# PlatformLab/RAMCloud

Hardware: AMD Instinct MI355X
Metric: device-resident CRC32C GB/s over 8MiB-segment batch; % of HBM roofline (higher is better)
Workload: dtype u8; 1 GPU; 1024 x 8 MiB device-resident segments (BASELINE config 2); segments_per_gpu=1024, segment_bytes=8388608, batch_bytes_per_gpu=8589934592, parallelism=single, exchange=none

## Files before the change

### ramcloud_amd/csrc/dev_checks.inc

```

namespace {

__device__ __forceinline__ uint32_t crc_bytes_g(const uint32_t* t1, uint32_t c, const gu8* p,
                                                uint32_t n)
{
    for (uint32_t k = 0; k < n; k++)
        c = t1[(c ^ p[k]) & 0xFF] ^ (c >> 8);
    return c;
}

__device__ __forceinline__ uint32_t le32_g(const gu8* p)
{
    return uint32_t(p[0]) | (uint32_t(p[1]) << 8) | (uint32_t(p[2]) << 16) | (uint32_t(p[3]) << 24);
}


__device__ __forceinline__ void obj_compare_one(const BatchDesc& d, ramcrc_seg_status* status,
                                                uint64_t i);

__global__ __launch_bounds__(256) void k_obj_compare(BatchDesc d, ramcrc_seg_status* status,
                                                     const uint32_t* nother)
{
    if (nother && *nother == 0)
        return;
    const uint64_t n = entry_count<kRecords>(d);
    for (uint64_t i = uint64_t(blockIdx.x) * blockDim.x + threadIdx.x; i < n;
         i += uint64_t(gridDim.x) * blockDim.x)
        obj_compare_one(d, status, i);
}

__device__ __forceinline__ void obj_compare_one(const BatchDesc& d, ramcrc_seg_status* status,
                                                uint64_t i)
{
    const u32x4 r = d.rec[i];
    const uint32_t type = r.w & 0x3f;
    const uint32_t hdr = replay_header_bytes(type);
    if (hdr == 0)
        return;
    const bool readable = r.z >= hdr && !(r.w & kRecOverlong);
    if (d.vstat && type == RAMCRC_LOG_ENTRY_TYPE_OBJ && readable && !is_large(uint64_t(r.z) - 4))
        return;
    const uint64_t payload = reinterpret_cast<uint64_t>(d.base) + uint64_t(r.x) * d.seg_bytes +
                             r.y + 1 + ((r.w >> 6) & 3) + 1;
    const gu8* p = reinterpret_cast<const gu8*>(payload);
    const uint32_t seg_flags = d.seg_status[r.x].x;
    uint32_t stored = 0, computed = 0;
    if (type == RAMCRC_LOG_ENTRY_TYPE_OBJ && readable) {
        stored = le32_g(p);
        computed = d.out[i];
    }
    if (!(seg_flags & RAMCRC_SEG_OK))
        return;
    bool ok = false;
    if (readable) {
        if (type == RAMCRC_LOG_ENTRY_TYPE_OBJ) {
            ok = computed == stored;
        } else {
            uint32_t at = hdr - 4, from = hdr, tail = 0;
            bool fits = true;
            switch (type) {
            case RAMCRC_LOG_ENTRY_TYPE_OBJTOMB: tail = r.z - hdr; break;
            case RAMCRC_LOG_ENTRY_TYPE_PREP:
                at = kPrepHeaderBytes - 4;
                from = kPrepHeaderBytes + 4;
                tail = r.z - from;
                break;
            case RAMCRC_LOG_ENTRY_TYPE_TXDECISION:
                tail = min(24u * le32_g(p + 36), r.z - hdr);
                break;
            case RAMCRC_LOG_ENTRY_TYPE_TXPLIST:
                tail = 24u * le32_g(p + 16);
                fits = tail <= r.z - hdr;
                break;
            default: break;
            }
            if (fits) {
                const uint32_t* t1 = &g_tab.pos[1 + kTinyRow0][0];
                const uint32_t c = ~crc_bytes_g(t1, crc_bytes_g(t1, 0xFFFFFFFFu, p, at), p + from, tail);
                d.out[i] = c;
                ok = c == le32_g(p + at);
            }
        }
    }
    if (!ok)
        atomicAdd(&status[r.x].bad_objects, 1u);
}

__global__ __launch_bounds__(256) void k_left(BatchDesc d, ramcrc_seg_status* status, const uint32_t* sum,
                                              const uint32_t* left, const unsigned long long* nleft,
                                              uint64_t left_cap, uint64_t nseg)
{
    const uint32_t sv = *sum;
    if (!(sv & kSumFast))
        return;
    const uint64_t tid = uint64_t(blockIdx.x) * blockDim.x + threadIdx.x, nt = uint64_t(gridDim.x) * blockDim.x;
    if (sv & kHardFull) {
        for (uint64_t s = tid; s < nseg; s += nt)
            status[s].bad_objects = 0;
        return;
    }
    const uint64_t nl = *nleft;
    const uint64_t n = nl < left_cap ? nl : left_cap;
    if (uint64_t(blockIdx.x) * blockDim.x >= n)
        return;
    __shared__ uint32_t tx4[4 * 256], tx1[256];
    for (uint32_t t = threadIdx.x; t < 4 * 256; t += blockDim.x)
        tx4[t] = g_tab.comb[0].t[t >> 8][t & 0xFF];
    for (uint32_t t = threadIdx.x; t < 256; t += blockDim.x)
        tx1[t] = g_tab.t0.t[t];
    __syncthreads();
    auto crc_global = [&](uint64_t a, uint32_t m) {
        typedef const __attribute__((address_space(1))) uint32_t g32;
        uint32_t c = 0xFFFFFFFFu;
        while (m && (a & 3)) {
            c = tx1[(c ^ *reinterpret_cast<const gu8*>(a)) & 0xFF] ^ (c >> 8);
            a++;
            m--;
        }
        for (; m >= 8; a += 8, m -= 8) {
            const uint32_t v0 = *reinterpret_cast<g32*>(a), v1 = *reinterpret_cast<g32*>(a + 4);
            uint32_t v = v0 ^ c;
            c = xor3(tx4[v & 0xFF], tx4[256 + ((v >> 8) & 0xFF)], tx4[512 + ((v >> 16) & 0xFF)]) ^
                tx4[768 + (v >> 24)];
            v = v1 ^ c;
            c = xor3(tx4[v & 0xFF], tx4[256 + ((v >> 8) & 0xFF)], tx4[512 + ((v >> 16) & 0xFF)]) ^
                tx4[768 + (v >> 24)];
        }
        while (m) {
            c = tx1[(c ^ *reinterpret_cast<const gu8*>(a)) & 0xFF] ^ (c >> 8);
            a++;
            m--;
        }
        return ~c;
    };
    for (uint64_t k = tid; k < n; k += nt) {
        const uint64_t i = left[k];
        const u32x4 r = d.rec[i];
        if (!replay_other(r)) {
            if ((r.w & 0x3f) != RAMCRC_LOG_ENTRY_TYPE_OBJ || !(d.seg_status[r.x].x & RAMCRC_SEG_OK))
                continue;
            const uint64_t payload = reinterpret_cast<uint64_t>(d.base) + uint64_t(r.x) * d.seg_bytes +
                                     r.y + 1 + ((r.w >> 6) & 3) + 1;
            const gu8* p = reinterpret_cast<const gu8*>(payload);
            const uint32_t c = crc_global(payload + 4, r.z - 4);
            d.out[i] = c;
            if (c != le32_g(p))
                atomicAdd(&status[r.x].bad_objects, 1u);
        } else {
            obj_compare_one(d, status, i);
        }
    }
}

__global__ __launch_bounds__(256) void k_obj_stamp(BatchDesc d)
{
    const uint64_t i = uint64_t(blockIdx.x) * blockDim.x + threadIdx.x;
    if (i >= d.n)
        return;
    if (d.len[i] < kObjHeaderBytes) {
        d.out[i] = 0;
        return;
    }
    const uint32_t c = d.out[i];
    uint8_t* p = const_cast<uint8_t*>(d.base) + d.off[i];
    p[0] = uint8_t(c);
    p[1] = uint8_t(c >> 8);
    p[2] = uint8_t(c >> 16);
    p[3] = uint8_t(c >> 24);
}

__global__ __launch_bounds__(256) void k_cert_prep(const uint32_t* heads, ramcrc_seg_cert* certs,
                                                   uint64_t n)
{
    const uint64_t i = uint64_t(blockIdx.x) * blockDim.x + threadIdx.x;
    if (i < n)
        certs[i] = ramcrc_seg_cert{heads[i], 0u};
}

__global__ __launch_bounds__(256) void k_cert_emit(const ramcrc_seg_cert* tmp,
                                                   const ramcrc_seg_status* st,
                                                   ramcrc_seg_cert* certs, uint32_t* flags, uint64_t n)
{
    const uint64_t i = uint64_t(blockIdx.x) * blockDim.x + threadIdx.x;
    if (i >= n)
        return;
    const ramcrc_seg_status s = st[i];
    certs[i] = ramcrc_seg_cert{tmp[i].segment_length, s.checksum};
    if (flags) {
        const uint32_t bad = s.flags & (RAMCRC_SEG_PAST_CAPACITY | RAMCRC_SEG_PAST_LENGTH |
                                        RAMCRC_SEG_CYCLE);
        flags[i] = bad ? bad : RAMCRC_SEG_OK;
    }
}


}
```

### ramcloud_amd/csrc/dev_chunks.inc

```

namespace {

__device__ __forceinline__ uint32_t scan_chunk(const uint8_t* lds, const RepOp& op, int lane,
                                               uint64_t S, uint64_t E, uint32_t init,
                                               uint64_t lo, uint64_t hi)
{
    uint32_t u0 = 0, u1 = 0, u2 = 0, u3 = 0;
    uint64_t first = lo & ~uint64_t(kBlock - 1);
    const uint64_t end = (hi + kBlock - 1) & ~uint64_t(kBlock - 1);

    auto step = [&](const u32x4& w) {
        u0 = op.apply(lds, u0, w.x);
        u1 = op.apply(lds, u1, w.y);
        u2 = op.apply(lds, u2, w.z);
        u3 = op.apply(lds, u3, w.w);
    };
    auto special = [&](uint64_t blk) {
        const uint64_t a = blk + uint64_t(lane) * 16;
        u32x4 w = {0u, 0u, 0u, 0u};
        if (a < E && a + 16 > S)
            w = load16(a);
        w.x = fix_word(w.x, a + 0, S, E, init);
        w.y = fix_word(w.y, a + 4, S, E, init);
        w.z = fix_word(w.z, a + 8, S, E, init);
        w.w = fix_word(w.w, a + 12, S, E, init);
        step(w);
    };

    while (first < end && (first < S + 4 || first + kBlock > E)) {
        special(first);
        first += kBlock;
    }
    uint64_t fast_end = end;
    if (first < end && end > E)
        fast_end = end - kBlock;

    const uint64_t nf = (fast_end - first) / kBlock;
    if (nf > 0) {
        const uint32_t lo_w = __builtin_amdgcn_readfirstlane(uint32_t(first));
        const uint32_t hi_w = __builtin_amdgcn_readfirstlane(uint32_t(first >> 32));
        const uint32_t nrec = __builtin_amdgcn_readfirstlane(uint32_t(nf * kBlock));
        void* basep = reinterpret_cast<void*>((uint64_t(hi_w) << 32) | lo_w);
        const __amdgpu_buffer_rsrc_t rsrc =
            __builtin_amdgcn_make_buffer_rsrc(basep, (short)0, int(nrec), 0x00020000);
        const uint32_t voff = uint32_t(lane) * 16;
        auto ldb = [&](uint64_t b) -> u32x4 {
            b = b < nf ? b : nf - 1;
            return __builtin_amdgcn_raw_buffer_load_b128(rsrc, voff, uint32_t(b * kBlock),
                                                         2 );
        };
        u32x4 A[kUnroll], B[kUnroll];
#pragma unroll
        for (int j = 0; j < kUnroll; j++)
            A[j] = ldb(j);
        uint64_t i = 0;
        for (; i + 2 * kUnroll <= nf; i += 2 * kUnroll) {
#pragma unroll
            for (int j = 0; j < kUnroll; j++)
                B[j] = ldb(i + kUnroll + j);
            __builtin_amdgcn_sched_barrier(0);
#pragma unroll
            for (int j = 0; j < kUnroll; j++)
                step(A[j]);
#pragma unroll
            for (int j = 0; j < kUnroll; j++)
                A[j] = ldb(i + 2 * kUnroll + j);
            __builtin_amdgcn_sched_barrier(0);
#pragma unroll
            for (int j = 0; j < kUnroll; j++)
                step(B[j]);
        }
#pragma unroll
        for (int j = 0; j < kUnroll; j++)
            if (i + j < nf)
                step(A[j]);
        if (i + kUnroll < nf) {
#pragma unroll
            for (int j = 0; j < kUnroll; j++)
                B[j] = ldb(i + kUnroll + j);
#pragma unroll
            for (int j = 0; j < kUnroll; j++)
                if (i + kUnroll + j < nf)
                    step(B[j]);
        }
    }
    if (fast_end < end)
        special(fast_end);

    uint32_t y = plain_apply(lds, kCombOff, u0) ^ u1;
    y = plain_apply(lds, kCombOff, y) ^ u2;
    y = plain_apply(lds, kCombOff, y) ^ u3;
    uint32_t z = plain_apply(lds, kCombOff, y);
#pragma unroll
    for (int lvl = 0; lvl < 6; lvl++) {
        const uint32_t other = __shfl_xor(z, 1 << lvl, kWaveSize);
        const bool upper = (lane >> lvl) & 1;
        const uint32_t lower_v = upper ? other : z;
        const uint32_t upper_v = upper ? z : other;
        z = plain_apply(lds, kCombOff + (1 + lvl) * 4096, lower_v) ^ upper_v;
    }
    return z;
}

__device__ __forceinline__ bool replay_other(const u32x4& r)
{
    const uint32_t type = r.w & 0x3f;
    const uint32_t hdr = replay_header_bytes(type);
    const bool readable = r.z >= hdr && !(r.w & kRecOverlong);
    return hdr != 0 && !(type == RAMCRC_LOG_ENTRY_TYPE_OBJ && readable && !is_large(uint64_t(r.z) - 4));
}



__device__ __forceinline__ void plan_locate(const Plan& pl, uint64_t n, uint64_t g, uint64_t& entry,
                                            uint64_t& k)
{
    uint64_t lo = 0, hi = pl.ngroups;
    while (hi - lo > 1) {
        const uint64_t mid = (lo + hi) >> 1;
        if (pl.group_pref[mid] <= g) lo = mid; else hi = mid;
    }
    const uint64_t gbase = pl.group_pref[lo];
    uint64_t a = lo * kThreads, b = a + kThreads;
    if (b > n) b = n;
    uint64_t l2 = a, h2 = b;
    while (h2 - l2 > 1) {
        const uint64_t mid = (l2 + h2) >> 1;
        if (gbase + pl.local[mid] <= g) l2 = mid; else h2 = mid;
    }
    entry = l2;
    k = g - gbase - pl.local[l2];
}

template <int kMode>
__global__ __launch_bounds__(kThreads, 1) void k_chunks(BatchDesc d, Plan pl, uint64_t per_seg)
{
    __shared__ __attribute__((aligned(16))) uint8_t lds[kLdsChunks];
    if (kMode != kSegAligned && plan_empty(pl))
        return;
    fill_replicated(lds, g_tab.stride_large);
    fill_plain(lds, kCombOff, &g_tab.comb[0].t[0][0], 7 * 1024);
    __syncthreads();

    const int lane = threadIdx.x & (kWaveSize - 1);
    const RepOp op(lane);
    const uint64_t wave = uint64_t(blockIdx.x) * kWavesPerGroup +
                          __builtin_amdgcn_readfirstlane(threadIdx.x / kWaveSize);
    const uint64_t nwaves = uint64_t(gridDim.x) * kWavesPerGroup;
    const uint64_t total = kMode == kSegAligned ? per_seg * d.n : pl.group_pref[pl.ngroups];
    if (total > pl.partials_cap) {
        if (wave == 0 && lane == 0)
            atomicOr(pl.status, 3u);
        return;
    }
    uint64_t g = wave;
    while (g < total) {
        const uint64_t gnext = g + nwaves;
        uint64_t i, k;
        if (kMode == kSegAligned) {
            i = g / per_seg;
            k = g - i * per_seg;
        } else {
            plan_locate(pl, d.n, g, i, k);
        }
        uint64_t S, E;
        buffer_range<kMode>(d, i, S, E);
        const uint32_t init = d.init ? d.init[i] : 0xFFFFFFFFu;
        const uint64_t cs = S >> d.cshift;
        const uint64_t c_lo = (cs + k) << d.cshift;
        const uint64_t lo = c_lo > S ? c_lo : S;
        const uint64_t c_hi = c_lo + (1ull << d.cshift);
        const uint64_t hi = c_hi < E ? c_hi : E;
        const uint32_t r = scan_chunk(lds, op, lane, S, E, init, lo, hi);
        if (lane == 0)
            pl.partials[g] = r;
        g = gnext;
    }
}

__device__ __forceinline__ uint64_t shfl64(uint64_t v, int src)
{
    const uint32_t lo = __shfl(uint32_t(v), src, kWaveSize);
    const uint32_t hi = __shfl(uint32_t(v >> 32), src, kWaveSize);
    return (uint64_t(hi) << 32) | lo;
}

template <int kMode>
__device__ __forceinline__ void combine_one(const BatchDesc& d, const Plan& pl, uint64_t per_seg,
                                            uint64_t i, uint64_t S, uint64_t E, int lane)
{
    const uint64_t g0 = kMode == kSegAligned ? i * per_seg
                                             : pl.group_pref[i / kThreads] + pl.local[i];
    const uint64_t cnt = chunk_count(S, E, d.cshift);
    const uint64_t cs = S >> d.cshift;
    const uint64_t pend = (E + kBlock - 1) & ~uint64_t(kBlock - 1);
    uint32_t R = 0;
    for (uint64_t k = lane; k < cnt; k += kWaveSize) {
        const uint32_t r = pl.partials[g0 + k];
        const uint64_t ek = (k + 1 == cnt) ? pend : ((cs + k + 1) << d.cshift);
        const uint64_t t = (pend - ek) / kBlock;
        R ^= t ? mulmod_dev(r, xpow_blocks(t)) : r;
    }
#pragma unroll
    for (int lvl = 0; lvl < 6; lvl++)
        R ^= __shfl_xor(R, 1 << lvl, kWaveSize);
    const uint32_t pad = uint32_t(pend - E);
    if (pad)
        R = mulmod_dev(R, g_tab.xinv[pad]);
    if (lane == 0)
        d.out[i] = (d.flags & RAMCRC_FINALIZE) ? ~R : R;
}

template <int kMode, bool kWide>
__global__ __launch_bounds__(256) void k_combine(BatchDesc d, Plan pl, uint64_t per_seg)
{
    const int lane = threadIdx.x & (kWaveSize - 1);
    const uint64_t wave = uint64_t(blockIdx.x) * (256 / kWaveSize) + threadIdx.x / kWaveSize;
    if (kMode != kSegAligned && (plan_empty(pl) || ((*pl.status) & kStatusRefused)))
        return;
    const uint64_t n = entry_count<kMode>(d);
    if (!kWide) {
        if (wave >= n)
            return;
        uint64_t S, E;
        buffer_range<kMode>(d, wave, S, E);
        if (is_large(E - S))
            combine_one<kMode>(d, pl, per_seg, wave, S, E, lane);
        return;
    }
    if (pl.group_pref[pl.ngroups] == 0)
        return;
    const uint64_t nwave = uint64_t(gridDim.x) * (256 / kWaveSize);
    for (uint64_t wv = wave; wv * kWaveSize < n; wv += nwave) {
        const uint64_t i = wv * kWaveSize + lane;
        uint64_t S = 0, E = 0;
        const bool big = i < n && buffer_range<kMode>(d, i, S, E) && is_large(E - S);
        uint64_t todo = __ballot(big);
        while (todo) {
            const int j = __builtin_ctzll(todo);
            todo &= todo - 1;
            combine_one<kMode>(d, pl, per_seg, wv * kWaveSize + j, shfl64(S, j), shfl64(E, j), lane);
        }
    }
}


}
```

### ramcloud_amd/csrc/dev_host.inc

```

namespace {

thread_local int t_last_hip = 0;

#define HIPCHK(expr)                              \
    do {                                          \
        hipError_t e_ = (expr);                   \
        if (e_ != hipSuccess) {                   \
            t_last_hip = int(e_);                 \
            return RAMCRC_EHIP;                   \
        }                                         \
    } while (0)

struct DeviceGuard {
    int prev = -1;
    bool ok = false;
    explicit DeviceGuard(int dev)
    {
        if (hipGetDevice(&prev) != hipSuccess)
            prev = -1;
        ok = hipSetDevice(dev) == hipSuccess;
    }
    ~DeviceGuard()
    {
        if (prev >= 0)
            (void)hipSetDevice(prev);
    }
};

}

struct ramcrc_ctx {
    int device = 0;
    int ncu = 256;
    int ncu_all = 256;
    std::recursive_mutex mu;
    uint32_t* partials = nullptr;
    uint64_t partials_cap = 0;
    uint64_t* plan_local = nullptr;
    uint64_t plan_cap = 0;
    uint64_t* group_pref = nullptr;
    uint64_t group_cap = 0;
    uint32_t* status = nullptr;
    BinTable* bins = nullptr;
    uint32_t bin_par = 0;
    int fail_after_count = 0;
    uint32_t dirty_bins = 0;
    int bin_straggler = 0;
    int bin_resident[5] = {-1, -1, -1, -1, -1};
    int bin_one = 0;
    u32x4* sdesc = nullptr;
    uint32_t* sidx = nullptr;
    uint32_t* sinit = nullptr;
    uint64_t sorted_cap = 0;
    uint32_t* obj_out = nullptr;
    uint64_t obj_out_cap = 0;
    uint32_t* cert_scratch = nullptr;
    uint64_t cert_scratch_cap = 0;
    uint8_t* h_stage = nullptr;
    uint64_t h_stage_cap = 0;
    uint8_t* d_stage = nullptr;
    uint64_t d_stage_cap = 0;
    hipStream_t copy_stream = nullptr;
    hipStream_t compute_stream = nullptr;
    void* walk_parts = nullptr;
    uint64_t walk_parts_cap = 0;
    uint32_t* walk_fallback = nullptr;
    uint64_t walk_fallback_cap = 0;
    uint64_t* walk_base = nullptr;
    uint64_t walk_base_cap = 0;
    void* walk_recs = nullptr;
    uint64_t walk_recs_cap = 0;
    void* walk_pool = nullptr;
    uint64_t walk_pool_cap = 0;
    uint32_t* walk_pool_owner = nullptr;
    uint64_t walk_pool_owner_cap = 0;
    uint32_t* walk_blocks = nullptr;
    uint64_t walk_blocks_cap = 0;
    unsigned long long* walk_pool_used = nullptr;
    uint64_t walk_pool_used_cap = 0;
    int verify_in_walk = 1;
    uint32_t* walk_left = nullptr;
    uint64_t walk_left_cap = 0;
    uint32_t* walk_sum = nullptr;
    uint64_t walk_sum_cap = 0;
    bool serial_walk = false;
    uint32_t walk_pshift = 0;
    bool timing = false;
    std::vector<std::pair<hipEvent_t, hipEvent_t>> ev_used, ev_free;
};

namespace {

int grow_device(void** p, uint64_t* cap, uint64_t need_elems, size_t elem)
{
    if (*cap >= need_elems && *p)
        return RAMCRC_OK;
    uint64_t n = need_elems < 1024 ? 1024 : need_elems;
    if (*p) {
        HIPCHK(hipDeviceSynchronize());
        HIPCHK(hipFree(*p));
        *p = nullptr;
        *cap = 0;
    }
    if (hipMalloc(p, n * elem) != hipSuccess) {
        *p = nullptr;
        return RAMCRC_ENOMEM;
    }
    *cap = n;
    return RAMCRC_OK;
}

int reserve_locked(ramcrc_ctx* c, uint64_t max_chunks, uint64_t max_entries)
{
    int rc = grow_device(reinterpret_cast<void**>(&c->partials), &c->partials_cap, max_chunks,
                         sizeof(uint32_t));
    if (rc)
        return rc;
    rc = grow_device(reinterpret_cast<void**>(&c->plan_local), &c->plan_cap, max_entries,
                     sizeof(uint64_t));
    if (rc)
        return rc;
    const uint64_t ngroups = (max_entries + kThreads - 1) / kThreads + 1;
    return grow_device(reinterpret_cast<void**>(&c->group_pref), &c->group_cap, ngroups,
                       sizeof(uint64_t));
}

uint64_t default_chunk_bound(uint64_t n)
{
    size_t free_b = 0, total_b = 0;
    if (hipMemGetInfo(&free_b, &total_b) != hipSuccess)
        total_b = 288ull << 30;
    return total_b / kChunk + 2 * n + 16;
}

Plan make_plan(ramcrc_ctx* c, uint64_t n)
{
    Plan pl{};
    pl.local = c->plan_local;
    pl.group_pref = c->group_pref;
    pl.ngroups = (n + kThreads - 1) / kThreads;
    pl.partials = c->partials;
    pl.partials_cap = c->partials_cap;
    pl.status = c->status;
    return pl;
}

constexpr unsigned kTimerEventFlags = hipEventDisableSystemFence;

struct ScanTimer {
    ramcrc_ctx* c;
    hipStream_t s;
    std::pair<hipEvent_t, hipEvent_t> ev{nullptr, nullptr};
    ScanTimer(ramcrc_ctx* ctx, hipStream_t stream) : c(ctx), s(stream)
    {
        if (!c->timing)
            return;
        if (!c->ev_free.empty()) {
            ev = c->ev_free.back();
            c->ev_free.pop_back();
        } else if (hipEventCreateWithFlags(&ev.first, kTimerEventFlags) != hipSuccess ||
                   hipEventCreateWithFlags(&ev.second, kTimerEventFlags) != hipSuccess) {
            ev = {nullptr, nullptr};
        }
    }
    template <typename F, typename... Args>
    void launch(F kernel, dim3 grid, dim3 block, Args... args)
    {
        if (ev.first)
            hipExtLaunchKernelGGL(kernel, grid, block, 0, s, ev.first, ev.second, 0, args...);
        else
            hipLaunchKernelGGL(kernel, grid, block, 0, s, args...);
    }
    ~ScanTimer()
    {
        if (ev.first)
            c->ev_used.push_back(ev);
    }
};

int reserve_sorted(ramcrc_ctx* c, uint64_t n)
{
    const uint64_t need = n + uint64_t(kG) * kNB;
    if (c->sorted_cap >= need)
        return RAMCRC_OK;
    uint64_t cap = c->sorted_cap;
    int rc = grow_device(reinterpret_cast<void**>(&c->sdesc), &cap, need, sizeof(u32x4));
    if (rc)
        return rc;
    cap = c->sorted_cap;
    rc = grow_device(reinterpret_cast<void**>(&c->sidx), &cap, need, sizeof(uint32_t));
    if (rc)
        return rc;
    cap = c->sorted_cap;
    rc = grow_device(reinterpret_cast<void**>(&c->sinit), &cap, need, sizeof(uint32_t));
    if (rc)
        return rc;
    c->sorted_cap = cap;
    return RAMCRC_OK;
}

uint64_t bin_grid(const ramcrc_ctx* c, uint64_t n)
{
    uint64_t grid = (n + uint64_t(kThreads) * kBinPer - 1) / (uint64_t(kThreads) * kBinPer);
    if (grid > uint64_t(c->ncu) * kBinWgsPerCu)
        grid = uint64_t(c->ncu) * kBinWgsPerCu;
    return grid;
}

template <int kMode>
int bin_begin(ramcrc_ctx* c, const BatchDesc& d, hipStream_t s, int skip_large, Sorted* so,
              const uint32_t* sum = nullptr)
{
    if (d.n >= (1ull << 32))
        return RAMCRC_EINVAL;
    int rc = reserve_sorted(c, d.n);
    if (rc)
        return rc;
    *so = Sorted{c->bins, c->sdesc, c->sidx, c->sinit, c->status, c->sorted_cap, c->bin_par, 0};
    if (hipError_t stale = hipGetLastError(); stale != hipSuccess)
        t_last_hip = int(stale);
    const uint64_t tiles = (d.n + uint64_t(kThreads) * kBinPer - 1) / (uint64_t(kThreads) * kBinPer);
    int& resident = c->bin_resident[kMode];
    if (resident < 0) {
        int nb = 0;
        if (hipOccupancyMaxActiveBlocksPerMultiprocessor(&nb, k_bin_one<kMode>, kThreads, 0) !=
            hipSuccess)
            nb = 0;
        resident = nb;
    }
    if (c->bin_one && !c->dirty_bins && !sum && tiles > 0 &&
        tiles <= uint64_t(c->ncu) * uint64_t(std::min(resident / 2, int(kBinWgsPerCu)))) {
        so->one = 1;
        hipLaunchKernelGGL(k_bin_one<kMode>, dim3(tiles), dim3(kThreads), 0, s, d, *so, skip_large,
                           c->bin_straggler ? 1u : 0u);
        c->bin_straggler = 0;
    } else {
        hipLaunchKernelGGL(k_bin_count<kMode>, dim3(bin_grid(c, d.n)), dim3(kThreads), 0, s, d,
                           *so, skip_large, sum);
    }
    HIPCHK(hipGetLastError());
    c->bin_par ^= 1u;
    return RAMCRC_OK;
}

template <int kMode>
int bin_finish(ramcrc_ctx* c, const BatchDesc& d, hipStream_t s, int skip_large, const Sorted& so,
               const uint32_t* sum = nullptr)
{
    if (c->fail_after_count > 0) {
        c->fail_after_count--;
        return RAMCRC_EHIP;
    }
    if (c->dirty_bins) {
        hipLaunchKernelGGL(k_test_dirty_bins, dim3(1), dim3(1), 0, s, c->bins, so.par,
                           uint32_t(c->dirty_bins >> 16), uint32_t(c->dirty_bins & 0xFFFF));
        c->dirty_bins = 0;
        HIPCHK(hipGetLastError());
    }
    {
        hipLaunchKernelGGL(k_bin_scatter<kMode>, dim3(bin_grid(c, d.n)), dim3(kThreads), 0, s, d,
                           so, skip_large, int(so.one), sum);
        HIPCHK(hipGetLastError());
    }
    {
        ScanTimer t(c, s);
        t.launch(k_entries, dim3(c->ncu), dim3(kEntWaves * kWaveSize), d, so);
    }
    HIPCHK(hipGetLastError());
    return RAMCRC_OK;
}

template <int kMode>
int launch_binned(ramcrc_ctx* c, const BatchDesc& d, hipStream_t s, int skip_large)
{
    Sorted so;
    int rc = bin_begin<kMode>(c, d, s, skip_large, &so);
    if (rc)
        return rc;
    return bin_finish<kMode>(c, d, s, skip_large, so);
}

template <int kMode>
int launch_planned(ramcrc_ctx* c, const BatchDesc& d, hipStream_t s, const uint32_t** nother = nullptr,
                   const uint32_t* sum = nullptr)
{
    Sorted so;
    int rc = bin_begin<kMode>(c, d, s, 1, &so, sum);
    if (rc)
        return rc;
    if (nother)
        *nother = &so.bt->ctr[so.par].nother;
    Plan pl = make_plan(c, d.n);
    pl.nlarge = &so.bt->ctr[so.par].nlarge;
    const uint64_t gcap = uint64_t(4) * c->ncu;
    hipLaunchKernelGGL(k_plan_count<kMode>, dim3(uint32_t(pl.ngroups < gcap ? pl.ngroups : gcap)),
                       dim3(kThreads), 0, s, d, pl);
    HIPCHK(hipGetLastError());
    hipLaunchKernelGGL(k_plan_scan, dim3(1), dim3(kThreads), 0, s, pl);
    HIPCHK(hipGetLastError());
    {
        ScanTimer t(c, s);
        t.launch(k_chunks<kMode>, dim3(c->ncu), dim3(kThreads), d, pl, uint64_t(0));
    }
    HIPCHK(hipGetLastError());
    const uint64_t cw = (d.n + 255) / 256, ccap = uint64_t(16) * c->ncu;
    if (d.n > kWideCombineMin)
        hipLaunchKernelGGL((k_combine<kMode, true>), dim3(uint32_t(cw < ccap ? cw : ccap)), dim3(256), 0, s,
                           d, pl, uint64_t(0));
    else
        hipLaunchKernelGGL((k_combine<kMode, false>), dim3((d.n + 3) / 4), dim3(256), 0, s, d, pl,
                           uint64_t(0));
    HIPCHK(hipGetLastError());
    return bin_finish<kMode>(c, d, s, 1, so, sum);
}


}
```

### ramcloud_amd/csrc/dev_plan.inc

```

namespace {

template <int kMode>
__global__ __launch_bounds__(kThreads) void k_plan_count(BatchDesc d, Plan pl)
{
    __shared__ uint64_t wsum[kWavesPerGroup];
    if (plan_empty(pl))
        return;
    const uint64_t n = entry_count<kMode>(d);
    for (uint64_t grp = blockIdx.x; grp < pl.ngroups; grp += gridDim.x) {
        const uint64_t i = grp * kThreads + threadIdx.x;
        uint64_t c = 0;
        if (i < n) {
            uint64_t S, E;
            buffer_range<kMode>(d, i, S, E);
            c = is_large(E - S) ? chunk_count(S, E, d.cshift) : 0;
        }
        const int lane = threadIdx.x & 63, w = threadIdx.x >> 6;
        uint64_t x = c;
#pragma unroll
        for (int s = 1; s < 64; s <<= 1) {
            const uint64_t y = __shfl_up(x, s, kWaveSize);
            if (lane >= s)
                x += y;
        }
        if (lane == 63)
            wsum[w] = x;
        __syncthreads();
        uint64_t before = 0;
        for (int j = 0; j < w; j++)
            before += wsum[j];
        if (i < d.n)
            pl.local[i] = before + x - c;
        if (threadIdx.x == kThreads - 1)
            pl.group_pref[grp] = before + x;
        __syncthreads();
    }
}

__global__ __launch_bounds__(kThreads) void k_plan_scan(Plan pl)
{
    __shared__ uint64_t wsum[kWavesPerGroup];
    __shared__ uint64_t carry_s;
    const int lane = threadIdx.x & 63, w = threadIdx.x >> 6;
    if (threadIdx.x == 0) {
        carry_s = 0;
        atomicAnd(pl.status, ~kStatusRefused);
    }
    if (plan_empty(pl)) {
        if (threadIdx.x == 0)
            pl.group_pref[pl.ngroups] = 0;
        return;
    }
    __syncthreads();
    for (uint64_t base = 0; base < pl.ngroups; base += kThreads) {
        const uint64_t i = base + threadIdx.x;
        const uint64_t c = i < pl.ngroups ? pl.group_pref[i] : 0;
        uint64_t x = c;
#pragma unroll
        for (int s = 1; s < 64; s <<= 1) {
            const uint64_t y = __shfl_up(x, s, kWaveSize);
            if (lane >= s)
                x += y;
        }
        if (lane == 63)
            wsum[w] = x;
        __syncthreads();
        uint64_t before = carry_s;
        for (int j = 0; j < w; j++)
            before += wsum[j];
        if (i < pl.ngroups)
            pl.group_pref[i] = before + x - c;
        __syncthreads();
        if (threadIdx.x == kThreads - 1)
            carry_s = before + x;
        __syncthreads();
    }
    if (threadIdx.x == 0)
        pl.group_pref[pl.ngroups] = carry_s;
}

__global__ void k_test_dirty_bins(BinTable* bt, uint32_t par, uint32_t bin, uint32_t add)
{
    if (bin < kNB)
        bt->ctr[par].hist[bin] += add;
}

__global__ void k_status_take(uint32_t* status)
{
    status[1] = atomicAnd(status, ~(kStatusSticky | kStatusBins));
}


}
```

### ramcloud_amd/csrc/dev_walk.inc

```

namespace {

constexpr uint32_t kWalkWin = 16384;
constexpr uint32_t kWalkStep = kWalkWin - 16;
constexpr int kWalkPer = int(kWalkWin / 16 / kWaveSize);
constexpr uint32_t kWalkMeta = 5 * kWaveSize;

struct WalkDesc {
    const uint8_t* base;
    uint64_t stride;
    uint64_t capacity;
    uint64_t nseg;
    const ramcrc_seg_cert* certs;
    ramcrc_seg_status* status;
    u32x4* entries;
    uint64_t cap;
    unsigned long long* n_entries;
    const uint32_t* only;
    uint64_t* seg_base;
    uint32_t* sum;
};

__device__ __forceinline__ uint32_t crc_small(const uint32_t* t, uint32_t c, uint32_t v, uint32_t m)
{
    const uint32_t x = c ^ v;
    uint32_t r = m >= 4 ? 0u : (c >> (8 * m));
#pragma unroll
    for (uint32_t k = 0; k < 4; k++)
        if (k < m)
            r ^= t[(m - 1 - k) * 256 + ((x >> (8 * k)) & 0xFF)];
    return r;
}

__device__ __forceinline__ void walk_issue(u32x4 (&r)[kWalkPer], uint64_t sb, uint64_t wbase,
                                           uint64_t capacity, int lane)
{
    const uint64_t base = rfl64(sb + wbase);
    const uint32_t nrec =
        __builtin_amdgcn_readfirstlane(uint32_t(wbase < capacity ? capacity - wbase : 0));
    const __amdgpu_buffer_rsrc_t rsrc =
        __builtin_amdgcn_make_buffer_rsrc(reinterpret_cast<void*>(base), (short)0, int(nrec),
                                          0x00020000);
#pragma unroll
    for (int k = 0; k < kWalkPer; k++)
        r[k] = __builtin_amdgcn_raw_buffer_load_b128(rsrc, uint32_t(lane + kWaveSize * k) * 16, 0, 0);
}

__device__ __forceinline__ void walk_store(uint8_t* win, const u32x4 (&r)[kWalkPer], int lane)
{
#pragma unroll
    for (int k = 0; k < kWalkPer; k++)
        *reinterpret_cast<u32x4*>(win + (lane + kWaveSize * k) * 16) = r[k];
}

__global__ __launch_bounds__(kWaveSize) void k_seg_walk(WalkDesc w)
{
    __shared__ __attribute__((aligned(16))) uint8_t win[2][kWalkWin];
    __shared__ __attribute__((aligned(16))) uint32_t tab[4 * 256];
    __shared__ uint32_t xm[kWalkMeta + 1];
    fill_plain(reinterpret_cast<uint8_t*>(tab), 0, &g_tab.pos[1 + kTinyRow0][0], 4 * 256);
    for (uint32_t t = threadIdx.x; t <= kWalkMeta; t += blockDim.x)
        xm[t] = g_tab.xmeta[t];
    __syncthreads();
    const int lane = threadIdx.x;
    uint32_t hard = 0;

    for (uint64_t seg = blockIdx.x; seg < w.nseg; seg += gridDim.x) {
        if (w.only && !w.only[seg])
            continue;
        const uint64_t sb = reinterpret_cast<uint64_t>(w.base) + seg * w.stride;
        const ramcrc_seg_cert cert = w.certs[seg];
        unsigned long long rbase = 0, rdone = 0, rtotal = 0;
        for (int pass = 0; pass < 2; pass++) {
        uint32_t pos = 0, crc = 0xFFFFFFFFu, count = 0, flags = 0;
        uint32_t rpos = 0, rq = 0;
        uint32_t ns = 0;

        auto flush = [&](uint32_t nrec, uint32_t tail) {
            const uint32_t pn = __shfl_down(rpos, 1, kWaveSize);
            const uint32_t nxt = lane + 1 == int(ns) ? tail : pn;
            const uint32_t hdr = rq & 0xFF, lb = (hdr >> 6) + 1;
            const uint32_t rlen = nxt - rpos - 1 - lb;
            const uint32_t rinfo = hdr | (rlen > ~(rpos + 1 + lb) ? kRecOverlong : 0u);
            uint32_t m = 0, r = 0;
            if (lane < int(ns)) {
                m = 1 + lb;
                r = crc_small(tab, 0u, hdr | (rlen << 8), m < 4 ? m : 4);
                if (m == 5)
                    r = crc_small(tab, r, rlen >> 24, 1);
            }
            uint32_t incl = m;
#pragma unroll
            for (int s = 1; s < kWaveSize; s <<= 1) {
                const uint32_t y = __shfl_up(incl, s, kWaveSize);
                if (lane >= s)
                    incl += y;
            }
            const uint32_t total = __shfl(incl, kWaveSize - 1, kWaveSize);
            uint32_t c = lane < int(ns) ? mulmod_horner(r, xm[total - incl]) : 0u;
#pragma unroll
            for (int s = 1; s < kWaveSize; s <<= 1)
                c ^= __shfl_xor(c, s, kWaveSize);
            crc = mulmod_horner(crc, xm[total]) ^ c;
            if (nrec && pass == 0) {
                rtotal += nrec;
            } else if (nrec) {
                const unsigned long long b = rbase + rdone;
                if (lane < int(nrec) && b + lane < w.cap) {
                    w.entries[b + lane] = u32x4{uint32_t(seg), rpos, rlen, rinfo};
                    hard |= w.sum ? replay_hard(rpos, rlen, rinfo) | kHardFull : 0u;
                }
                rdone += nrec;
            }
            ns = 0;
        };

        int cur = 0;
        uint32_t wb = 0;
        u32x4 pf[kWalkPer];
        __syncthreads();
        walk_issue(pf, sb, 0, w.capacity, lane);
        walk_store(win[0], pf, lane);
        walk_issue(pf, sb, kWalkStep, w.capacity, lane);
        __syncthreads();

        const uint32_t cap32 = uint32_t(w.capacity);
        const uint32_t limit = cert.segment_length < cap32 ? cert.segment_length : cap32;
        uint32_t steps = 0, tail = 0;
        bool overrun = false;
        while (pos < limit) {
            if (steps >= cap32) {
                flags |= RAMCRC_SEG_CYCLE;
                break;
            }
            if (pos - wb > kWalkWin - 8) {
                const uint64_t nb = uint64_t(wb) + kWalkStep;
                if (uint64_t(pos) >= nb && uint64_t(pos) - nb <= kWalkWin - 8) {
                    walk_store(win[cur ^ 1], pf, lane);
                    cur ^= 1;
                    wb = uint32_t(nb);
                } else {
                    wb = pos & ~15u;
                    walk_issue(pf, sb, wb, w.capacity, lane);
                    walk_store(win[cur], pf, lane);
                }
                __syncthreads();
                walk_issue(pf, sb, uint64_t(wb) + kWalkStep, w.capacity, lane);
            }
            if (ns == uint32_t(kWaveSize))
                flush(ns, pos);
            const uint32_t* w32 = reinterpret_cast<const uint32_t*>(win[cur]);
            const uint64_t wend = uint64_t(wb) + (kWalkWin - 8);
            const uint32_t last = limit - 1 < wend ? limit - 1 : uint32_t(wend);
            const uint32_t span = last - wb;
            uint32_t nsmax = uint32_t(kWaveSize);
            if (cap32 - steps < nsmax - ns)
                nsmax = ns + (cap32 - steps);
            const uint32_t ns0 = ns;
            uint32_t next;
            for (;;) {
                const uint32_t o = pos - wb;
                const uint32_t d0 = __builtin_amdgcn_readfirstlane(w32[o >> 2]);
                const uint32_t d1 = __builtin_amdgcn_readfirstlane(w32[(o >> 2) + 1]);
                const uint64_t q = ((uint64_t(d1) << 32) | d0) >> (8 * (o & 3));
                const uint32_t t = (uint32_t(q) >> 6) & 3;
                uint32_t fld;
                uint64_t len64;
                asm("s_lshl_b32 %0, %2, 19\n\ts_add_u32 %0, %0, 0x80008\n\ts_bfe_u64 %1, %3, %0"
                    : "=&s"(fld), "=s"(len64) : "s"(t), "s"(q) : "scc");
                next = pos + t + 2 + uint32_t(len64);
                const bool mine = lane == int(ns);
                rpos = mine ? pos : rpos;
                rq = mine ? uint32_t(q) : rq;
                ns++;
                if (next - wb > span)
                    break;
                if (ns == nsmax)
                    break;
                pos = next;
            }
            steps += ns - ns0;
            tail = next;
            if (next > cap32) {
                flags |= RAMCRC_SEG_PAST_CAPACITY;
                overrun = true;
                break;
            }
            pos = next;
        }
        count = steps - (overrun ? 1u : 0u);
        if (ns)
            flush(overrun ? ns - 1 : ns, tail);
        if (pass == 0) {
            unsigned long long b = 0;
            if (lane == 0 && rtotal)
                b = atomicAdd(w.n_entries, rtotal);
            rbase = __shfl(b, 0, kWaveSize);
            if (lane == 0 && w.seg_base)
                w.seg_base[seg] = rbase;
            if (rtotal == 0)
                pass = 1;
        }
        if (rbase + rtotal > w.cap)
            flags |= RAMCRC_SEG_TABLE_FULL;
        if (pass == 0)
            continue;
        const uint32_t fin = ~crc_small(tab, crc, cert.segment_length, 4);
        if (!(flags & (RAMCRC_SEG_PAST_CAPACITY | RAMCRC_SEG_CYCLE))) {
            if (pos > cert.segment_length)
                flags |= RAMCRC_SEG_PAST_LENGTH;
            else if (fin != cert.checksum)
                flags |= RAMCRC_SEG_BAD_CHECKSUM;
            else if (!(flags & RAMCRC_SEG_TABLE_FULL))
                flags |= RAMCRC_SEG_OK;
        }
        if (lane == 0) {
            ramcrc_seg_status st;
            st.flags = flags;
            st.checksum = fin;
            st.entries = count;
            st.bad_objects = 0;
            w.status[seg] = st;
        }
        }
    }
    {
        const uint32_t hw = (__ballot(hard & 1u) ? 1u : 0u) | (__ballot(hard & 2u) ? 2u : 0u) |
                           (__ballot(hard & 4u) ? 4u : 0u) | (__ballot(hard & kHardFull) ? kHardFull : 0u);
        if (w.sum && hw && lane == 0)
            atomicOr(w.sum, hw);
    }
}

#ifndef RAMCRC_PART_SHIFT
#define RAMCRC_PART_SHIFT 16
#endif
constexpr uint32_t kPartShift = RAMCRC_PART_SHIFT;
constexpr uint32_t kPartShiftMin = 13;
constexpr uint32_t kNoStart = 0xFFFFFFFFu;
#ifndef RAMCRC_SYNC_HOPS
#define RAMCRC_SYNC_HOPS 6
#endif
#ifndef RAMCRC_SYNC_PER
#define RAMCRC_SYNC_PER 8
#endif
#ifndef RAMCRC_SYNC_STAGE_KIB
#define RAMCRC_SYNC_STAGE_KIB 7
#endif
constexpr int kSyncHops = RAMCRC_SYNC_HOPS;
constexpr int kSyncPer = RAMCRC_SYNC_PER;
constexpr uint32_t kSyncRound = kSyncPer * kWaveSize;
static_assert(kSyncPer % 4 == 0 && kSyncPer <= 32, "candidates per lane: whole dwords");
constexpr uint32_t kSyncSpan = 16384;
constexpr uint32_t kSyncStage = RAMCRC_SYNC_STAGE_KIB * 1024;
constexpr uint32_t kMeetMax = 4;
constexpr uint32_t kMeetHops = 3;
constexpr uint32_t kRewalkBudget = 1u << 15;
constexpr uint32_t kPartWalked = 1u, kPartWrap = 2u, kPartOverrun = 4u, kPartEmit = 8u;
constexpr uint32_t kPartSpill = 16u;
constexpr uint32_t kPartChase = 32u;
constexpr uint32_t kPartHuge = 64u;
constexpr uint32_t kMaxBlocks = 15;
constexpr uint32_t kPartRec = 64;

struct PartRes {
    uint32_t start;
    uint32_t exit;
    uint32_t count;
    uint32_t nmeta;
    uint32_t raw;
    uint32_t flags;
    uint64_t rec;
    uint32_t pre;
    uint32_t cut;
};

struct PWalk {
    const uint8_t* base;
    uint64_t stride;
    uint32_t capacity;
    uint32_t nparts;
    uint64_t nseg;
    const ramcrc_seg_cert* certs;
    ramcrc_seg_status* status;
    u32x4* entries;
    uint64_t cap;
    unsigned long long* n_entries;
    PartRes* parts;
    uint32_t* fallback;
    uint64_t* seg_base;
    uint2* recs;
    uint32_t pshift;
    const uint32_t* geo;
    uint2* pool;
    uint32_t* pool_owner;
    uint32_t* blocks;
    unsigned long long* pool_used;
    uint64_t pool_cap;
    uint32_t* sum;
    uint32_t* obj_crc;
    uint32_t* left;
    unsigned long long* nleft;
    uint64_t left_cap;
    uint32_t vmode;
};

typedef const __attribute__((address_space(1))) uint32_t gu32;

__device__ __forceinline__ uint64_t seg_peek(uint64_t seg, uint32_t pos, uint32_t capacity)
{
    const uint32_t a = pos & ~3u;
    const bool two = a + 4 < capacity;
    const uint32_t w0 = *reinterpret_cast<gu32*>(seg + a);
    uint32_t w1 = *reinterpret_cast<gu32*>(seg + (two ? a + 4 : a));
    w1 = two ? w1 : 0u;
    return ((uint64_t(w1) << 32) | w0) >> (8 * (pos & 3));
}

__device__ __forceinline__ uint32_t meta_update(const uint32_t* tab, uint32_t c, uint64_t q,
                                                uint32_t mbytes)
{
    c = crc_small(tab, c, uint32_t(q), mbytes < 4 ? mbytes : 4);
    if (mbytes == 5)
        c = crc_small(tab, c, uint32_t(q >> 32), 1);
    return c;
}

__device__ __forceinline__ uint32_t xpow8_dev(uint32_t d)
{
    uint32_t r = ramcrc::kOne;
#pragma unroll
    for (int j = 0; j < 4; j++) {
        const uint32_t b = (d >> (8 * j)) & 0xFF;
        if (b)
            r = r == ramcrc::kOne ? g_tab.xbyte[j][b] : mulmod_dev(r, g_tab.xbyte[j][b]);
    }
    return r;
}

__device__ __forceinline__ uint32_t walk_limit(const PWalk& w, uint64_t seg)
{
    const uint32_t len = w.certs[seg].segment_length;
    return len < w.capacity ? len : w.capacity;
}

__device__ __forceinline__ PWalk walk_geo(PWalk w)
{
    if (w.geo) {
        w.pshift = *w.geo;
        w.nparts = uint32_t((uint64_t(w.capacity) + (1ull << w.pshift) - 1) >> w.pshift);
    }
    return w;
}

constexpr uint32_t kPartShiftMax = 20;
constexpr int kProbeHops = 8;
constexpr uint32_t kPartShiftLow = kPartShift;

__device__ __forceinline__ uint32_t walk_sum_seen(const uint32_t* sum)
{
    return sum ? __hip_atomic_load(sum, __ATOMIC_RELAXED, __HIP_MEMORY_SCOPE_AGENT) : kHardAll;
}

#ifndef RAMCRC_FAST_MEAN
#define RAMCRC_FAST_MEAN 176
#endif
constexpr uint32_t kFastMean = RAMCRC_FAST_MEAN;
constexpr uint32_t kFastMean8 = 120;

constexpr uint32_t kLeftMax = 1024;
__device__ __forceinline__ uint32_t left_append(const PWalk& w, uint64_t slot, uint32_t len, uint32_t hdr)
{
    const uint32_t type = hdr & 0x3f;
    if (replay_header_bytes(type) == 0)
        return 0u;
    if (type == RAMCRC_LOG_ENTRY_TYPE_OBJ && !(hdr & kRecOverlong) && len >= kObjHeaderBytes &&
        len > kLeftMax)
        return kHardFull;
    const unsigned long long k = atomicAdd(w.nleft, 1ull);
    if (k >= w.left_cap || slot > 0xFFFFFFFFull)
        return kHardFull;
    w.left[k] = uint32_t(slot);
    return 0u;
}

__global__ __launch_bounds__(kWaveSize) void k_walk_probe(PWalk w, uint32_t forced, uint32_t* geo)
{
    const int lane = threadIdx.x;
    const uint64_t ns = w.nseg < uint64_t(kWaveSize) ? w.nseg : uint64_t(kWaveSize);
    uint64_t dist = 0, hops = 0;
    if (!forced && uint64_t(lane) < ns) {
        const uint64_t seg = uint64_t(lane) * w.nseg / ns;
        const uint64_t sb = reinterpret_cast<uint64_t>(w.base) + seg * w.stride;
        const uint32_t limit = walk_limit(w, seg);
        uint32_t pos = 0;
        for (int hh = 0; hh < kProbeHops && pos < limit; hh++) {
            const uint64_t q = seg_peek(sb, pos, w.capacity);
            const Hop h = hop_of(q, pos);
            if (!plausible(q, h, w.capacity) || h.next > limit)
                break;
            dist += h.next - pos;
            hops++;
            pos = uint32_t(h.next);
        }
    }
#pragma unroll
    for (int o = 1; o < kWaveSize; o <<= 1) {
        dist += __shfl_xor(dist, o, kWaveSize);
        hops += __shfl_xor(hops, o, kWaveSize);
    }
    if (lane == 0) {
        *w.n_entries = 0;
        w.pool_used[0] = 0;
        if (w.nleft)
            *w.nleft = 0;
        uint32_t shift = kPartShift;
        if (forced) {
            shift = forced;
        } else if (hops) {
            const uint64_t t = 64 * (dist / hops);
            uint32_t l = 63 - uint32_t(__builtin_clzll(t | 1));
            if (t * t >= (1ull << (2 * l)) * 2)
                l++;
            shift = l < kPartShift ? kPartShift : (l > kPartShiftMax ? kPartShiftMax : l);
            if (shift == 17)
                shift = 18;
        }
        *geo = shift;
        uint32_t sstage = kSyncStage;
        if (!forced && hops) {
            const uint64_t want = ((16 * (dist / hops)) + 1023) & ~uint64_t(1023);
            sstage = uint32_t(want < 1024 ? 1024 : (want > kSyncStage ? kSyncStage : want));
        }
        geo[1] = sstage;
        if (w.sum) {
            const bool fast = w.obj_crc && w.nleft &&
                              (w.vmode == 2 || (hops && dist <= uint64_t(kFastMean) * hops));
            const bool small = hops && dist <= uint64_t(kFastMean8) * hops;
            *w.sum = fast ? (kSumFast | (small ? kSumStage8 : 0u)) : 0u;
        }
    }
}

constexpr uint32_t kSyncWin = kSyncStage - 16;
constexpr int kSyncWaves = 4;
constexpr uint64_t kSyncJunkKey = 1ull << 63;

__device__ __forceinline__ uint32_t wave_min(uint32_t v)
{
    v = min(v, uint32_t(__builtin_amdgcn_update_dpp(-1, int(v), 0xB1, 0xF, 0xF, false)));
    v = min(v, uint32_t(__builtin_amdgcn_update_dpp(-1, int(v), 0x4E, 0xF, 0xF, false)));
    v = min(v, uint32_t(__builtin_amdgcn_update_dpp(-1, int(v), 0x141, 0xF, 0xF, false)));
    v = min(v, uint32_t(__builtin_amdgcn_update_dpp(-1, int(v), 0x140, 0xF, 0xF, false)));
    v = min(v, uint32_t(__builtin_amdgcn_update_dpp(-1, int(v), 0x142, 0xA, 0xF, false)));
    v = min(v, uint32_t(__builtin_amdgcn_update_dpp(-1, int(v), 0x143, 0xC, 0xF, false)));
    return uint32_t(__builtin_amdgcn_readlane(int(v), 63));
}

struct SyncPart {
    uint64_t sb;
    uint32_t k;
    uint32_t B;
    uint32_t seglen;
};

__device__ __forceinline__ SyncPart sync_part(const PWalk& w, uint64_t i)
{
    SyncPart P;
    const uint64_t seg = i / w.nparts;
    P.k = uint32_t(i - seg * w.nparts);
    P.B = P.k << w.pshift;
    P.seglen = w.certs[seg].segment_length;
    P.sb = reinterpret_cast<uint64_t>(w.base) + seg * w.stride;
    return P;
}

__global__ __launch_bounds__(kSyncWaves * kWaveSize) void k_walk_sync(PWalk w0)
{
    const PWalk w = walk_geo(w0);
    __shared__ __attribute__((aligned(16))) uint8_t wins[kSyncWaves][kSyncStage];
    __shared__ uint16_t lists[kSyncWaves][kSyncRound];
    constexpr uint32_t kSU = kSyncStage / 1024;
    const int lane = threadIdx.x & (kWaveSize - 1);
    const int wv = threadIdx.x / kWaveSize;
    uint8_t* win = wins[wv];
    uint16_t* list = lists[wv];
    const uint64_t nwave = uint64_t(gridDim.x) * kSyncWaves;
    const uint64_t total = w.nseg * w.nparts;
    u32x4 v[kSU];
    const uint32_t ss = w.geo ? __builtin_amdgcn_readfirstlane(w.geo[1]) : kSyncStage;
    auto stage_load = [&](const SyncPart& P) {
#pragma unroll
        for (uint32_t u = 0; u < kSU; u++) {
            const uint64_t a = uint64_t(P.B) + u * 1024 + uint32_t(lane) * 16;
            if (u * 1024 < ss)
                v[u] = a + 16 <= w.capacity ? load16(P.sb + a) : u32x4{0u, 0u, 0u, 0u};
        }
    };
    uint64_t i = uint64_t(blockIdx.x) * kSyncWaves + wv;
    SyncPart nxt{};
    if (i < total) {
        nxt = sync_part(w, i);
        if (nxt.k != 0)
            stage_load(nxt);
    }
    for (; i < total; i += nwave) {
        const SyncPart P = nxt;
        const uint32_t B = P.B;
        const uint64_t sb = P.sb;
        const uint32_t limit = P.seglen < w.capacity ? P.seglen : w.capacity;
        uint64_t end64 = uint64_t(B) + kSyncSpan;
        end64 = end64 < uint64_t(B) + (1ull << w.pshift) ? end64 : uint64_t(B) + (1ull << w.pshift);
        end64 = end64 < w.capacity ? end64 : w.capacity;
        const uint32_t end = uint32_t(end64 < limit ? end64 : limit);
        const bool search_part = P.k != 0 && end > B;
        if (search_part) {
#pragma unroll
            for (uint32_t u = 0; u < kSU; u++)
                if (u * 1024 < ss)
                    *reinterpret_cast<u32x4*>(win + u * 1024 + uint32_t(lane) * 16) = v[u];
        }
        if (i + nwave < total) {
            nxt = sync_part(w, i + nwave);
            if (nxt.k != 0)
                stage_load(nxt);
        }
        if (!search_part) {
            if (P.k != 0 && lane == 0)
                w.parts[i].start = kNoStart;
            continue;
        }
        asm volatile("s_waitcnt lgkmcnt(0)" ::: "memory");
        auto peek_lds = [&](uint32_t p) -> uint64_t {
            const uint32_t o = p - B;
            const uint32_t* w32 = reinterpret_cast<const uint32_t*>(win + (o & ~3u));
            return ((uint64_t(w32[1]) << 32) | w32[0]) >> (8 * (o & 3));
        };
        auto peek = [&](uint32_t p) -> uint64_t {
            return p - B + 8 <= ss ? peek_lds(p) : seg_peek(sb, p, w.capacity);
        };
        const bool kill4 = w.capacity <= (1u << 24);
        const bool kill3 = w.capacity <= (1u << 23);
        auto search = [&](auto lds_only_c, uint32_t to) -> uint32_t {
            constexpr bool lds_only = decltype(lds_only_c)::value;
            auto peek_any = [&](uint32_t p) -> uint64_t {
                if constexpr (lds_only)
                    return peek_lds(p);
                else
                    return peek(p);
            };
            const uint32_t wend = B + ss - 16;
            uint64_t best = ~0ull;
            uint32_t bound = 0xFFFFFFFFu;
            for (uint32_t c0 = B; c0 < to && c0 < bound && !(best < kSyncJunkKey);
                 c0 += kSyncRound) {
                const uint32_t cl = c0 + uint32_t(lane) * kSyncPer;
                constexpr int kWords = (kSyncPer / 4 + 3) & ~1;
                uint32_t d[kWords];
#pragma unroll
                for (int u = 0; u < kWords; u += 2) {
                    const uint32_t pc = cl + 4 * u;
                    const uint64_t v = peek_any(lds_only && pc - B > ss - 8 ? B + ss - 8 : pc);
                    d[u] = uint32_t(v);
                    d[u + 1] = uint32_t(v >> 32);
                }
                uint32_t alive = 0;
#pragma unroll
                for (int g = 0; g < kSyncPer / 4; g++)
                    alive |= first_hop4(d[g], __builtin_amdgcn_alignbyte(d[g + 1], d[g], 3), kill4,
                                        kill3)
                             << (4 * g);
                alive &= to > cl ? (to - cl >= kSyncPer ? ~0u : (1u << (to - cl)) - 1u) : 0u;
                uint32_t total = 0;
#pragma unroll
                for (int j = 0; j < kSyncPer; j++) {
                    const uint64_t m = __ballot((alive >> j) & 1);
                    const uint32_t at = total + __builtin_amdgcn_mbcnt_hi(
                                                    uint32_t(m >> 32), __builtin_amdgcn_mbcnt_lo(uint32_t(m), 0u));
                    if ((alive >> j) & 1)
                        list[at] = uint16_t(uint32_t(lane) * kSyncPer + j);
                    total += uint32_t(__popcll(m));
                }
                asm volatile("s_waitcnt lgkmcnt(0)" ::: "memory");
                for (uint32_t t0 = 0; t0 < total; t0 += kWaveSize) {
                    const bool have = t0 + uint32_t(lane) < total;
                    const uint32_t c = c0 + (have ? list[t0 + uint32_t(lane)] : 0u);
                    bool live = have;
                    bool junk = false;
                    uint32_t p = c, first = 0, second = 0;
                    for (int hh = 0; hh < kSyncHops && __ballot(live && p < limit); hh++) {
                        if (live && p < limit) {
                            if (hh > 0 && lds_only && p >= wend) {
                                live = false;
                            } else {
                                const uint64_t q = peek_any(p);
                                const Hop h = hop_of(q, p);
                                if (plausible(q, h, w.capacity) && h.next <= limit && h.len != 0) {
                                    p = uint32_t(h.next);
                                    const uint32_t ty = uint32_t(q) & 0x3F;
                                    junk = junk || (ty != RAMCRC_LOG_ENTRY_TYPE_OBJ &&
                                                    ty != RAMCRC_LOG_ENTRY_TYPE_OBJTOMB);
                                } else {
                                    live = false;
                                }
                            }
                        }
                        if (hh == 0)
                            first = p;
                        if (hh == 1)
                            second = p;
                    }
                    if (second == 0)
                        second = p;
                    if (first == 0)
                        first = p;
                    const uint32_t fb = wave_min(live ? first : 0xFFFFFFFFu);
                    bound = fb < bound ? fb : bound;
                    for (int cls = 0; cls < 2; cls++) {
                        const bool lc = live && (cls == 1 || !junk);
                        const uint32_t s2 = wave_min(lc ? second : 0xFFFFFFFFu);
                        if (s2 != 0xFFFFFFFFu) {
                            const uint64_t tie = __ballot(lc && second == s2);
                            const uint32_t lo = __popcll(tie) == 1
                                                    ? uint32_t(__builtin_amdgcn_readlane(int(c), __builtin_ctzll(tie)))
                                                    : wave_min(lc && second == s2 ? c : 0xFFFFFFFFu);
                            const uint64_t key = (cls ? kSyncJunkKey : 0ull) |
                                                 (uint64_t(s2) << 32) | lo;
                            best = key < best ? key : best;
                            break;
                        }
                    }
                }
            }
            return best == ~0ull ? kNoStart : uint32_t(best);
        };
        const uint32_t lds_to = B + ss - 24 < end ? B + ss - 24 : end;
        uint32_t guess = search(std::true_type{}, lds_to);
        if (guess == kNoStart)
            guess = search(std::false_type{}, end);
        if (lane == 0)
            w.parts[i].start = guess;
    }
}

struct GlobalPeek {
    uint64_t sb;
    uint32_t capacity;
    __device__ uint64_t operator()(uint32_t p) const { return seg_peek(sb, p, capacity); }
};

template <class Sink, class Peek>
__device__ __forceinline__ void walk_lane(const PWalk& w, const uint32_t* tab, uint32_t pos,
                                          uint32_t stop, PartRes& r, Sink&& sink, uint32_t budget,
                                          Peek&& peek)
{
    uint32_t count = 0, nmeta = 0, raw = 0, flags = kPartWalked, hops = 0;
    uint64_t q = pos < stop ? peek(pos) : 0ull;
    while (pos < stop) {
        if (hops++ >= budget) {
            flags |= kPartWrap;
            break;
        }
        const Hop h = hop_of(q, pos);
        raw = meta_update(tab, raw, q, h.mbytes);
        nmeta += h.mbytes;
        if (h.next > 0xFFFFFFFFull) {
            flags |= kPartWrap;
            break;
        }
        if (h.next > w.capacity) {
            flags |= kPartOverrun;
            break;
        }
        const uint32_t next = uint32_t(h.next);
        const uint64_t qn = next < stop ? peek(next) : 0ull;
        sink(count, pos, h.len, uint32_t(q) & 0xFF);
        count++;
        pos = next;
        q = qn;
    }
    r.exit = pos;
    r.count = count;
    r.nmeta = nmeta;
    r.raw = raw;
    r.flags = flags;
}

template <class Sink>
__device__ __forceinline__ void walk_lane(const PWalk& w, const uint32_t* tab, uint64_t seg,
                                          uint64_t sb, uint32_t pos, uint32_t stop, PartRes& r,
                                          Sink&& sink, uint32_t budget)
{
    walk_lane(w, tab, pos, stop, r, sink, budget, GlobalPeek{sb, w.capacity});
}

#ifndef RAMCRC_FIX_WIN_KIB
#define RAMCRC_FIX_WIN_KIB 16
#endif
constexpr uint32_t kFixWin = RAMCRC_FIX_WIN_KIB * 1024;
struct WinPeek {
    uint8_t* lds;
    uint64_t sb;
    uint32_t capacity;
    uint32_t wb;
    __device__ uint64_t operator()(uint32_t p)
    {
        if (wb == kNoStart || p < wb || ((p - wb) & ~3u) + 8 > kFixWin) {
            const uint32_t b = p & ~15u;
            const uint32_t l16 = (threadIdx.x & (kWaveSize - 1)) * 16;
            u32x4 v[kFixWin / 1024];
#pragma unroll
            for (uint32_t u = 0; u < kFixWin / 1024; u++) {
                const uint64_t a = uint64_t(b) + u * 1024 + l16;
                v[u] = a + 16 <= capacity ? load16(sb + a) : u32x4{0u, 0u, 0u, 0u};
            }
#pragma unroll
            for (uint32_t u = 0; u < kFixWin / 1024; u++)
                *reinterpret_cast<u32x4*>(lds + u * 1024 + l16) = v[u];
            asm volatile("s_waitcnt lgkmcnt(0)" ::: "memory");
            wb = b;
        }
        const uint32_t o = p - wb;
        const uint32_t* w32 = reinterpret_cast<const uint32_t*>(lds + (o & ~3u));
        return ((uint64_t(w32[1]) << 32) | w32[0]) >> (8 * (o & 3));
    }
};

struct NoSink {
    __device__ void operator()(uint32_t, uint32_t, uint32_t, uint32_t) const {}
};

struct TableSink {
    u32x4* out;
    uint64_t n;
    uint32_t seg;
    uint32_t* hard;
    const PWalk* fast = nullptr;
    uint64_t slot0 = 0;
    __device__ void operator()(uint32_t idx, uint32_t pos, uint32_t len, uint32_t hdr) const
    {
        if (idx < n) {
            out[idx] = u32x4{seg, pos, len, hdr};
            if (hard)
                *hard |= replay_hard(pos, len, hdr);
            if (fast)
                *hard |= left_append(*fast, slot0 + idx, len, hdr);
        }
    }
};

__device__ __forceinline__ void walk_tab_fill(uint32_t* tab)
{
    for (uint32_t t = threadIdx.x; t < 4 * 256; t += blockDim.x)
        tab[t] = g_tab.pos[1 + kTinyRow0 + t / 256][t % 256];
    __syncthreads();
}

constexpr uint32_t kLRec = kPartRec;
__device__ __forceinline__ uint32_t lrec_slot(uint32_t e, uint32_t t)
{
    return (e + t) & (kLRec - 1);
}
__global__ __launch_bounds__(256) void k_walk_parts(PWalk w0)
{
    const PWalk w = walk_geo(w0);
    __shared__ uint32_t tab[4 * 256];
    __shared__ uint2 lrec[256][kLRec];
    walk_tab_fill(tab);
    const uint64_t i = uint64_t(blockIdx.x) * blockDim.x + threadIdx.x;
    const bool valid = i < w.nseg * w.nparts;
    PartRes r{};
    uint2* mine = lrec[threadIdx.x];
    bool huge = false, lost = false;
    uint32_t curk = 0;
    auto put_block = [&](uint32_t j, uint32_t n) {
        const uint32_t b = j * kLRec / kPartRec, off = (j * kLRec) % kPartRec;
        uint2* dst = nullptr;
        if (b == 0) {
            dst = w.recs + i * kPartRec + off;
        } else if (b <= kMaxBlocks && !lost) {
            if (off == 0) {
                const unsigned long long k = atomicAdd(w.pool_used, 1ull);
                curk = k < w.pool_cap ? uint32_t(k) : 0xFFFFFFFFu;
                if (curk != 0xFFFFFFFFu) {
                    w.blocks[i * kMaxBlocks + (b - 1)] = curk;
                    w.pool_owner[k] = uint32_t(i * 16 + b);
                }
            }
            if (curk != 0xFFFFFFFFu)
                dst = w.pool + uint64_t(curk) * kPartRec + off;
        }
        if (!dst) {
            lost = true;
            return;
        }
        for (uint32_t e = 0; e < n; e += 2) {
            const uint2 a0 = mine[lrec_slot(e, threadIdx.x)], a1 = mine[lrec_slot(e + 1, threadIdx.x)];
            if (e + 1 < n)
                *reinterpret_cast<uint4*>(dst + e) = make_uint4(a0.x, a0.y, a1.x, a1.y);
            else
                dst[e] = a0;
        }
    };
    if (valid) {
        const uint64_t seg = i / w.nparts;
        const uint32_t k = uint32_t(i - seg * w.nparts);
        const uint32_t B = k << w.pshift;
        const uint32_t limit = walk_limit(w, seg);
        r = w.parts[i];
        const uint32_t start = k == 0 ? 0u : r.start;
        r.start = start;
        if (start == kNoStart || B >= limit) {
            r.flags = 0;
            r.count = r.nmeta = r.raw = 0;
            r.exit = start;
        } else {
            const uint32_t pend = uint32_t(uint64_t(B) + (1ull << w.pshift) < w.capacity
                                               ? uint64_t(B) + (1ull << w.pshift) : w.capacity);
            const uint64_t sb = reinterpret_cast<uint64_t>(w.base) + seg * w.stride;
            auto sink = [&](uint32_t idx, uint32_t pos, uint32_t len, uint32_t hdr) {
                if (idx == kLRec)
                    put_block(0, kLRec);
                mine[lrec_slot(idx, threadIdx.x)] = make_uint2(pos, (len << 8) | hdr);
                huge = huge || len >= (1u << 24);
                if (idx >= kLRec && (idx & (kLRec - 1)) == kLRec - 1)
                    put_block(idx / kLRec, kLRec);
            };
            const uint32_t stop = pend < limit ? pend : limit;
            walk_lane(w, tab, seg, sb, start, stop, r, sink, 1u << w.pshift);
            if (r.count > kLRec && (r.count & (kLRec - 1)))
                put_block(r.count / kLRec, r.count & (kLRec - 1));
            if (r.count > kPartRec * (1 + kMaxBlocks) || huge || lost)
                r.flags |= kPartSpill;
            if (huge)
                r.flags |= kPartHuge;
        }
        w.parts[i] = r;
    }
    asm volatile("s_waitcnt lgkmcnt(0)" ::: "memory");
    const int lane = threadIdx.x & (kWaveSize - 1);
    const bool flush = valid && (r.flags & kPartWalked) && !(r.flags & kPartHuge) && r.count <= kLRec;
    uint64_t todo = __ballot(flush);
    while (todo) {
        const int j = __builtin_ctzll(todo);
        todo &= todo - 1;
        const uint32_t n = __shfl(r.count, j, kWaveSize);
        const uint64_t dst = (i - uint64_t(lane) + uint64_t(j)) * kPartRec;
        const uint32_t t = (threadIdx.x & ~63u) + uint32_t(j);
        const uint2* src = lrec[t];
        for (uint32_t e = uint32_t(lane); e < n; e += kWaveSize)
            w.recs[dst + e] = src[lrec_slot(e, t)];
    }
}


__global__ __launch_bounds__(kWaveSize) void k_walk_fix(PWalk w0)
{
    const PWalk w = walk_geo(w0);
    __shared__ uint32_t tab[4 * 256];
    __shared__ __attribute__((aligned(16))) uint8_t win[kFixWin];
    walk_tab_fill(tab);
    const int lane = threadIdx.x;
    for (uint64_t seg = blockIdx.x; seg < w.nseg; seg += gridDim.x) {
        const uint32_t limit = walk_limit(w, seg);
        const ramcrc_seg_cert cert = w.certs[seg];
        const uint64_t sb = reinterpret_cast<uint64_t>(w.base) + seg * w.stride;
        WinPeek wpeek{win, sb, w.capacity, kNoStart};
        PartRes* parts = w.parts + seg * w.nparts;
        uint32_t pos = 0, crc = 0xFFFFFFFFu, count = 0, rewalk = 0;
        bool overrun = false, fallback = false;
        auto fold = [&](bool acc, uint32_t nmeta, uint32_t raw) {
            const uint32_t nm = acc ? nmeta : 0u;
            uint32_t incl = nm;
#pragma unroll
            for (int s = 1; s < kWaveSize; s <<= 1) {
                const uint32_t y = __shfl_down(incl, s, kWaveSize);
                if (lane + s < kWaveSize)
                    incl += y;
            }
            const uint32_t n_all = __shfl(incl, 0, kWaveSize);
            uint32_t c = acc ? mulmod_horner(raw, xpow8_dev(incl - nm)) : 0u;
#pragma unroll
            for (int s = 1; s < kWaveSize; s <<= 1)
                c ^= __shfl_xor(c, s, kWaveSize);
            crc = mulmod_horner(crc, xpow8_dev(n_all)) ^ c;
        };
        auto meet_at = [&](uint32_t k, uint32_t st, uint32_t fl, uint32_t gc, uint32_t pe,
                           uint32_t& wr, uint32_t& wn) -> int {
            wr = wn = 0;
            const uint64_t Ek = (uint64_t(k) << w.pshift) + (1ull << w.pshift);
            if (!(fl & kPartWalked) || (fl & kPartWrap) || uint64_t(pe) >= Ek)
                return -1;
            const uint32_t gn = (fl & kPartHuge) ? 0u : (gc < kPartRec ? gc : kPartRec);
            const uint64_t base = (uint64_t(seg) * w.nparts + k) * kPartRec;
            uint32_t p = pe;
            for (uint32_t hh = 0;; hh++) {
                if (p == st)
                    return int(hh << 8);
                for (uint32_t c = 1; c <= kMeetMax && c < gn; c++)
                    if (w.recs[base + c].x == p)
                        return int((hh << 8) | c);
                if (hh == kMeetHops || p >= limit || uint64_t(p) >= Ek)
                    return -1;
                const uint64_t q = seg_peek(sb, p, w.capacity);
                const Hop h = hop_of(q, p);
                if (h.next > w.capacity)
                    return -1;
                wr = meta_update(tab, wr, q, h.mbytes);
                wn += h.mbytes;
                p = uint32_t(h.next);
            }
        };
        const uint32_t nlive =
            limit == 0 ? 0u : uint32_t((uint64_t(limit) + (1ull << w.pshift) - 1) >> w.pshift);
        for (uint32_t k0 = 0; k0 < nlive && !overrun && !fallback; k0 += kWaveSize) {
            const uint32_t k = k0 + uint32_t(lane);
            const bool in = k < nlive;
            PartRes r{};
            if (in)
                r = parts[k];
            const uint32_t gst = r.start;
            constexpr int kResolved = -2;
            uint32_t ex = r.exit, wr = 0, wn = 0;
            int mt = -1;
            {
                uint32_t pe = __shfl_up(ex, 1, kWaveSize);
                pe = lane == 0 ? pos : pe;
                if (in)
                    mt = meet_at(k, gst, r.flags, r.count, pe, wr, wn);
                if (mt > 0)
                    r.start = pe;
            }
            bool ok = !in || mt >= 0, emit = in && mt >= 0;
            while (true) {
                const uint64_t bad = __ballot(!ok);
                if (!bad)
                    break;
                const int j = int(__builtin_ctzll(bad));
                const uint64_t ovr = __ballot(emit && (r.flags & kPartOverrun));
                if (ovr && int(__builtin_ctzll(ovr)) < j)
                    break;
                const uint32_t kj = k0 + uint32_t(j);
                const uint32_t pe = j == 0 ? pos : uint32_t(__builtin_amdgcn_readlane(int(ex), j - 1));
                const uint32_t st = uint32_t(__builtin_amdgcn_readlane(int(gst), j));
                const uint32_t fl = uint32_t(__builtin_amdgcn_readlane(int(r.flags), j));
                const uint64_t Ej64 = (uint64_t(kj) << w.pshift) + (1ull << w.pshift);
                const uint32_t Ej = uint32_t(Ej64 < w.capacity ? Ej64 : w.capacity);
                const uint32_t stop = Ej < limit ? Ej : limit;
                const uint32_t budget = rewalk < kRewalkBudget ? kRewalkBudget - rewalk : 0u;
                bool jemit = true;
                uint32_t jex = pe;
                if (uint64_t(pe) >= Ej64) {
                    jemit = false;
                } else if (fl & kPartWalked) {
                    const uint32_t gc = uint32_t(__builtin_amdgcn_readlane(int(r.count), j));
                    const uint32_t gn = (fl & kPartHuge) ? 0u : (gc < kPartRec ? gc : kPartRec);
                    const uint64_t pidx = uint64_t(seg) * w.nparts + kj;
                    uint2 g = make_uint2(0xFFFFFFFFu, 0u);
                    if (uint32_t(lane) < gn)
                        g = w.recs[pidx * kPartRec + uint32_t(lane)];
                    uint32_t p = pe, wc = 0, wnn = 0, wrr = 0, wflags = kPartWalked;
                    int cut = -1;
                    uint2 mine = make_uint2(0u, 0u), mine0 = make_uint2(0u, 0u);
                    uint64_t mq = 0;
                    uint32_t myblk = 0xFFFFFFFFu;
                    bool huge = false, pool_ok = true;
                    auto fold_block = [&](uint32_t n) {
                        const bool inr = uint32_t(lane) < n;
                        const uint32_t mb = inr ? uint32_t((mq >> 6) & 3) + 2 : 0u;
                        const uint32_t re = inr ? meta_update(tab, 0u, mq, mb) : 0u;
                        uint32_t incl = mb;
#pragma unroll
                        for (int s2 = 1; s2 < kWaveSize; s2 <<= 1) {
                            const uint32_t y = __shfl_down(incl, s2, kWaveSize);
                            if (lane + s2 < kWaveSize)
                                incl += y;
                        }
                        const uint32_t hn = __shfl(incl, 0, kWaveSize);
                        uint32_t hr = inr ? mulmod_horner(re, xpow8_dev(incl - mb)) : 0u;
#pragma unroll
                        for (int s2 = 1; s2 < kWaveSize; s2 <<= 1)
                            hr ^= __shfl_xor(hr, s2, kWaveSize);
                        wrr = mulmod_horner(wrr, xpow8_dev(hn)) ^ hr;
                        wnn += hn;
                    };
                    auto store_block = [&](uint32_t b, uint32_t n) {
                        if (b == 0) {
                            mine0 = mine;
                            return;
                        }
                        if (!pool_ok || b > kMaxBlocks) {
                            pool_ok = false;
                            return;
                        }
                        unsigned long long k = 0;
                        if (lane == 0)
                            k = atomicAdd(w.pool_used, 1ull);
                        k = __shfl(k, 0, kWaveSize);
                        if (k >= w.pool_cap) {
                            pool_ok = false;
                            return;
                        }
                        if (uint32_t(lane) < n)
                            w.pool[k * kPartRec + uint32_t(lane)] = mine;
                        if (lane == 0)
                            w.pool_owner[k] = 0xFFFFFFFFu;
                        if (uint32_t(lane) == b)
                            myblk = uint32_t(k);
                    };
                    while (true) {
                        const uint64_t hit = __ballot(uint32_t(lane) < gn && g.x == p);
                        if (hit || (!(fl & kPartWrap) && p == st)) {
                            cut = hit ? int(__builtin_ctzll(hit)) : 0;
                            break;
                        }
                        if (p >= stop)
                            break;
                        if (wc >= budget) {
                            wflags |= kPartWrap;
                            break;
                        }
                        const uint64_t q = wpeek(p);
                        const Hop h = hop_of(q, p);
                        if (uint32_t(lane) == (wc & (kWaveSize - 1)))
                            mq = q;
                        if (h.next > 0xFFFFFFFFull) {
                            wflags |= kPartWrap;
                            break;
                        }
                        if (h.next > w.capacity) {
                            wflags |= kPartOverrun;
                            break;
                        }
                        if (uint32_t(lane) == (wc & (kWaveSize - 1)))
                            mine = make_uint2(p, (h.len << 8) | (uint32_t(q) & 0xFF));
                        huge = huge || h.len >= (1u << 24);
                        wc++;
                        p = uint32_t(h.next);
                        if ((wc & (kWaveSize - 1)) == 0) {
                            fold_block(kWaveSize);
                            store_block(wc / kWaveSize - 1, kWaveSize);
                        }
                    }
                    rewalk += wc + 1;
                    {
                        const uint32_t rem = (wc & (kWaveSize - 1)) +
                                             ((wflags & (kPartWrap | kPartOverrun)) ? 1u : 0u);
                        if (rem)
                            fold_block(rem);
                    }
                    if (cut >= 0 && (fl & kPartWrap)) {
                        wflags |= kPartWrap;
                    } else if (cut >= 0) {
                        const bool inp = lane < cut;
                        const uint32_t mb = inp ? ((g.y >> 6) & 3) + 2 : 0u;
                        const uint64_t qe = uint64_t(g.y & 0xFF) | (uint64_t(g.y >> 8) << 8);
                        const uint32_t re = inp ? meta_update(tab, 0u, qe, mb) : 0u;
                        uint32_t incl = mb;
#pragma unroll
                        for (int s = 1; s < kWaveSize; s <<= 1) {
                            const uint32_t y = __shfl_down(incl, s, kWaveSize);
                            if (lane + s < kWaveSize)
                                incl += y;
                        }
                        const uint32_t pn = __shfl(incl, 0, kWaveSize);
                        uint32_t pr = inp ? mulmod_horner(re, xpow8_dev(incl - mb)) : 0u;
#pragma unroll
                        for (int s = 1; s < kWaveSize; s <<= 1)
                            pr ^= __shfl_xor(pr, s, kWaveSize);
                        const uint32_t tn = uint32_t(__builtin_amdgcn_readlane(int(r.nmeta), j));
                        const uint32_t tr = uint32_t(__builtin_amdgcn_readlane(int(r.raw), j));
                        const uint32_t sn = tn - pn;
                        const uint32_t sr = tr ^ mulmod_horner(pr, xpow8_dev(sn));
                        jex = uint32_t(__builtin_amdgcn_readlane(int(r.exit), j));
                        const uint32_t nn = wnn + sn;
                        const uint32_t rr = mulmod_horner(wrr, xpow8_dev(sn)) ^ sr;
                        if (lane == j) {
                            r.start = pe;
                            r.count = wc + gc - uint32_t(cut);
                            r.nmeta = nn;
                            r.raw = rr;
                            r.pre = wc;
                            r.cut = uint32_t(cut);
                            mt = kResolved;
                        }
                    } else {
                        jex = p;
                        if (wc > kPartRec && (wc & (kPartRec - 1)))
                            store_block(wc / kPartRec, wc & (kPartRec - 1));
                        const bool keep = !huge && pool_ok && wc <= kPartRec * (1 + kMaxBlocks);
                        if (keep) {
                            const uint2 first = wc <= kPartRec ? mine : mine0;
                            if (uint32_t(lane) < (wc < kPartRec ? wc : kPartRec))
                                w.recs[pidx * kPartRec + uint32_t(lane)] = first;
                            const uint32_t nb = (wc + kPartRec - 1) / kPartRec;
                            if (lane >= 1 && uint32_t(lane) <= kMaxBlocks) {
                                const uint32_t own = uint32_t(pidx * 16 + uint32_t(lane));
                                const uint32_t old = w.blocks[pidx * kMaxBlocks + uint32_t(lane) - 1];
                                if (old < w.pool_cap && w.pool_owner[old] == own)
                                    w.pool_owner[old] = 0xFFFFFFFFu;
                                if (uint32_t(lane) < nb) {
                                    w.blocks[pidx * kMaxBlocks + uint32_t(lane) - 1] = myblk;
                                    w.pool_owner[myblk] = own;
                                }
                            }
                        }
                        if (lane == j) {
                            r.start = pe;
                            r.exit = p;
                            r.count = wc;
                            r.nmeta = wnn;
                            r.raw = wrr;
                            r.flags = keep ? wflags : (wflags | kPartChase);
                            r.pre = r.cut = 0;
                            mt = kResolved;
                        }
                    }
                    if (wflags & kPartWrap)
                        fallback = true;
                } else {
                    PartRes x;
                    uint2 mine = make_uint2(0u, 0u);
                    bool huge = false;
                    walk_lane(w, tab, pe, stop, x,
                              [&](uint32_t idx, uint32_t rp, uint32_t len, uint32_t hdr) {
                                  if (uint32_t(lane) == idx)
                                      mine = make_uint2(rp, (len << 8) | hdr);
                                  huge = huge || len >= (1u << 24);
                              },
                              budget, wpeek);
                    rewalk += x.count + 1;
                    jex = x.exit;
                    const bool keep = x.count <= kPartRec && !huge;
                    if (keep && uint32_t(lane) < x.count)
                        w.recs[(uint64_t(seg) * w.nparts + kj) * kPartRec + uint32_t(lane)] = mine;
                    if (lane == j) {
                        r.start = pe;
                        r.exit = x.exit;
                        r.count = x.count;
                        r.nmeta = x.nmeta;
                        r.raw = x.raw;
                        r.flags = keep ? x.flags : (x.flags | kPartChase);
                        r.pre = r.cut = 0;
                        mt = kResolved;
                    }
                    if (x.flags & kPartWrap)
                        fallback = true;
                }
                if (fallback)
                    break;
                if (lane == j) {
                    ok = true;
                    emit = jemit;
                    ex = jex;
                    mt = kResolved;
                }
                if (lane == j + 1 && in) {
                    mt = meet_at(k, gst, r.flags, r.count, jex, wr, wn);
                    r.start = mt > 0 ? jex : gst;
                    ok = mt >= 0;
                    emit = ok;
                }
            }
            if (fallback)
                break;
            const uint64_t ovr = __ballot(emit && (r.flags & kPartOverrun));
            const int olane = ovr ? int(__builtin_ctzll(ovr)) : kWaveSize;
            if (lane > olane)
                emit = false;
            if (emit && mt > 0) {
                const uint32_t hops = uint32_t(mt) >> 8, cut = uint32_t(mt) & 0xFF;
                const uint64_t base = (uint64_t(seg) * w.nparts + k) * kPartRec;
                uint32_t jr = 0, jn = 0;
                for (uint32_t e = 0; e < cut; e++) {
                    const uint2 g = w.recs[base + e];
                    const uint32_t mb = ((g.y >> 6) & 3) + 2;
                    const uint64_t qe = uint64_t(g.y & 0xFF) | (uint64_t(g.y >> 8) << 8);
                    jr = meta_update(tab, jr, qe, mb);
                    jn += mb;
                }
                const uint32_t tn = r.nmeta - jn;
                const uint32_t tr = r.raw ^ mulmod_horner(jr, xpow8_dev(tn));
                r.raw = mulmod_horner(wr, xpow8_dev(tn)) ^ tr;
                r.nmeta = wn + tn;
                r.count = hops + r.count - cut;
                r.pre = hops;
                r.cut = cut;
            } else if (emit && mt == 0) {
                r.pre = r.cut = 0;
            }
            const uint32_t c = emit ? r.count : 0u;
            uint32_t incl = c;
#pragma unroll
            for (int s = 1; s < kWaveSize; s <<= 1) {
                const uint32_t y = __shfl_up(incl, s, kWaveSize);
                if (lane >= s)
                    incl += y;
            }
            fold(emit, r.nmeta, r.raw);
            if (emit) {
                r.rec = count + incl - c;
                r.flags |= kPartEmit;
                parts[k] = r;
            }
            count += uint32_t(__builtin_amdgcn_readlane(int(incl), kWaveSize - 1));
            const int last = olane < kWaveSize ? olane
                                               : int(nlive - 1 - k0 < uint32_t(kWaveSize - 1)
                                                         ? nlive - 1 - k0 : uint32_t(kWaveSize - 1));
            pos = uint32_t(__builtin_amdgcn_readlane(int(ex), last));
            overrun = olane < kWaveSize;
        }
        if (fallback) {
            if (lane == 0)
                w.fallback[seg] = 1;
            continue;
        }
        uint32_t flags = 0;
        const uint32_t fin = ~crc_small(tab, crc, cert.segment_length, 4);
        if (overrun)
            flags |= RAMCRC_SEG_PAST_CAPACITY;
        else if (pos > cert.segment_length)
            flags |= RAMCRC_SEG_PAST_LENGTH;
        else if (fin != cert.checksum)
            flags |= RAMCRC_SEG_BAD_CHECKSUM;
        unsigned long long b = 0;
        if (lane == 0 && count)
            b = atomicAdd(w.n_entries, (unsigned long long)count);
        b = __shfl(b, 0, kWaveSize);
        if (b + count > w.cap)
            flags |= RAMCRC_SEG_TABLE_FULL;
        if (!(flags & (RAMCRC_SEG_PAST_CAPACITY | RAMCRC_SEG_PAST_LENGTH | RAMCRC_SEG_BAD_CHECKSUM |
                       RAMCRC_SEG_TABLE_FULL)))
            flags |= RAMCRC_SEG_OK;
        if (lane == 0) {
            w.fallback[seg] = 0;
            w.seg_base[seg] = b;
            ramcrc_seg_status st;
            st.flags = flags;
            st.checksum = fin;
            st.entries = count;
            st.bad_objects = 0;
            w.status[seg] = st;
        }
    }
}

__global__ __launch_bounds__(256) void k_walk_emit(PWalk w0)
{
    const PWalk w = walk_geo(w0);
    __shared__ uint32_t tab[4 * 256];
    walk_tab_fill(tab);
    const uint64_t i = uint64_t(blockIdx.x) * blockDim.x + threadIdx.x;
    const bool valid = i < w.nseg * w.nparts;
    const uint64_t seg = valid ? i / w.nparts : 0;
    PartRes r{};
    bool emit = false;
    uint64_t slot = 0;
    if (valid) {
        r = w.parts[i];
        emit = (r.flags & kPartEmit) && !w.fallback[seg];
        if (emit)
            slot = w.seg_base[seg] + r.rec;
    }
    const bool chase = emit && (r.flags & (kPartChase | kPartSpill));
    const uint32_t pre = emit && !chase ? r.pre : 0u;
    uint32_t hard = 0;
    if (chase || pre) {
        const uint32_t k = uint32_t(i - seg * w.nparts);
        const uint32_t B = k << w.pshift;
        const uint32_t limit = walk_limit(w, seg);
        const uint32_t pend = uint32_t(uint64_t(B) + (1ull << w.pshift) < w.capacity ? uint64_t(B) + (1ull << w.pshift)
                                                                             : w.capacity);
        const uint64_t sb = reinterpret_cast<uint64_t>(w.base) + seg * w.stride;
        PartRes x;
        const bool fast = w.sum && (walk_sum_seen(w.sum) & kSumFast);
        walk_lane(w, tab, seg, sb, r.start, pend < limit ? pend : limit, x,
                  TableSink{w.entries + slot, slot < w.cap ? w.cap - slot : 0, uint32_t(seg),
                            w.sum ? &hard : nullptr, fast ? &w : nullptr, slot},
                  chase ? (1u << w.pshift) : pre);
    }
    if (w.sum) {
        const uint32_t hw = (__ballot(hard & 1u) ? 1u : 0u) | (__ballot(hard & 2u) ? 2u : 0u) |
                           (__ballot(hard & 4u) ? 4u : 0u) | (__ballot(hard & kHardFull) ? kHardFull : 0u);
        if (hw && (threadIdx.x & (kWaveSize - 1)) == 0 && (hw & ~walk_sum_seen(w.sum)))
            atomicOr(w.sum, hw);
    }
}

static_assert(kPartRec == kWaveSize, "k_walk_copy: one lane per record of a block");

#ifndef RAMCRC_COPY_U
#define RAMCRC_COPY_U 4
#endif
constexpr int kCopyU = RAMCRC_COPY_U;
__global__ __launch_bounds__(256) void k_walk_copy(PWalk w0)
{
    const PWalk w = walk_geo(w0);
    const uint64_t nfirst = w.nseg * w.nparts;
    const uint64_t used = *w.pool_used;
    const uint64_t nblk = nfirst + (used < w.pool_cap ? used : w.pool_cap);
    const uint64_t nwave = uint64_t(gridDim.x) * (blockDim.x / kWaveSize);
    const uint32_t lane = threadIdx.x & (kWaveSize - 1);
    const uint32_t seen = walk_sum_seen(w.sum);
    if (w.sum && (seen & kSumFast))
        return;
    uint32_t hard = 0;
    for (uint64_t b0 = (uint64_t(blockIdx.x) * (blockDim.x / kWaveSize) +
                        __builtin_amdgcn_readfirstlane(threadIdx.x / kWaveSize)) * kCopyU;
         b0 < nblk; b0 += nwave * kCopyU) {
        uint64_t part[kCopyU];
        uint32_t blk[kCopyU];
        uint2 v[kCopyU];
#pragma unroll
        for (int u = 0; u < kCopyU; u++) {
            const uint64_t bi = b0 + u;
            blk[u] = ~0u;
            part[u] = 0;
            if (bi < nfirst) {
                part[u] = bi;
                blk[u] = 0;
                v[u] = w.recs[bi * kPartRec + lane];
            } else if (bi < nblk) {
                const uint32_t own = w.pool_owner[bi - nfirst];
                v[u] = w.pool[(bi - nfirst) * kPartRec + lane];
                if (own != 0xFFFFFFFFu) {
                    part[u] = own / 16;
                    blk[u] = own % 16;
                }
            }
        }
        PartRes r[kCopyU];
#pragma unroll
        for (int u = 0; u < kCopyU; u++)
            if (blk[u] != ~0u)
                r[u] = w.parts[part[u]];
        uint32_t fb[kCopyU];
        uint64_t sbase[kCopyU];
#pragma unroll
        for (int u = 0; u < kCopyU; u++) {
            const uint32_t fl = r[u].flags;
            if (blk[u] != ~0u && (!(fl & kPartEmit) || (fl & (kPartChase | kPartSpill))))
                blk[u] = ~0u;
            if (blk[u] != ~0u) {
                const uint64_t seg = part[u] / w.nparts;
                fb[u] = w.fallback[seg];
                sbase[u] = w.seg_base[seg];
            }
        }
#pragma unroll
        for (int u = 0; u < kCopyU; u++) {
            if (blk[u] == ~0u || fb[u])
                continue;
            const uint32_t n = r[u].count - r[u].pre;
            const uint32_t ri = blk[u] * kPartRec + lane;
            if (ri < r[u].cut || ri - r[u].cut >= n)
                continue;
            const uint64_t dst = sbase[u] + r[u].rec + r[u].pre + (ri - r[u].cut);
            if (dst < w.cap) {
                const u32x4 rec = {uint32_t(part[u] / w.nparts), v[u].x, v[u].y >> 8, v[u].y & 0xFF};
                __builtin_nontemporal_store(rec, &w.entries[dst]);
                hard |= (seen & kHardAll) != kHardAll ? replay_hard(v[u].x, v[u].y >> 8, v[u].y & 0xFF) : 0u;
            }
        }
    }
    {
        const uint32_t hw = (__ballot(hard & 1u) ? 1u : 0u) | (__ballot(hard & 2u) ? 2u : 0u) |
                           (__ballot(hard & 4u) ? 4u : 0u);
        if ((hw & ~seen) && lane == 0)
            atomicOr(w.sum, hw);
    }
}


constexpr int kVWaves = 4;
constexpr uint32_t kVStageS = 8192, kVStageL = 12288;

__device__ __forceinline__ uint32_t crc_lds(const uint8_t* st, const uint32_t* tx4, const uint32_t* tx1,
                                            uint32_t o, uint32_t n)
{
    uint32_t c = 0xFFFFFFFFu;
    while (n && (o & 3)) {
        c = tx1[(c ^ st[o]) & 0xFF] ^ (c >> 8);
        o++;
        n--;
    }
    const uint32_t* s32 = reinterpret_cast<const uint32_t*>(st);
    auto step4 = [&](uint32_t v) {
        v ^= c;
        c = xor3(tx4[v & 0xFF], tx4[256 + ((v >> 8) & 0xFF)], tx4[512 + ((v >> 16) & 0xFF)]) ^
            tx4[768 + (v >> 24)];
    };
    for (; n >= 16; o += 16, n -= 16) {
        const uint32_t a = s32[o >> 2], b = s32[(o >> 2) + 1], e = s32[(o >> 2) + 2], f = s32[(o >> 2) + 3];
        step4(a);
        step4(b);
        step4(e);
        step4(f);
    }
    for (; n >= 4; o += 4, n -= 4)
        step4(s32[o >> 2]);
    while (n) {
        c = tx1[(c ^ st[o]) & 0xFF] ^ (c >> 8);
        o++;
        n--;
    }
    return ~c;
}


template <uint32_t kVStage>
__global__ __launch_bounds__(kVWaves * kWaveSize) void k_walk_copyv(PWalk w0)
{
    constexpr uint32_t kVLoads = kVStage / 1024;
    const PWalk w = walk_geo(w0);
    const uint32_t seen = walk_sum_seen(w.sum);
    if (!w.sum || !(seen & kSumFast))
        return;
    if (bool(seen & kSumStage8) != (kVStage == kVStageS))
        return;
    __shared__ uint32_t tx4[4 * 256];
    __shared__ uint32_t tx1[256];
    __shared__ __attribute__((aligned(16))) uint8_t stage[kVWaves][kVStage];
    for (uint32_t t = threadIdx.x; t < 4 * 256; t += blockDim.x)
        tx4[t] = g_tab.comb[0].t[t >> 8][t & 0xFF];
    for (uint32_t t = threadIdx.x; t < 256; t += blockDim.x)
        tx1[t] = g_tab.t0.t[t];
    __syncthreads();
    const uint32_t lane = threadIdx.x & (kWaveSize - 1);
    const uint32_t wv = __builtin_amdgcn_readfirstlane(threadIdx.x / kWaveSize);
    const uint64_t nwave = uint64_t(gridDim.x) * kVWaves;
    const uint64_t nall = w.nseg * w.nparts;
    uint8_t* st = stage[wv];
    uint32_t hard = 0;
    for (uint64_t p = uint64_t(blockIdx.x) * kVWaves + wv; p < nall; p += nwave) {
        const PartRes r = w.parts[p];
        if (!(r.flags & kPartEmit) || (r.flags & (kPartChase | kPartSpill)))
            continue;
        const uint64_t seg = p / w.nparts;
        if (w.fallback[seg])
            continue;
        const uint32_t n = r.count - r.pre;
        if (n == 0)
            continue;
        const uint64_t sbase = w.seg_base[seg] + r.rec + r.pre;
        const uint32_t sflags = w.status[seg].flags;
        const uint64_t sb = reinterpret_cast<uint64_t>(w.base) + seg * w.stride;
        const uint32_t b0 = r.cut / kPartRec, b1 = (r.cut + n - 1) / kPartRec;
        const uint32_t bidx = b1 > 0 && lane < kMaxBlocks ? w.blocks[p * kMaxBlocks + lane] : 0u;
        auto recs_of = [&](uint32_t b) -> uint2 {
            if (b > b1)
                return make_uint2(0u, 0u);
            if (b == 0)
                return w.recs[p * kPartRec + lane];
            const uint32_t k = uint32_t(__shfl(int(bidx), int(b - 1), kWaveSize));
            return w.pool[uint64_t(k) * kPartRec + lane];
        };
        struct Lane {
            u32x4 rec;
            uint64_t dst;
            uint32_t pl;
            bool valid, todo;
        };
        auto lane_of = [&](uint32_t b, uint2 v) -> Lane {
            Lane L;
            const uint32_t ri = b * kPartRec + lane;
            L.rec = u32x4{uint32_t(seg), v.x, v.y >> 8, v.y & 0xFF};
            L.dst = sbase + (ri - r.cut);
            L.valid = b <= b1 && ri >= r.cut && ri - r.cut < n && L.dst < w.cap;
            L.todo = L.valid && !replay_other(L.rec) && (L.rec.w & 0x3f) == RAMCRC_LOG_ENTRY_TYPE_OBJ &&
                     L.rec.z >= kObjHeaderBytes && !(L.rec.w & kRecOverlong) && (sflags & RAMCRC_SEG_OK);
            L.pl = L.rec.y + 1 + ((L.rec.w >> 6) & 3) + 1;
            return L;
        };
        auto base_of = [&](const Lane& L, uint32_t& units) -> uint32_t {
            uint32_t lo = L.todo ? L.pl : 0xFFFFFFFFu, hi = L.todo ? L.pl + L.rec.z : 0u;
#pragma unroll
            for (int s2 = 1; s2 < kWaveSize; s2 <<= 1) {
                lo = min(lo, uint32_t(__shfl_xor(int(lo), s2, kWaveSize)));
                hi = max(hi, uint32_t(__shfl_xor(int(hi), s2, kWaveSize)));
            }
            const uint32_t base = lo & ~15u;
            units = hi > base ? min((hi - base + 1023) / 1024, kVLoads) : 0u;
            return base;
        };
        auto issue = [&](uint32_t base, uint32_t units, u32x4 (&t)[kVLoads]) {
#pragma unroll
            for (uint32_t u = 0; u < kVLoads; u++) {
                const uint64_t a = uint64_t(base) + u * 1024 + lane * 16;
                if (u < units)
                    t[u] = a + 16 <= w.capacity ? load16(sb + a) : u32x4{0u, 0u, 0u, 0u};
            }
        };
        Lane cur = lane_of(b0, recs_of(b0));
        uint2 vn = recs_of(b0 + 1);
        uint32_t units = 0;
        uint32_t base = base_of(cur, units);
        u32x4 t[kVLoads];
        issue(base, units, t);
        for (uint32_t b = b0; b <= b1; b++) {
#pragma unroll
            for (uint32_t u = 0; u < kVLoads; u++)
                if (u < units)
                    *reinterpret_cast<u32x4*>(st + u * 1024 + lane * 16) = t[u];
            const Lane nxt = lane_of(b + 1, vn);
            uint32_t nunits = 0;
            const uint32_t nbase = base_of(nxt, nunits);
            if (b + 1 <= b1)
                issue(nbase, nunits, t);
            vn = recs_of(b + 2);
            asm volatile("s_waitcnt lgkmcnt(0)" ::: "memory");
            if (cur.valid) {
                __builtin_nontemporal_store(cur.rec, &w.entries[cur.dst]);
                hard |= (seen & kHardAll) != kHardAll ? replay_hard(cur.rec.y, cur.rec.z, cur.rec.w) : 0u;
                if (replay_other(cur.rec))
                    hard |= left_append(w, cur.dst, cur.rec.z, cur.rec.w);
            }
            if (cur.todo) {
                if (uint64_t(cur.pl) + cur.rec.z <= uint64_t(base) + kVStage) {
                    const uint32_t o = cur.pl - base;
                    const uint32_t crc = crc_lds(st, tx4, tx1, o + 4, cur.rec.z - 4);
                    const uint32_t stored = uint32_t(st[o]) | (uint32_t(st[o + 1]) << 8) |
                                            (uint32_t(st[o + 2]) << 16) | (uint32_t(st[o + 3]) << 24);
                    w.obj_crc[cur.dst] = crc;
                    if (crc != stored)
                        atomicAdd(&w.status[seg].bad_objects, 1u);
                } else {
                    hard |= left_append(w, cur.dst, cur.rec.z, cur.rec.w);
                }
            }
            cur = nxt;
            base = nbase;
            units = nunits;
        }
    }
    const uint32_t hw = (__ballot(hard & 1u) ? 1u : 0u) | (__ballot(hard & 2u) ? 2u : 0u) |
                       (__ballot(hard & 4u) ? 4u : 0u) | (__ballot(hard & kHardFull) ? kHardFull : 0u);
    if ((hw & ~seen) && lane == 0)
        atomicOr(w.sum, hw);
}

}
```

### ramcloud_amd/csrc/ramcrc_device.hip

```cpp
#include <hip/hip_runtime.h>
#include <hip/hip_ext.h>

#include <mutex>
#include <new>
#include <utility>
#include <vector>
#include <stdio.h>
#include <string.h>

#include "gf2.h"
#include "walk_rules.h"
#include "murmur3.h"
#include "partition_rules.h"
#include "lookup_rules.h"
#include "resolve_rules.h"
#include "sidelog_rules.h"
#include "ramcrc.h"

namespace {

using namespace ramcrc_walk;

using ramcrc::OpTable;

}

#include "dev_common.inc"
#include "dev_chunks.inc"
#include "dev_bins.inc"
#include "dev_entries.inc"
#include "dev_plan.inc"
#include "dev_host.inc"
#include "dev_walk.inc"
#include "dev_checks.inc"
#include "dev_append.inc"
#include "dev_sidelog.inc"
#include "dev_partition.inc"
#include "dev_resolve.inc"
#include "dev_replay_table.inc"

extern "C" {

int ramcrc_device_count(void)
{
    int n = 0;
    if (hipGetDeviceCount(&n) != hipSuccess)
        return 0;
    return n;
}

int ramcrc_last_hip_error(void) { return t_last_hip; }

const char* ramcrc_strerror(int code)
{
    switch (code) {
    case RAMCRC_OK: return "ok";
    case RAMCRC_EINVAL: return "invalid argument";
    case RAMCRC_ENOMEM: return "out of memory";
    case RAMCRC_EHIP: return hipGetErrorString(hipError_t(t_last_hip));
    case RAMCRC_ENODEV: return "no usable device";
    case RAMCRC_ERCCL: return "rccl failure";
    case RAMCRC_EREFUSED: return "launch refused: chunk scratch too small (ramcrc_ctx_reserve), or a placement list refused";
    case RAMCRC_EINTERNAL: return "launch refused: inconsistent small-entry bin layout";
    case RAMCRC_EPEER: return "another rank of the shard failed this step";
    default: return "unknown error";
    }
}

#ifndef RAMCRC_SRC_SHA
#define RAMCRC_SRC_SHA "unknown"
#endif
#ifndef RAMCRC_DEFINES
#define RAMCRC_DEFINES "none"
#endif
#define RAMCRC_STR2(x) #x
#define RAMCRC_STR(x) RAMCRC_STR2(x)

int ramcrc_debug_stamps(void* out, uint64_t bytes)
{
#if RAMCRC_STAMPS
    if (bytes > sizeof(g_stamps))
        bytes = sizeof(g_stamps);
    return hipMemcpyFromSymbol(out, HIP_SYMBOL(g_stamps), bytes) == hipSuccess ? RAMCRC_OK : RAMCRC_EHIP;
#else
    (void)out;
    (void)bytes;
    return RAMCRC_EINVAL;
#endif
}

const char* ramcrc_build_info(void)
{
    return "ramcrc gfx950 src_sha=" RAMCRC_SRC_SHA
           " chunk=" RAMCRC_STR(RAMCRC_CHUNK_SHIFT) "..20 (adaptive: largest giving every wave two chunks)"
           " block=1KiB waves/WG=16 unroll=" RAMCRC_STR(RAMCRC_UNROLL)
           " lds_chunks=" RAMCRC_STR(RAMCRC_LDS_CHUNKS) " lds_entries=" RAMCRC_STR(RAMCRC_LDS_ENTRIES)
           " entries: waves=" RAMCRC_STR(RAMCRC_ENT_WAVES) " smallk=" RAMCRC_STR(RAMCRC_SMALLK)
           " pu=" RAMCRC_STR(RAMCRC_PU)
           " large_min=64KiB part_shift=" RAMCRC_STR(RAMCRC_PART_SHIFT)
           " defines=" RAMCRC_DEFINES;
}

int ramcrc_ctx_create(int device, ramcrc_ctx** out)
{
    if (!out)
        return RAMCRC_EINVAL;
    *out = nullptr;
    int ndev = 0;
    if (hipGetDeviceCount(&ndev) != hipSuccess || device < 0 || device >= ndev)
        return RAMCRC_ENODEV;
    DeviceGuard g(device);
    if (!g.ok)
        return RAMCRC_ENODEV;
    hipDeviceProp_t prop;
    HIPCHK(hipGetDeviceProperties(&prop, device));
    if (strncmp(prop.gcnArchName, "gfx950", 6) != 0) {
        fprintf(stderr, "ramcrc: device %d is %s, this build targets gfx950 only\n", device,
                prop.gcnArchName);
        return RAMCRC_ENODEV;
    }
    ramcrc_ctx* c = new (std::nothrow) ramcrc_ctx();
    if (!c)
        return RAMCRC_ENOMEM;
    c->device = device;
    c->ncu = prop.multiProcessorCount;
    c->ncu_all = c->ncu;
    if (hipMalloc(reinterpret_cast<void**>(&c->status), 16) != hipSuccess) {
        delete c;
        return RAMCRC_ENOMEM;
    }
    (void)hipMemset(c->status, 0, 16);
    if (hipMalloc(reinterpret_cast<void**>(&c->bins), sizeof(BinTable)) != hipSuccess) {
        ramcrc_ctx_destroy(c);
        return RAMCRC_ENOMEM;
    }
    (void)hipMemset(c->bins, 0, sizeof(BinTable));
    *out = c;
    return RAMCRC_OK;
}

int ramcrc_ctx_destroy(ramcrc_ctx* c)
{
    if (!c)
        return RAMCRC_OK;
    DeviceGuard g(c->device);
    (void)hipDeviceSynchronize();
    if (c->partials) (void)hipFree(c->partials);
    if (c->plan_local) (void)hipFree(c->plan_local);
    if (c->group_pref) (void)hipFree(c->group_pref);
    if (c->status) (void)hipFree(c->status);
    if (c->bins) (void)hipFree(c->bins);
    if (c->sdesc) (void)hipFree(c->sdesc);
    if (c->sidx) (void)hipFree(c->sidx);
    if (c->sinit) (void)hipFree(c->sinit);
    if (c->obj_out) (void)hipFree(c->obj_out);
    if (c->cert_scratch) (void)hipFree(c->cert_scratch);
    if (c->walk_parts) (void)hipFree(c->walk_parts);
    if (c->walk_fallback) (void)hipFree(c->walk_fallback);
    if (c->walk_base) (void)hipFree(c->walk_base);
    if (c->walk_recs) (void)hipFree(c->walk_recs);
    if (c->walk_pool) (void)hipFree(c->walk_pool);
    if (c->walk_pool_owner) (void)hipFree(c->walk_pool_owner);
    if (c->walk_blocks) (void)hipFree(c->walk_blocks);
    if (c->walk_pool_used) (void)hipFree(c->walk_pool_used);
    if (c->walk_sum) (void)hipFree(c->walk_sum);
    if (c->walk_left) (void)hipFree(c->walk_left);
    if (c->d_stage) (void)hipFree(c->d_stage);
    if (c->h_stage) (void)hipHostFree(c->h_stage);
    if (c->copy_stream) (void)hipStreamDestroy(c->copy_stream);
    if (c->compute_stream) (void)hipStreamDestroy(c->compute_stream);
    for (auto& ev : c->ev_used) {
        (void)hipEventDestroy(ev.first);
        (void)hipEventDestroy(ev.second);
    }
    for (auto& ev : c->ev_free) {
        (void)hipEventDestroy(ev.first);
        (void)hipEventDestroy(ev.second);
    }
    delete c;
    return RAMCRC_OK;
}

int ramcrc_ctx_reserve(ramcrc_ctx* c, uint64_t max_chunks, uint64_t max_entries)
{
    if (!c)
        return RAMCRC_EINVAL;
    std::lock_guard<std::recursive_mutex> lk(c->mu);
    DeviceGuard g(c->device);
    return reserve_locked(c, max_chunks, max_entries);
}

int ramcrc_ctx_set_option(ramcrc_ctx* c, int option, int64_t value)
{
    if (!c)
        return RAMCRC_EINVAL;
    std::lock_guard<std::recursive_mutex> lk(c->mu);
    switch (option) {
    case RAMCRC_OPT_SERIAL_WALK: c->serial_walk = value != 0; return RAMCRC_OK;
    case RAMCRC_OPT_TEST_FAIL_AFTER_COUNT:
        if (value < 0 || value > 1000)
            return RAMCRC_EINVAL;
        c->fail_after_count = int(value);
        return RAMCRC_OK;
    case RAMCRC_OPT_TEST_DIRTY_BINS:
        if (value < 0 || value > 0xFFFFFFFFll)
            return RAMCRC_EINVAL;
        c->dirty_bins = uint32_t(value);
        return RAMCRC_OK;
    case RAMCRC_OPT_TEST_BIN_STRAGGLER:
        c->bin_straggler = value != 0;
        return RAMCRC_OK;
    case RAMCRC_OPT_BIN_ONE:
        c->bin_one = value != 0;
        return RAMCRC_OK;
    case RAMCRC_OPT_VERIFY_IN_WALK:
        if (value < 0 || value > 2)
            return RAMCRC_EINVAL;
        c->verify_in_walk = int(value);
        return RAMCRC_OK;
    case RAMCRC_OPT_WALK_PART_SHIFT:
        if (value != 0 && (value < kPartShiftMin || value > 20))
            return RAMCRC_EINVAL;
        c->walk_pshift = uint32_t(value);
        return RAMCRC_OK;
    default: return RAMCRC_EINVAL;
    }
}

int ramcrc_ctx_set_timing(ramcrc_ctx* c, int enable)
{
    if (!c)
        return RAMCRC_EINVAL;
    std::lock_guard<std::recursive_mutex> lk(c->mu);
    c->timing = enable != 0;
    return RAMCRC_OK;
}

int ramcrc_stream_create_cu_mask(int device, const uint32_t* cu_mask, uint32_t mask_words,
                                 void** out_stream)
{
    if (!cu_mask || !out_stream || mask_words == 0 || mask_words > 8)
        return RAMCRC_EINVAL;
    DeviceGuard g(device);
    if (!g.ok)
        return RAMCRC_ENODEV;
    hipStream_t st = nullptr;
    HIPCHK(hipExtStreamCreateWithCUMask(&st, mask_words, cu_mask));
    *out_stream = st;
    return RAMCRC_OK;
}

int ramcrc_stream_destroy(void* stream)
{
    if (!stream)
        return RAMCRC_EINVAL;
    HIPCHK(hipStreamDestroy(reinterpret_cast<hipStream_t>(stream)));
    return RAMCRC_OK;
}

int ramcrc_ctx_set_cus(ramcrc_ctx* c, int ncu)
{
    if (!c || ncu < 0)
        return RAMCRC_EINVAL;
    std::lock_guard<std::recursive_mutex> lk(c->mu);
    if (ncu == 0 || ncu > c->ncu_all)
        ncu = c->ncu_all;
    c->ncu = ncu;
    return RAMCRC_OK;
}

int ramcrc_ctx_scan_time(ramcrc_ctx* c, double* total_ms, uint64_t* launches)
{
    if (!c)
        return RAMCRC_EINVAL;
    std::lock_guard<std::recursive_mutex> lk(c->mu);
    DeviceGuard g(c->device);
    double sum = 0;
    uint64_t cnt = 0;
    for (auto& ev : c->ev_used) {
        HIPCHK(hipEventSynchronize(ev.second));
        float ms = 0;
        HIPCHK(hipEventElapsedTime(&ms, ev.first, ev.second));
        sum += ms;
        cnt++;
        c->ev_free.push_back(ev);
    }
    c->ev_used.clear();
    if (total_ms)
        *total_ms = sum;
    if (launches)
        *launches = cnt;
    return RAMCRC_OK;
}

int ramcrc_ctx_debug_bins(ramcrc_ctx* c, uint64_t* host, uint64_t nwords, uint32_t* par_next)
{
    if (!c || !host)
        return RAMCRC_EINVAL;
    std::lock_guard<std::recursive_mutex> lk(c->mu);
    DeviceGuard g(c->device);
    HIPCHK(hipDeviceSynchronize());
    std::vector<uint64_t> v;
    BinTable h;
    HIPCHK(hipMemcpy(&h, c->bins, sizeof(BinTable), hipMemcpyDeviceToHost));
    for (int b = 0; b < kNB; b++) v.push_back(h.count[b]);
    for (int p = 0; p < 2; p++)
        for (int b = 0; b < kNB; b++) v.push_back(h.ctr[p].cursor[b]);
    for (int p = 0; p < 2; p++)
        for (int b = 0; b < kNB; b++) v.push_back(h.ctr[p].hist[b]);
    v.push_back(h.rescues);
    for (uint64_t i = 0; i < nwords && i < v.size(); i++)
        host[i] = v[i];
    if (par_next)
        *par_next = c->bin_par;
    return RAMCRC_OK;
}

int ramcrc_ctx_status(ramcrc_ctx* c, uint32_t* status)
{
    if (!c || !status)
        return RAMCRC_EINVAL;
    DeviceGuard g(c->device);
    HIPCHK(hipMemcpy(status, c->status, sizeof(uint32_t), hipMemcpyDeviceToHost));
    return RAMCRC_OK;
}

int ramcrc_ctx_check(ramcrc_ctx* c, void* stream)
{
    if (!c)
        return RAMCRC_EINVAL;
    std::lock_guard<std::recursive_mutex> lk(c->mu);
    DeviceGuard g(c->device);
    hipStream_t s = reinterpret_cast<hipStream_t>(stream);
    HIPCHK(hipStreamSynchronize(s));
    uint32_t st = 0;
    HIPCHK(hipMemcpy(&st, c->status, sizeof(uint32_t), hipMemcpyDeviceToHost));
    if (!(st & kStatusSticky))
        return RAMCRC_OK;
    hipLaunchKernelGGL(k_status_take, dim3(1), dim3(1), 0, s, c->status);
    HIPCHK(hipGetLastError());
    HIPCHK(hipStreamSynchronize(s));
    HIPCHK(hipMemcpy(&st, c->status + 1, sizeof(uint32_t), hipMemcpyDeviceToHost));
    if (st & kStatusBins)
        return RAMCRC_EINTERNAL;
    return (st & kStatusSticky) ? RAMCRC_EREFUSED : RAMCRC_OK;
}

int ramcrc_segments_device(ramcrc_ctx* c, const void* d_base, uint64_t seg_bytes, uint64_t nseg,
                           const uint32_t* d_init, uint32_t* d_out, uint32_t flags, void* stream)
{
    if (!c || !d_out || (!d_base && nseg && seg_bytes) || (flags & ~RAMCRC_FINALIZE))
        return RAMCRC_EINVAL;
    if (nseg == 0)
        return RAMCRC_OK;
    std::lock_guard<std::recursive_mutex> lk(c->mu);
    DeviceGuard g(c->device);
    hipStream_t s = reinterpret_cast<hipStream_t>(stream);
    BatchDesc d{};
    d.cshift = kChunkShift;
    d.base = static_cast<const uint8_t*>(d_base);
    d.seg_bytes = seg_bytes;
    d.n = nseg;
    d.init = d_init;
    d.out = d_out;
    d.flags = flags;
    if (seg_bytes < kLargeMin) {
        return launch_binned<kSegUniform>(c, d, s, 0);
    }
    const uint64_t B = reinterpret_cast<uint64_t>(d_base);
    if ((B % kChunk) == 0 && (seg_bytes % kChunk) == 0) {
        const uint64_t waves = uint64_t(c->ncu) * kWavesPerGroup;
        uint32_t shift = kChunkShift;
        while (shift < 20 && (B % (2ull << shift)) == 0 && (seg_bytes % (2ull << shift)) == 0 &&
               (seg_bytes >> (shift + 1)) * nseg >= 2 * waves)
            shift++;
        d.cshift = shift;
        const uint64_t per = seg_bytes >> shift;
        int rc = reserve_locked(c, per * nseg, 1);
        if (rc)
            return rc;
        Plan pl = make_plan(c, 0);
        {
            ScanTimer t(c, s);
            t.launch(k_chunks<kSegAligned>, dim3(c->ncu), dim3(kThreads), d, pl, per);
        }
        HIPCHK(hipGetLastError());
        hipLaunchKernelGGL((k_combine<kSegAligned, false>), dim3((nseg + 3) / 4), dim3(256), 0, s,
                           d, pl, per);
        HIPCHK(hipGetLastError());
        return RAMCRC_OK;
    }
    int rc = reserve_locked(c, nseg * (seg_bytes / kChunk + 2) + 16, nseg);
    if (rc)
        return rc;
    return launch_planned<kSegUniform>(c, d, s);
}

int ramcrc_batch_device(ramcrc_ctx* c, const void* d_base, const uint64_t* d_off,
                        const uint64_t* d_len, const uint32_t* d_init, uint32_t* d_out, uint64_t n,
                        uint32_t flags, void* stream)
{
    if (flags & ~RAMCRC_FINALIZE)
        return RAMCRC_EINVAL;
    if (n == 0)
        return c ? RAMCRC_OK : RAMCRC_EINVAL;
    if (!c || !d_out || !d_off || !d_len || !d_base)
        return RAMCRC_EINVAL;
    std::lock_guard<std::recursive_mutex> lk(c->mu);
    DeviceGuard g(c->device);
    int rc = reserve_locked(c, default_chunk_bound(n), n);
    if (rc)
        return rc;
    BatchDesc d{};
    d.cshift = kChunkShift;
    d.base = static_cast<const uint8_t*>(d_base);
    d.off = d_off;
    d.len = d_len;
    d.n = n;
    d.init = d_init;
    d.out = d_out;
    d.flags = flags;
    return launch_planned<kTable>(c, d, reinterpret_cast<hipStream_t>(stream));
}

int ramcrc_entries_device(ramcrc_ctx* c, const void* d_base, const uint64_t* d_off,
                          const uint64_t* d_len, const uint32_t* d_init, uint32_t* d_out, uint64_t n,
                          uint32_t flags, void* stream)
{
    if (flags & ~RAMCRC_FINALIZE)
        return RAMCRC_EINVAL;
    if (n == 0)
        return c ? RAMCRC_OK : RAMCRC_EINVAL;
    if (!c || !d_out || !d_off || !d_len || !d_base)
        return RAMCRC_EINVAL;
    std::lock_guard<std::recursive_mutex> lk(c->mu);
    DeviceGuard g(c->device);
    hipStream_t s = reinterpret_cast<hipStream_t>(stream);
    BatchDesc d{};
    d.cshift = kChunkShift;
    d.base = static_cast<const uint8_t*>(d_base);
    d.off = d_off;
    d.len = d_len;
    d.n = n;
    d.init = d_init;
    d.out = d_out;
    d.flags = flags;
    return launch_binned<kTable>(c, d, s, 0);
}

int ramcrc_batch_host(ramcrc_ctx* c, const void* const* ptrs, const uint64_t* lens,
                      const uint32_t* init, uint32_t* out, uint64_t n, uint32_t flags)
{
    if (!c || (n && (!ptrs || !lens || !out)) || (flags & ~RAMCRC_FINALIZE))
        return RAMCRC_EINVAL;
    if (n == 0)
        return RAMCRC_OK;
    std::lock_guard<std::recursive_mutex> lk(c->mu);
    DeviceGuard g(c->device);
    uint64_t total = 0;
    for (uint64_t i = 0; i < n; i++) {
        if (lens[i] && !ptrs[i])
            return RAMCRC_EINVAL;
        total += (lens[i] + 15) & ~uint64_t(15);
    }
    const uint64_t meta = n * (2 * sizeof(uint64_t) + 2 * sizeof(uint32_t));
    const uint64_t need = total + meta + 64;
    if (c->h_stage_cap < need) {
        if (c->h_stage) (void)hipHostFree(c->h_stage);
        c->h_stage = nullptr;
        c->h_stage_cap = 0;
        if (hipHostMalloc(reinterpret_cast<void**>(&c->h_stage), need, hipHostMallocDefault) !=
            hipSuccess)
            return RAMCRC_ENOMEM;
        c->h_stage_cap = need;
    }
    if (c->d_stage_cap < need) {
        if (c->d_stage) (void)hipFree(c->d_stage);
        c->d_stage = nullptr;
        c->d_stage_cap = 0;
        if (hipMalloc(reinterpret_cast<void**>(&c->d_stage), need) != hipSuccess)
            return RAMCRC_ENOMEM;
        c->d_stage_cap = need;
    }
    if (!c->copy_stream)
        HIPCHK(hipStreamCreateWithFlags(&c->copy_stream, hipStreamNonBlocking));
    uint8_t* h = c->h_stage;
    uint64_t* h_off = reinterpret_cast<uint64_t*>(h + total);
    uint64_t* h_len = h_off + n;
    uint32_t* h_init = reinterpret_cast<uint32_t*>(h_len + n);
    uint32_t* h_out = h_init + n;
    uint64_t pos = 0;
    for (uint64_t i = 0; i < n; i++) {
        if (lens[i])
            memcpy(h + pos, ptrs[i], lens[i]);
        h_off[i] = pos;
        h_len[i] = lens[i];
        h_init[i] = init ? init[i] : 0xFFFFFFFFu;
        pos += (lens[i] + 15) & ~uint64_t(15);
    }
    uint8_t* d = c->d_stage;
    hipStream_t s = c->copy_stream;
    const uint64_t in_bytes = total + n * (2 * sizeof(uint64_t) + sizeof(uint32_t));
    HIPCHK(hipMemcpyAsync(d, h, in_bytes, hipMemcpyHostToDevice, s));
    uint64_t* d_off = reinterpret_cast<uint64_t*>(d + total);
    uint64_t* d_len = d_off + n;
    uint32_t* d_init = reinterpret_cast<uint32_t*>(d_len + n);
    uint32_t* d_out = d_init + n;
    int rc = ramcrc_batch_device(c, d, d_off, d_len, d_init, d_out, n, flags, s);
    if (rc) {
        (void)hipStreamSynchronize(s);
        return rc;
    }
    HIPCHK(hipMemcpyAsync(h_out, d_out, n * sizeof(uint32_t), hipMemcpyDeviceToHost, s));
    rc = ramcrc_ctx_check(c, s);
    if (rc)
        return rc;
    memcpy(out, h_out, n * sizeof(uint32_t));
    return RAMCRC_OK;
}

int ramcrc_stream_host(ramcrc_ctx* c, const void* h_base, uint64_t seg_bytes, uint64_t nseg,
                       uint32_t* h_out, uint32_t flags, int batch, int depth)
{
    if (!c || !h_base || !h_out || batch < 1 || depth < 1 || seg_bytes == 0 ||
        (flags & ~RAMCRC_FINALIZE))
        return RAMCRC_EINVAL;
    if (nseg == 0)
        return RAMCRC_OK;
    std::lock_guard<std::recursive_mutex> lk(c->mu);
    DeviceGuard g(c->device);
    if (depth > 8)
        depth = 8;
    const uint64_t slot_bytes = uint64_t(batch) * seg_bytes;
    const uint64_t slot_stride = (slot_bytes + 4 * uint64_t(batch) + 4095) & ~uint64_t(4095);
    const uint64_t need = slot_stride * uint64_t(depth);
    if (c->d_stage_cap < need) {
        if (c->d_stage) (void)hipFree(c->d_stage);
        c->d_stage = nullptr;
        c->d_stage_cap = 0;
        if (hipMalloc(reinterpret_cast<void**>(&c->d_stage), need) != hipSuccess)
            return RAMCRC_ENOMEM;
        c->d_stage_cap = need;
    }
    if (!c->copy_stream)
        HIPCHK(hipStreamCreateWithFlags(&c->copy_stream, hipStreamNonBlocking));
    if (!c->compute_stream)
        HIPCHK(hipStreamCreateWithFlags(&c->compute_stream, hipStreamNonBlocking));
    hipEvent_t copied[8] = {}, done[8] = {};
    int rc = RAMCRC_OK;
    auto hip = [&](hipError_t e) {
        if (e != hipSuccess && rc == RAMCRC_OK) {
            t_last_hip = int(e);
            rc = RAMCRC_EHIP;
        }
        return rc == RAMCRC_OK;
    };
    for (int k = 0; k < depth && rc == RAMCRC_OK; k++) {
        hip(hipEventCreateWithFlags(&copied[k], hipEventDisableTiming));
        hip(hipEventCreateWithFlags(&done[k], hipEventDisableTiming));
    }
    const uint8_t* src = static_cast<const uint8_t*>(h_base);
    const uint64_t nb = (nseg + batch - 1) / batch;
    for (uint64_t b = 0; b < nb && rc == RAMCRC_OK; b++) {
        const int k = int(b % depth);
        const uint64_t first = b * batch;
        const uint64_t cnt = (nseg - first) < uint64_t(batch) ? (nseg - first) : uint64_t(batch);
        uint8_t* slot = c->d_stage + uint64_t(k) * slot_stride;
        uint32_t* slot_out = reinterpret_cast<uint32_t*>(slot + slot_bytes);
        if (b >= uint64_t(depth) && !hip(hipStreamWaitEvent(c->copy_stream, done[k], 0)))
            break;
        if (!hip(hipMemcpyAsync(slot, src + first * seg_bytes, cnt * seg_bytes,
                                hipMemcpyHostToDevice, c->copy_stream)) ||
            !hip(hipEventRecord(copied[k], c->copy_stream)) ||
            !hip(hipStreamWaitEvent(c->compute_stream, copied[k], 0)))
            break;
        rc = ramcrc_segments_device(c, slot, seg_bytes, cnt, nullptr, slot_out, flags,
                                    c->compute_stream);
        if (rc)
            break;
        if (!hip(hipMemcpyAsync(h_out + first, slot_out, cnt * sizeof(uint32_t),
                                hipMemcpyDeviceToHost, c->compute_stream)) ||
            !hip(hipEventRecord(done[k], c->compute_stream)))
            break;
    }
    hip(hipStreamSynchronize(c->compute_stream));
    hip(hipStreamSynchronize(c->copy_stream));
    for (int k = 0; k < depth; k++) {
        if (copied[k]) (void)hipEventDestroy(copied[k]);
        if (done[k]) (void)hipEventDestroy(done[k]);
    }
    return rc;
}


namespace {
int walk_impl(ramcrc_ctx* c, const void* d_base, uint64_t seg_stride, uint32_t seg_capacity,
              uint64_t n_seg, const ramcrc_seg_cert* d_certs, ramcrc_seg_status* d_status,
              ramcrc_seg_entry* d_entries, uint64_t entries_cap, uint64_t* d_n_entries,
              hipStream_t s, uint32_t* sum, uint32_t* d_obj_crc = nullptr);
int verify_impl(ramcrc_ctx* c, const void* d_base, uint64_t seg_stride,
                const ramcrc_seg_entry* d_entries, uint64_t entries_cap, const uint64_t* d_n_entries,
                uint32_t* d_obj_crc, ramcrc_seg_status* d_status, hipStream_t s, const uint32_t* sum,
                uint64_t n_seg = 0);
}

int ramcrc_segment_walk_device(ramcrc_ctx* c, const void* d_base, uint64_t seg_stride,
                               uint32_t seg_capacity, uint64_t n_seg,
                               const ramcrc_seg_cert* d_certs, ramcrc_seg_status* d_status,
                               ramcrc_seg_entry* d_entries, uint64_t entries_cap,
                               uint64_t* d_n_entries, void* stream)
{
    if (!c)
        return RAMCRC_EINVAL;
    std::lock_guard<std::recursive_mutex> lk(c->mu);
    DeviceGuard g(c->device);
    return walk_impl(c, d_base, seg_stride, seg_capacity, n_seg, d_certs, d_status, d_entries,
                     entries_cap, d_n_entries, reinterpret_cast<hipStream_t>(stream), nullptr);
}

int ramcrc_replay_verify_device(ramcrc_ctx* c, const void* d_base, uint64_t seg_stride,
                                uint32_t seg_capacity, uint64_t n_seg, const ramcrc_seg_cert* d_certs,
                                ramcrc_seg_status* d_status, ramcrc_seg_entry* d_entries,
                                uint64_t entries_cap, uint64_t* d_n_entries, uint32_t* d_obj_crc,
                                void* stream)
{
    if (!c)
        return RAMCRC_EINVAL;
    if (entries_cap && !d_obj_crc)
        return RAMCRC_EINVAL;
    std::lock_guard<std::recursive_mutex> lk(c->mu);
    DeviceGuard g(c->device);
    hipStream_t s = reinterpret_cast<hipStream_t>(stream);
    int rc = grow_device(reinterpret_cast<void**>(&c->walk_sum), &c->walk_sum_cap, 4, sizeof(uint32_t));
    if (rc)
        return rc;
    rc = walk_impl(c, d_base, seg_stride, seg_capacity, n_seg, d_certs, d_status, d_entries,
                   entries_cap, d_n_entries, s, c->walk_sum,
                   entries_cap && c->verify_in_walk ? d_obj_crc : nullptr);
    if (rc || n_seg == 0)
        return rc;
    return verify_impl(c, d_base, seg_stride, d_entries, entries_cap, d_n_entries, d_obj_crc,
                       d_status, s, c->walk_sum, n_seg);
}

namespace {
int walk_impl(ramcrc_ctx* c, const void* d_base, uint64_t seg_stride, uint32_t seg_capacity,
              uint64_t n_seg, const ramcrc_seg_cert* d_certs, ramcrc_seg_status* d_status,
              ramcrc_seg_entry* d_entries, uint64_t entries_cap, uint64_t* d_n_entries,
              hipStream_t s, uint32_t* sum, uint32_t* d_obj_crc)
{
    if (!d_n_entries || (entries_cap && !d_entries))
        return RAMCRC_EINVAL;
    if (n_seg && (!d_base || !d_certs || !d_status))
        return RAMCRC_EINVAL;
    if ((reinterpret_cast<uintptr_t>(d_base) & 15) || (seg_stride & 15) || (seg_capacity & 15) ||
        n_seg > 0xFFFFFFFFull || (n_seg > 1 && seg_stride < seg_capacity))
        return RAMCRC_EINVAL;
    if (n_seg == 0 || c->serial_walk) {
        HIPCHK(hipMemsetAsync(d_n_entries, 0, sizeof(uint64_t), s));
        if (sum)
            HIPCHK(hipMemsetAsync(sum, 0, sizeof(uint32_t), s));
    }
    if (n_seg == 0)
        return RAMCRC_OK;
    WalkDesc w{};
    w.base = static_cast<const uint8_t*>(d_base);
    w.stride = seg_stride;
    w.capacity = seg_capacity;
    w.nseg = n_seg;
    w.certs = d_certs;
    w.status = d_status;
    w.entries = reinterpret_cast<u32x4*>(d_entries);
    w.cap = entries_cap;
    w.n_entries = reinterpret_cast<unsigned long long*>(d_n_entries);
    w.only = nullptr;
    w.sum = sum;
    {
        int rc0 = grow_device(reinterpret_cast<void**>(&c->walk_base), &c->walk_base_cap, n_seg,
                              sizeof(uint64_t));
        if (rc0)
            return rc0;
    }
    w.seg_base = c->walk_base;
    uint64_t grid = n_seg;
    if (grid > uint64_t(64) * c->ncu)
        grid = uint64_t(64) * c->ncu;
    if (!c->serial_walk) {
        const uint32_t pshift = c->walk_pshift ? c->walk_pshift : kPartShiftLow;
        const uint32_t nparts = uint32_t((uint64_t(seg_capacity) + (1ull << pshift) - 1) >> pshift);
        const uint64_t total = n_seg * uint64_t(nparts);
        int rc = grow_device(&c->walk_parts, &c->walk_parts_cap, total, sizeof(PartRes));
        if (!rc)
            rc = grow_device(reinterpret_cast<void**>(&c->walk_fallback), &c->walk_fallback_cap,
                             n_seg, sizeof(uint32_t));
        if (!rc)
            rc = grow_device(&c->walk_recs, &c->walk_recs_cap, total * kPartRec, sizeof(uint2));
        uint64_t pool_blocks = (n_seg * uint64_t(seg_capacity) / 96) / kPartRec + 1;
        const uint64_t cap_blocks = entries_cap / kPartRec + 1;
        pool_blocks = pool_blocks < cap_blocks ? pool_blocks : cap_blocks;
        if (!rc)
            rc = grow_device(&c->walk_pool, &c->walk_pool_cap, pool_blocks * kPartRec, sizeof(uint2));
        if (!rc)
            rc = grow_device(reinterpret_cast<void**>(&c->walk_pool_owner), &c->walk_pool_owner_cap,
                             pool_blocks, sizeof(uint32_t));
        if (!rc)
            rc = grow_device(reinterpret_cast<void**>(&c->walk_blocks), &c->walk_blocks_cap,
                             total * kMaxBlocks, sizeof(uint32_t));
        if (!rc)
            rc = grow_device(reinterpret_cast<void**>(&c->walk_pool_used), &c->walk_pool_used_cap, 3,
                             sizeof(unsigned long long));
        const uint64_t left_cap = entries_cap / 8 + 65536 < entries_cap ? entries_cap / 8 + 65536 : entries_cap;
        if (!rc && d_obj_crc && sum)
            rc = grow_device(reinterpret_cast<void**>(&c->walk_left), &c->walk_left_cap, left_cap,
                             sizeof(uint32_t));
        if (rc)
            return rc;
        PWalk pw{};
        pw.base = w.base;
        pw.stride = seg_stride;
        pw.capacity = seg_capacity;
        pw.nparts = nparts;
        pw.nseg = n_seg;
        pw.certs = d_certs;
        pw.status = d_status;
        pw.entries = w.entries;
        pw.cap = entries_cap;
        pw.n_entries = w.n_entries;
        pw.parts = static_cast<PartRes*>(c->walk_parts);
        pw.fallback = c->walk_fallback;
        pw.seg_base = c->walk_base;
        pw.recs = static_cast<uint2*>(c->walk_recs);
        pw.pshift = pshift;
        uint32_t* geo = reinterpret_cast<uint32_t*>(c->walk_pool_used + 1);
        pw.geo = geo;
        pw.pool = static_cast<uint2*>(c->walk_pool);
        pw.pool_owner = c->walk_pool_owner;
        pw.blocks = c->walk_blocks;
        pw.pool_used = c->walk_pool_used;
        pw.pool_cap = pool_blocks;
        pw.sum = sum;
        if (d_obj_crc && sum) {
            pw.obj_crc = d_obj_crc;
            pw.left = c->walk_left;
            pw.nleft = c->walk_pool_used + 2;
            pw.left_cap = left_cap;
            pw.vmode = uint32_t(c->verify_in_walk);
        }
        HIPCHK(hipMemsetAsync(c->walk_blocks, 0xFF, total * kMaxBlocks * sizeof(uint32_t), s));
        HIPCHK(hipMemsetAsync(c->walk_pool_owner, 0xFF, pool_blocks * sizeof(uint32_t), s));
        hipLaunchKernelGGL(k_walk_probe, dim3(1), dim3(kWaveSize), 0, s, pw, c->walk_pshift, geo);
        HIPCHK(hipGetLastError());
        if (nparts > 1) {
            uint64_t g0 = (total + kSyncWaves - 1) / kSyncWaves;
            if (g0 > uint64_t(8) * c->ncu)
                g0 = uint64_t(8) * c->ncu;
            hipLaunchKernelGGL(k_walk_sync, dim3(g0), dim3(kSyncWaves * kWaveSize), 0, s, pw);
            HIPCHK(hipGetLastError());
        }
        hipLaunchKernelGGL(k_walk_parts, dim3((total + 255) / 256), dim3(256), 0, s, pw);
        HIPCHK(hipGetLastError());
        hipLaunchKernelGGL(k_walk_fix, dim3(grid), dim3(kWaveSize), 0, s, pw);
        HIPCHK(hipGetLastError());
        hipLaunchKernelGGL(k_walk_emit, dim3((total + 255) / 256), dim3(256), 0, s, pw);
        HIPCHK(hipGetLastError());
        uint64_t gc = (total + pool_blocks + 4 * kCopyU - 1) / (4 * kCopyU);
        if (gc > uint64_t(32) * c->ncu)
            gc = uint64_t(32) * c->ncu;
        hipLaunchKernelGGL(k_walk_copy, dim3(gc), dim3(256), 0, s, pw);
        HIPCHK(hipGetLastError());
        if (pw.obj_crc) {
            uint64_t gv = (total + kVWaves - 1) / kVWaves;
            if (gv > uint64_t(16) * c->ncu)
                gv = uint64_t(16) * c->ncu;
            {
                ScanTimer t(c, s);
                t.launch(k_walk_copyv<kVStageS>, dim3(gv), dim3(kVWaves * kWaveSize), pw);
            }
            HIPCHK(hipGetLastError());
            {
                ScanTimer t(c, s);
                t.launch(k_walk_copyv<kVStageL>, dim3(gv), dim3(kVWaves * kWaveSize), pw);
            }
            HIPCHK(hipGetLastError());
        }
        w.only = c->walk_fallback;
    }
    hipLaunchKernelGGL(k_seg_walk, dim3(grid), dim3(kWaveSize), 0, s, w);
    HIPCHK(hipGetLastError());
    return RAMCRC_OK;
}
}

int ramcrc_segments_certify_device(ramcrc_ctx* c, const void* d_base, uint64_t seg_stride,
                                   uint32_t seg_capacity, uint64_t n_seg, const uint32_t* d_heads,
                                   ramcrc_seg_cert* d_certs, uint32_t* d_flags, void* stream)
{
    if (!c)
        return RAMCRC_EINVAL;
    if (n_seg == 0)
        return RAMCRC_OK;
    if (!d_base || !d_heads || !d_certs || n_seg > 0xFFFFFFFFull)
        return RAMCRC_EINVAL;
    std::lock_guard<std::recursive_mutex> lk(c->mu);
    DeviceGuard g(c->device);
    hipStream_t s = reinterpret_cast<hipStream_t>(stream);
    const uint64_t need = n_seg * (sizeof(ramcrc_seg_cert) + sizeof(ramcrc_seg_status)) / 4 + 2;
    int rc = grow_device(reinterpret_cast<void**>(&c->cert_scratch), &c->cert_scratch_cap, need,
                         sizeof(uint32_t));
    if (rc)
        return rc;
    uint64_t* d_n = reinterpret_cast<uint64_t*>(c->cert_scratch);
    ramcrc_seg_cert* tmp = reinterpret_cast<ramcrc_seg_cert*>(c->cert_scratch + 2);
    ramcrc_seg_status* st = reinterpret_cast<ramcrc_seg_status*>(tmp + n_seg);
    const dim3 grid(uint32_t((n_seg + 255) / 256));
    hipLaunchKernelGGL(k_cert_prep, grid, dim3(256), 0, s, d_heads, tmp, n_seg);
    HIPCHK(hipGetLastError());
    rc = ramcrc_segment_walk_device(c, d_base, seg_stride, seg_capacity, n_seg, tmp, st, nullptr, 0,
                                    d_n, stream);
    if (rc)
        return rc;
    hipLaunchKernelGGL(k_cert_emit, grid, dim3(256), 0, s, tmp, st, d_certs, d_flags, n_seg);
    HIPCHK(hipGetLastError());
    return RAMCRC_OK;
}

namespace {
int app_launch(ramcrc_ctx* c, const void* d_base, uint64_t seg_stride, uint64_t n_seg,
               const ramcrc_seg_status* d_status, const ramcrc_seg_entry* d_entries,
               uint64_t entries_cap, const uint64_t* d_n_entries, const ramcrc_placement* d_place,
               uint64_t place_cap, const uint64_t* d_n_place, uint32_t n_part, void* d_out,
               uint64_t out_stride, uint32_t out_capacity, ramcrc_seg_cert* d_out_certs,
               ramcrc_append_status* d_out_status, SlDesc* sl, void* stream)
{
    if (!c || n_part == 0 || out_stride < out_capacity || n_seg > 0xFFFFFFFFull ||
        place_cap > 0xFFFFFFFFull)
        return RAMCRC_EINVAL;
    if (n_seg == 0)
        return RAMCRC_OK;
    if (!d_base || !d_status || !d_n_entries || !d_n_place || !d_out || !d_out_certs ||
        !d_out_status || (entries_cap && !d_entries) || (place_cap && !d_place))
        return RAMCRC_EINVAL;
    const uint64_t B = reinterpret_cast<uint64_t>(d_base), O = reinterpret_cast<uint64_t>(d_out);
    if ((B & 15) || (seg_stride & 15))
        return RAMCRC_EINVAL;
    const uint64_t n_out = n_seg * n_part;
    if ((seg_stride && n_seg > UINT64_MAX / seg_stride) ||
        (out_stride && n_out > UINT64_MAX / out_stride) || n_out > UINT64_MAX / sizeof(AppState))
        return RAMCRC_EINVAL;
    const uint64_t src_bytes = n_seg * seg_stride, out_bytes = n_out * out_stride;
    if (B > UINT64_MAX - src_bytes || O > UINT64_MAX - out_bytes ||
        (B < O + out_bytes && O < B + src_bytes))
        return RAMCRC_EINVAL;
    std::lock_guard<std::recursive_mutex> lk(c->mu);
    DeviceGuard g(c->device);
    hipStream_t s = reinterpret_cast<hipStream_t>(stream);
    const uint64_t head_words = (4 + 3 * n_seg + 3) & ~uint64_t(3);
    const uint64_t state_words = n_part > kAppLdsParts ? n_out * (sizeof(AppState) / 4) : 0;
    const uint64_t app_words = head_words + state_words;
    const uint64_t sl_at = (app_words + kSlCountWords - 1) / kSlCountWords * kSlCountWords;
    int rc = reserve_locked(c, sl ? sl_at + kSlCountWords : app_words, place_cap / 2 + 1);
    if (rc)
        return rc;
    AppDesc a{};
    a.base = B;
    a.stride = seg_stride;
    a.nseg = n_seg;
    a.status = d_status;
    a.entries = reinterpret_cast<const u32x4*>(d_entries);
    a.ecap = entries_cap;
    a.n_entries = d_n_entries;
    a.place = reinterpret_cast<const uint2*>(d_place);
    a.pcap = place_cap;
    a.n_place = d_n_place;
    a.npart = n_part;
    a.ocap = out_capacity;
    a.out = O;
    a.ostride = out_stride;
    a.certs = d_out_certs;
    a.ostat = d_out_status;
    a.refuse = c->partials;
    a.run_lo = c->partials + 4;
    a.run_hi = a.run_lo + n_seg;
    a.run_cnt = a.run_hi + n_seg;
    a.pdst = reinterpret_cast<uint32_t*>(c->plan_local);
    a.states = reinterpret_cast<AppState*>(c->partials + head_words);
    a.ctx_status = c->status;
    HIPCHK(hipMemsetAsync(c->partials, 0, head_words * sizeof(uint32_t), s));
    if (sl) {
        sl->counts = reinterpret_cast<unsigned long long*>(c->partials + sl_at);
        HIPCHK(hipMemsetAsync(sl->counts, 0, kSlCountWords * sizeof(uint32_t), s));
    }
    const uint64_t cap_grid = uint64_t(8) * c->ncu;
    uint64_t gm = (place_cap + 255) / 256;
    gm = gm < 1 ? 1 : (gm > cap_grid ? cap_grid : gm);
    hipLaunchKernelGGL(k_app_mark, dim3(uint32_t(gm)), dim3(256), 0, s, a);
    HIPCHK(hipGetLastError());
    uint32_t nown = 1;
    while (nown < 8 && 2 * nown <= n_part && n_seg * (2 * nown) <= uint64_t(16) * c->ncu)
        nown *= 2;
    a.nown = nown;
    const uint64_t gs = n_seg * nown < uint64_t(16) * c->ncu ? n_seg * nown : uint64_t(16) * c->ncu;
    if (n_part <= kAppLdsParts)
        hipLaunchKernelGGL(k_app_scan<true>, dim3(uint32_t(gs)), dim3(kWaveSize), 0, s, a);
    else
        hipLaunchKernelGGL(k_app_scan<false>, dim3(uint32_t(gs)), dim3(kWaveSize), 0, s, a);
    HIPCHK(hipGetLastError());
    if (place_cap) {
        uint64_t gc = (place_cap + kAppCopyThreads - 1) / kAppCopyThreads;
        gc = gc > cap_grid ? cap_grid : gc;
        hipLaunchKernelGGL(k_app_copy, dim3(uint32_t(gc)), dim3(kAppCopyThreads), 0, s, a);
        HIPCHK(hipGetLastError());
    }
    if (sl) {
        uint64_t gt = (place_cap + kSlThreads - 1) / kSlThreads;
        gt = gt < 1 ? 1 : (gt > cap_grid ? cap_grid : gt);
        hipLaunchKernelGGL(k_sl_stamp, dim3(uint32_t(gt)), dim3(kSlThreads), 0, s, a, *sl);
        HIPCHK(hipGetLastError());
    }
    return RAMCRC_OK;
}
}

int ramcrc_recovery_append_device(ramcrc_ctx* c, const void* d_base, uint64_t seg_stride,
                                  uint64_t n_seg, const ramcrc_seg_status* d_status,
                                  const ramcrc_seg_entry* d_entries, uint64_t entries_cap,
                                  const uint64_t* d_n_entries, const ramcrc_placement* d_place,
                                  uint64_t place_cap, const uint64_t* d_n_place, uint32_t n_part,
                                  void* d_out, uint64_t out_stride, uint32_t out_capacity,
                                  ramcrc_seg_cert* d_out_certs, ramcrc_append_status* d_out_status,
                                  void* stream)
{
    return app_launch(c, d_base, seg_stride, n_seg, d_status, d_entries, entries_cap, d_n_entries,
                      d_place, place_cap, d_n_place, n_part, d_out, out_stride, out_capacity,
                      d_out_certs, d_out_status, nullptr, stream);
}

int ramcrc_replay_sidelog_device(ramcrc_ctx* c, const void* d_base, uint64_t seg_stride,
                                 uint64_t n_seg, const ramcrc_seg_status* d_status,
                                 const ramcrc_seg_entry* d_entries, uint64_t entries_cap,
                                 const uint64_t* d_n_entries, const ramcrc_placement* d_live,
                                 uint64_t live_cap, const uint64_t* d_n_live, uint32_t timestamp,
                                 void* d_out, uint64_t out_stride, uint32_t out_capacity,
                                 ramcrc_seg_cert* d_out_certs, ramcrc_append_status* d_out_status,
                                 ramcrc_log_ref* d_refs, ramcrc_sidelog_counts* d_counts,
                                 void* stream)
{
    if (!d_counts)
        return RAMCRC_EINVAL;
    SlDesc sl{};
    sl.refs = reinterpret_cast<uint2*>(d_refs);
    sl.counts_out = d_counts;
    sl.timestamp = timestamp;
    return app_launch(c, d_base, seg_stride, n_seg, d_status, d_entries, entries_cap, d_n_entries,
                      d_live, live_cap, d_n_live, 1, d_out, out_stride, out_capacity, d_out_certs,
                      d_out_status, &sl, stream);
}

int ramcrc_recovery_partition_device(ramcrc_ctx* c, const void* d_base, uint64_t seg_stride,
                                     uint64_t n_seg, const ramcrc_seg_status* d_status,
                                     const ramcrc_seg_entry* d_entries, uint64_t entries_cap,
                                     const uint64_t* d_n_entries, const ramcrc_tablet* d_tablets,
                                     uint32_t n_tablets, uint32_t n_part,
                                     ramcrc_placement* d_place, uint64_t place_cap,
                                     uint64_t* d_n_place, uint64_t* d_key_hash,
                                     ramcrc_partition_status* d_part_status, void* stream)
{
    if (!c || n_seg >= 0xFFFFFFFFull || entries_cap >= 0xFFFFFFFFull || place_cap >= 0xFFFFFFFFull)
        return RAMCRC_EINVAL;
    if (!d_n_place || !d_n_entries || (n_seg && (!d_base || !d_status || !d_part_status)) ||
        (entries_cap && !d_entries) || (place_cap && !d_place) || (n_tablets && !d_tablets))
        return RAMCRC_EINVAL;
    const uint64_t B = reinterpret_cast<uint64_t>(d_base);
    if ((B & 15) || (seg_stride & 15) || (seg_stride && n_seg > UINT64_MAX / seg_stride))
        return RAMCRC_EINVAL;
    std::lock_guard<std::recursive_mutex> lk(c->mu);
    DeviceGuard g(c->device);
    hipStream_t s = reinterpret_cast<hipStream_t>(stream);
    const uint64_t head_words = 4 + 9 * n_seg;
    int rc = reserve_locked(c, head_words, entries_cap);
    if (rc)
        return rc;
    PartDesc a{};
    a.base = B;
    a.stride = seg_stride;
    a.nseg = n_seg;
    a.status = d_status;
    a.entries = reinterpret_cast<const u32x4*>(d_entries);
    a.ecap = entries_cap;
    a.n_entries = d_n_entries;
    a.tablets = d_tablets;
    a.ntab = n_tablets;
    a.npart = n_part;
    a.place = reinterpret_cast<uint2*>(d_place);
    a.pcap = place_cap;
    a.n_place = d_n_place;
    a.key_hash = d_key_hash;
    a.pstat = d_part_status;
    a.refuse = c->partials;
    a.run_lo = c->partials + 4;
    a.run_hi = a.run_lo + n_seg;
    a.run_cnt = a.run_hi + n_seg;
    a.hdr_cnt = a.run_cnt + n_seg;
    a.hdr_first = a.hdr_cnt + n_seg;
    a.sflags = a.hdr_first + n_seg;
    a.counts = a.sflags + n_seg;
    a.cls = c->plan_local;
    a.tile_sum = c->group_pref;
    a.ctx_status = c->status;
    HIPCHK(hipMemsetAsync(c->partials, 0, head_words * sizeof(uint32_t), s));
    const uint64_t cap_grid = uint64_t(8) * c->ncu;
    auto grid_of = [&](uint64_t items, uint64_t per) {
        uint64_t gr = (items + per - 1) / per;
        return dim3(uint32_t(gr < 1 ? 1 : (gr > cap_grid ? cap_grid : gr)));
    };
    const uint64_t heads_items = entries_cap > n_tablets ? entries_cap : n_tablets;
    hipLaunchKernelGGL(k_part_heads, grid_of(heads_items, kPartThreads), dim3(kPartThreads), 0, s, a);
    HIPCHK(hipGetLastError());
    if (n_tablets <= kPartLdsTablets)
        hipLaunchKernelGGL(k_part_classify<true>, grid_of(entries_cap, kPartThreads),
                           dim3(kPartThreads), 0, s, a);
    else
        hipLaunchKernelGGL(k_part_classify<false>, grid_of(entries_cap, kPartThreads),
                           dim3(kPartThreads), 0, s, a);
    HIPCHK(hipGetLastError());
    hipLaunchKernelGGL(k_part_void, grid_of(n_seg, 1), dim3(kWaveSize), 0, s, a);
    HIPCHK(hipGetLastError());
    hipLaunchKernelGGL(k_part_tiles, grid_of(entries_cap, kPartTile), dim3(kPartThreads), 0, s, a);
    HIPCHK(hipGetLastError());
    hipLaunchKernelGGL(k_part_scan, dim3(1), dim3(kPartThreads), 0, s, a);
    HIPCHK(hipGetLastError());
    hipLaunchKernelGGL(k_part_emit, grid_of(entries_cap, kPartTile), dim3(kPartThreads), 0, s, a);
    HIPCHK(hipGetLastError());
    return RAMCRC_OK;
}

int ramcrc_replay_resolve_device(ramcrc_ctx* c, const void* d_base, uint64_t seg_stride,
                                 uint64_t n_seg, const ramcrc_seg_status* d_status,
                                 const ramcrc_seg_entry* d_entries, uint64_t entries_cap,
                                 const uint64_t* d_n_entries, const uint64_t* d_key_hash,
                                 uint32_t* d_winner, ramcrc_placement* d_live, uint64_t live_cap,
                                 uint64_t* d_n_live, ramcrc_resolve_counts* d_counts, void* stream)
{
    if (!c || n_seg >= 0xFFFFFFFFull || entries_cap >= 0xFFFFFFFFull || live_cap >= 0xFFFFFFFFull)
        return RAMCRC_EINVAL;
    if (!d_n_live || !d_counts || !d_n_entries || (n_seg && (!d_base || !d_status)) ||
        (entries_cap && !d_entries) || (live_cap && !d_live))
        return RAMCRC_EINVAL;
    const uint64_t B = reinterpret_cast<uint64_t>(d_base);
    if ((B & 15) || (seg_stride & 15) || (seg_stride && n_seg > UINT64_MAX / seg_stride))
        return RAMCRC_EINVAL;
    std::lock_guard<std::recursive_mutex> lk(c->mu);
    DeviceGuard g(c->device);
    hipStream_t s = reinterpret_cast<hipStream_t>(stream);
    const uint64_t slots = ramcrc_res::slots_for(entries_cap);
    int rc = reserve_locked(c, kResHeadWords + 2 * kResSlotWords * slots, 2 * entries_cap);
    if (rc)
        return rc;
    ResDesc a{};
    a.base = B;
    a.stride = seg_stride;
    a.nseg = n_seg;
    a.status = d_status;
    a.entries = reinterpret_cast<const u32x4*>(d_entries);
    a.ecap = entries_cap;
    a.n_entries = d_n_entries;
    a.key_hash = d_key_hash;
    a.winner = d_winner;
    a.live = reinterpret_cast<uint2*>(d_live);
    a.lcap = live_cap;
    a.n_live = d_n_live;
    a.counts_out = d_counts;
    a.refuse = c->partials;
    a.counts = reinterpret_cast<unsigned long long*>(c->partials + 4);
    a.slots = reinterpret_cast<unsigned long long*>(c->partials + kResHeadWords);
    a.rec_ver = c->plan_local;
    a.rec_slot = c->plan_local + entries_cap;
    a.tile_sum = c->group_pref;
    a.ctx_status = c->status;
    HIPCHK(hipMemsetAsync(c->partials, 0, kResHeadWords * sizeof(uint32_t), s));
    const uint64_t cap_grid = uint64_t(8) * c->ncu;
    auto grid_of = [&](uint64_t items, uint64_t per) {
        uint64_t gr = (items + per - 1) / per;
        return dim3(uint32_t(gr < 1 ? 1 : (gr > cap_grid ? cap_grid : gr)));
    };
    hipLaunchKernelGGL(k_res_zero, grid_of(kResSlotWords * slots, kPartThreads), dim3(kPartThreads), 0, s, a);
    HIPCHK(hipGetLastError());
    if (d_key_hash)
        hipLaunchKernelGGL(k_res_insert<true>, grid_of(entries_cap, kPartThreads), dim3(kPartThreads),
                           0, s, a);
    else
        hipLaunchKernelGGL(k_res_insert<false>, grid_of(entries_cap, kPartThreads), dim3(kPartThreads),
                           0, s, a);
    HIPCHK(hipGetLastError());
    hipLaunchKernelGGL(k_res_pick, grid_of(entries_cap, kPartThreads), dim3(kPartThreads), 0, s, a);
    HIPCHK(hipGetLastError());
    hipLaunchKernelGGL(k_res_tiles, grid_of(entries_cap, kPartTile), dim3(kPartThreads), 0, s, a);
    HIPCHK(hipGetLastError());
    hipLaunchKernelGGL(k_res_scan, dim3(1), dim3(kPartThreads), 0, s, a);
    HIPCHK(hipGetLastError());
    hipLaunchKernelGGL(k_res_emit, grid_of(entries_cap, kPartTile), dim3(kPartThreads), 0, s, a);
    HIPCHK(hipGetLastError());
    return RAMCRC_OK;
}

struct ramcrc_replay_table {
    ramcrc_ctx* ctx = nullptr;
    std::mutex mu;
    unsigned long long* mem = nullptr;
    uint64_t key_cap = 0, nslots = 0;
    uint32_t max_batches = 0;
    std::vector<uint64_t> ecap;
};

namespace {
RtabDesc rtab_desc(const ramcrc_replay_table* t)
{
    RtabDesc a{};
    a.head = t->mem;
    a.batches = reinterpret_cast<RtabBatch*>(t->mem + kRtabHeadWords);
    a.bcount = reinterpret_cast<RtabCount*>(a.batches + t->max_batches);
    a.slots = reinterpret_cast<unsigned long long*>(a.bcount + t->max_batches);
    a.nslots = t->nslots;
    a.key_cap = t->key_cap;
    a.n_batches = uint32_t(t->ecap.size());
    a.ctx_status = t->ctx->status;
    return a;
}

uint32_t rtab_grid(const ramcrc_ctx* c, uint64_t items, uint64_t per)
{
    const uint64_t cap_grid = uint64_t(8) * c->ncu;
    const uint64_t gr = (items + per - 1) / per;
    return uint32_t(gr < 1 ? 1 : (gr > cap_grid ? cap_grid : gr));
}
}

int ramcrc_replay_table_create(ramcrc_ctx* c, uint64_t key_cap, uint32_t max_batches,
                               ramcrc_replay_table** out)
{
    if (!out)
        return RAMCRC_EINVAL;
    *out = nullptr;
    if (!c || key_cap >= 0xFFFFFFFFull || max_batches == 0 || max_batches > RAMCRC_REPLAY_TABLE_MAX_BATCHES)
        return RAMCRC_EINVAL;
    std::lock_guard<std::recursive_mutex> lk(c->mu);
    DeviceGuard g(c->device);
    ramcrc_replay_table* t = new (std::nothrow) ramcrc_replay_table();
    if (!t)
        return RAMCRC_ENOMEM;
    t->ctx = c;
    t->key_cap = key_cap;
    t->nslots = ramcrc_res::slots_for(key_cap);
    t->max_batches = max_batches;
    const uint64_t words =
        kRtabHeadWords + ((sizeof(RtabBatch) + sizeof(RtabCount)) / 8) * max_batches +
        kRtabSlotWords * t->nslots;
    if (hipMalloc(reinterpret_cast<void**>(&t->mem), words * 8) != hipSuccess) {
        delete t;
        return RAMCRC_ENOMEM;
    }
    if (hipMemset(t->mem, 0, words * 8) != hipSuccess) {
        (void)hipFree(t->mem);
        delete t;
        return RAMCRC_EHIP;
    }
    *out = t;
    return RAMCRC_OK;
}

int ramcrc_replay_table_destroy(ramcrc_replay_table* t)
{
    if (!t)
        return RAMCRC_OK;
    {
        DeviceGuard g(t->ctx->device);
        (void)hipDeviceSynchronize();
        (void)hipFree(t->mem);
    }
    delete t;
    return RAMCRC_OK;
}

int ramcrc_replay_table_reset(ramcrc_replay_table* t, void* stream)
{
    if (!t)
        return RAMCRC_EINVAL;
    std::lock_guard<std::mutex> lt(t->mu);
    ramcrc_ctx* c = t->ctx;
    std::lock_guard<std::recursive_mutex> lk(c->mu);
    DeviceGuard g(c->device);
    const RtabDesc a = rtab_desc(t);
    hipLaunchKernelGGL(k_rtab_zero, dim3(rtab_grid(c, kRtabSlotWords * t->nslots, kPartThreads)),
                       dim3(kPartThreads), 0, reinterpret_cast<hipStream_t>(stream), a);
    HIPCHK(hipGetLastError());
    t->ecap.clear();
    return RAMCRC_OK;
}

int ramcrc_replay_table_add_device(ramcrc_replay_table* t, const void* d_base, uint64_t seg_stride,
                                   uint64_t n_seg, const ramcrc_seg_status* d_status,
                                   const ramcrc_seg_entry* d_entries, uint64_t entries_cap,
                                   const uint64_t* d_n_entries, const uint64_t* d_key_hash,
                                   uint64_t* d_work, uint32_t* batch, void* stream)
{
    if (!t || n_seg >= 0xFFFFFFFFull || entries_cap >= 0xFFFFFFFFull)
        return RAMCRC_EINVAL;
    if (!d_n_entries || (n_seg && (!d_base || !d_status)) ||
        (entries_cap && (!d_entries || !d_work)))
        return RAMCRC_EINVAL;
    const uint64_t B = reinterpret_cast<uint64_t>(d_base);
    if ((B & 15) || (seg_stride & 15) || (seg_stride && n_seg > UINT64_MAX / seg_stride))
        return RAMCRC_EINVAL;
    std::lock_guard<std::mutex> lt(t->mu);
    if (t->ecap.size() >= t->max_batches)
        return RAMCRC_EINVAL;
    ramcrc_ctx* c = t->ctx;
    std::lock_guard<std::recursive_mutex> lk(c->mu);
    DeviceGuard g(c->device);
    hipStream_t s = reinterpret_cast<hipStream_t>(stream);
    RtabDesc a = rtab_desc(t);
    a.batch = uint32_t(t->ecap.size());
    a.open.base = B;
    a.open.stride = seg_stride;
    a.open.nseg = n_seg;
    a.open.status = d_status;
    a.open.entries = reinterpret_cast<const u32x4*>(d_entries);
    a.open.n_entries = d_n_entries;
    a.open.ecap = entries_cap;
    a.open.key_hash = d_key_hash;
    a.open.work = d_work;
    hipLaunchKernelGGL(k_rtab_open, dim3(1), dim3(kWaveSize), 0, s, a);
    HIPCHK(hipGetLastError());
    t->ecap.push_back(entries_cap);
    if (batch)
        *batch = a.batch;
    const dim3 grid(rtab_grid(c, entries_cap, kPartThreads));
    if (d_key_hash)
        hipLaunchKernelGGL(k_rtab_insert<true>, grid, dim3(kPartThreads), 0, s, a);
    else
        hipLaunchKernelGGL(k_rtab_insert<false>, grid, dim3(kPartThreads), 0, s, a);
    HIPCHK(hipGetLastError());
    hipLaunchKernelGGL(k_rtab_pick, grid, dim3(kPartThreads), 0, s, a);
    HIPCHK(hipGetLastError());
    return RAMCRC_OK;
}

int ramcrc_replay_table_live_device(ramcrc_replay_table* t, uint32_t batch,
                                    ramcrc_replay_ref* d_winner, ramcrc_placement* d_live,
                                    uint64_t live_cap, uint64_t* d_n_live,
                                    ramcrc_resolve_counts* d_counts, void* stream)
{
    if (!t || !d_n_live || !d_counts || live_cap >= 0xFFFFFFFFull || (live_cap && !d_live))
        return RAMCRC_EINVAL;
    std::lock_guard<std::mutex> lt(t->mu);
    if (batch >= t->ecap.size())
        return RAMCRC_EINVAL;
    ramcrc_ctx* c = t->ctx;
    std::lock_guard<std::recursive_mutex> lk(c->mu);
    DeviceGuard g(c->device);
    hipStream_t s = reinterpret_cast<hipStream_t>(stream);
    const uint64_t ecap = t->ecap[batch];
    int rc = grow_device(reinterpret_cast<void**>(&c->group_pref), &c->group_cap,
                         (ecap + kThreads - 1) / kThreads + 1, sizeof(uint64_t));
    if (rc)
        return rc;
    RtabDesc a = rtab_desc(t);
    a.batch = batch;
    a.winner = reinterpret_cast<uint2*>(d_winner);
    a.live = reinterpret_cast<uint2*>(d_live);
    a.lcap = live_cap;
    a.n_live = d_n_live;
    a.counts_out = d_counts;
    a.tile_sum = c->group_pref;
    const dim3 grid(rtab_grid(c, ecap, kPartTile));
    hipLaunchKernelGGL(k_rtab_tiles, grid, dim3(kPartThreads), 0, s, a);
    HIPCHK(hipGetLastError());
    hipLaunchKernelGGL(k_rtab_scan, dim3(1), dim3(kPartThreads), 0, s, a);
    HIPCHK(hipGetLastError());
    hipLaunchKernelGGL(k_rtab_emit, grid, dim3(kPartThreads), 0, s, a);
    HIPCHK(hipGetLastError());
    return RAMCRC_OK;
}

int ramcrc_replay_table_stats_device(ramcrc_replay_table* t, ramcrc_replay_table_stats* d_stats,
                                     void* stream)
{
    if (!t || !d_stats)
        return RAMCRC_EINVAL;
    std::lock_guard<std::mutex> lt(t->mu);
    ramcrc_ctx* c = t->ctx;
    std::lock_guard<std::recursive_mutex> lk(c->mu);
    DeviceGuard g(c->device);
    hipStream_t s = reinterpret_cast<hipStream_t>(stream);
    RtabDesc a = rtab_desc(t);
    a.stats_out = d_stats;
    HIPCHK(hipMemsetAsync(d_stats, 0, sizeof(*d_stats), s));
    hipLaunchKernelGGL(k_rtab_stats, dim3(rtab_grid(c, t->nslots, kPartThreads)), dim3(kPartThreads),
                       0, s, a);
    HIPCHK(hipGetLastError());
    return RAMCRC_OK;
}

int ramcrc_replay_table_lookup_device(ramcrc_replay_table* t, const void* d_keys, uint64_t keys_bytes,
                                      const ramcrc_lookup_key* d_queries, uint64_t n_queries,
                                      const uint64_t* d_key_hash, ramcrc_lookup_result* d_results,
                                      ramcrc_lookup_counts* d_counts, void* stream)
{
    if (!t || n_queries >= 0xFFFFFFFFull || (n_queries && (!d_queries || !d_results)) ||
        (keys_bytes && !d_keys))
        return RAMCRC_EINVAL;
    const uint64_t K = reinterpret_cast<uint64_t>(d_keys);
    if ((reinterpret_cast<uint64_t>(d_queries) & 7) || (reinterpret_cast<uint64_t>(d_results) & 15) ||
        K > UINT64_MAX - keys_bytes)
        return RAMCRC_EINVAL;
    if (n_queries == 0 && !d_counts)
        return RAMCRC_OK;
    std::lock_guard<std::mutex> lt(t->mu);
    ramcrc_ctx* c = t->ctx;
    std::lock_guard<std::recursive_mutex> lk(c->mu);
    DeviceGuard g(c->device);
    hipStream_t s = reinterpret_cast<hipStream_t>(stream);
    int rc = reserve_locked(c, kLookCountWords, 0);
    if (rc)
        return rc;
    const RtabDesc a = rtab_desc(t);
    LookDesc q{};
    q.keys = K;
    q.keys_bytes = keys_bytes;
    q.queries = reinterpret_cast<const uint64_t*>(d_queries);
    q.nq = n_queries;
    q.key_hash = d_key_hash;
    q.results = reinterpret_cast<u32x4*>(d_results);
    q.counts_out = d_counts;
    q.counts = reinterpret_cast<unsigned long long*>(c->partials);
    if (d_counts)
        HIPCHK(hipMemsetAsync(q.counts, 0, kLookCountWords * sizeof(uint32_t), s));
    const dim3 grid(rtab_grid(c, n_queries, kPartThreads));
    if (d_key_hash)
        hipLaunchKernelGGL(k_rtab_lookup<true>, grid, dim3(kPartThreads), 0, s, a, q);
    else
        hipLaunchKernelGGL(k_rtab_lookup<false>, grid, dim3(kPartThreads), 0, s, a, q);
    HIPCHK(hipGetLastError());
    return RAMCRC_OK;
}

int ramcrc_verify_objects_device(ramcrc_ctx* c, const void* d_base, uint64_t seg_stride,
                                 const ramcrc_seg_entry* d_entries, uint64_t entries_cap,
                                 const uint64_t* d_n_entries, uint32_t* d_obj_crc,
                                 ramcrc_seg_status* d_status, void* stream)
{
    if (!c)
        return RAMCRC_EINVAL;
    std::lock_guard<std::recursive_mutex> lk(c->mu);
    DeviceGuard g(c->device);
    return verify_impl(c, d_base, seg_stride, d_entries, entries_cap, d_n_entries, d_obj_crc,
                       d_status, reinterpret_cast<hipStream_t>(stream), nullptr);
}

namespace {
int verify_impl(ramcrc_ctx* c, const void* d_base, uint64_t seg_stride,
                const ramcrc_seg_entry* d_entries, uint64_t entries_cap, const uint64_t* d_n_entries,
                uint32_t* d_obj_crc, ramcrc_seg_status* d_status, hipStream_t s, const uint32_t* sum,
                uint64_t n_seg)
{
    if (entries_cap == 0)
        return RAMCRC_OK;
    if (!d_base || !d_entries || !d_n_entries || !d_obj_crc || !d_status)
        return RAMCRC_EINVAL;
    int rc = reserve_locked(c, default_chunk_bound(entries_cap), entries_cap);
    if (rc)
        return rc;
    BatchDesc d{};
    d.cshift = kChunkShift;
    d.base = static_cast<const uint8_t*>(d_base);
    d.seg_bytes = seg_stride;
    d.n = entries_cap;
    d.vstat = d_status;
    d.rec = reinterpret_cast<const u32x4*>(d_entries);
    d.n_dev = d_n_entries;
    d.seg_status = reinterpret_cast<const u32x4*>(d_status);
    d.out = d_obj_crc;
    d.flags = RAMCRC_FINALIZE;
    if (sum && c->walk_left && !c->serial_walk) {
        uint64_t gl = uint64_t(4) * c->ncu;
        hipLaunchKernelGGL(k_left, dim3(gl), dim3(256), 0, s, d, d_status, sum, c->walk_left,
                           reinterpret_cast<const unsigned long long*>(c->walk_pool_used + 2),
                           c->walk_left_cap, n_seg);
        HIPCHK(hipGetLastError());
    }
    const uint32_t* nother = nullptr;
    rc = launch_planned<kRecords>(c, d, s, &nother, sum);
    if (rc)
        return rc;
    uint64_t grid = (entries_cap + 255) / 256;
    grid = grid < uint64_t(16) * c->ncu ? grid : uint64_t(16) * c->ncu;
    hipLaunchKernelGGL(k_obj_compare, dim3(grid), dim3(256), 0, s, d, d_status, nother);
    HIPCHK(hipGetLastError());
    return RAMCRC_OK;
}
}

int ramcrc_assemble_objects_device(ramcrc_ctx* c, void* d_base, const uint64_t* d_off,
                                   const uint64_t* d_len, uint32_t* d_out, uint64_t n,
                                   void* stream)
{
    if (n == 0)
        return c ? RAMCRC_OK : RAMCRC_EINVAL;
    if (!c || !d_base || !d_off || !d_len)
        return RAMCRC_EINVAL;
    std::lock_guard<std::recursive_mutex> lk(c->mu);
    DeviceGuard g(c->device);
    hipStream_t s = reinterpret_cast<hipStream_t>(stream);
    int rc = reserve_locked(c, default_chunk_bound(n), n);
    if (rc)
        return rc;
    if (!d_out) {
        rc = grow_device(reinterpret_cast<void**>(&c->obj_out), &c->obj_out_cap, n,
                         sizeof(uint32_t));
        if (rc)
            return rc;
        d_out = c->obj_out;
    }
    BatchDesc d{};
    d.cshift = kChunkShift;
    d.base = static_cast<const uint8_t*>(d_base);
    d.off = d_off;
    d.len = d_len;
    d.n = n;
    d.out = d_out;
    d.flags = RAMCRC_FINALIZE;
    rc = launch_planned<kObjects>(c, d, s);
    if (rc)
        return rc;
    hipLaunchKernelGGL(k_obj_stamp, dim3((n + 255) / 256), dim3(256), 0, s, d);
    HIPCHK(hipGetLastError());
    return RAMCRC_OK;
}

int ramcrc_assemble_objects_host(ramcrc_ctx* c, void* const* objs, const uint64_t* lens,
                                 uint64_t n)
{
    if (!c || (n && (!objs || !lens)))
        return RAMCRC_EINVAL;
    std::vector<const void*> ptrs;
    std::vector<uint64_t> ls;
    std::vector<uint64_t> which;
    for (uint64_t i = 0; i < n; i++) {
        if (lens[i] < kObjHeaderBytes)
            continue;
        if (!objs[i])
            return RAMCRC_EINVAL;
        ptrs.push_back(static_cast<const uint8_t*>(objs[i]) + 4);
        ls.push_back(lens[i] - 4);
        which.push_back(i);
    }
    if (ptrs.empty())
        return RAMCRC_OK;
    std::vector<uint32_t> out(ptrs.size());
    int rc = ramcrc_batch_host(c, ptrs.data(), ls.data(), nullptr, out.data(), ptrs.size(),
                               RAMCRC_FINALIZE);
    if (rc)
        return rc;
    for (size_t k = 0; k < which.size(); k++) {
        uint8_t* p = static_cast<uint8_t*>(objs[which[k]]);
        for (int b = 0; b < 4; b++)
            p[b] = uint8_t(out[k] >> (8 * b));
    }
    return RAMCRC_OK;
}

}
```

Measured before the change: 6890 GB/s.

## Fuse replay planning, combine, and leftover verification kernels to cut launches

Merges plan count and scan into one kernel that uses a last-block ticket, and folds the large-object combine, the leftover-record CRC and the object compare into a single replay-tail kernel. It also moves the parallel walker's map clear into the sync kernel instead of a separate memset, and runs the serial fallback walk inline inside the fix-up kernel rather than launching another walker. The aim is to remove several kernel launches, memsets and round-trips through global memory on the replay path. In exchange it adds grid-level ticket synchronisation and more complex control flow, with a risk of ordering or coherence bugs.

```diff
diff --git a/ramcloud_amd/csrc/dev_checks.inc b/ramcloud_amd/csrc/dev_checks.inc
--- a/ramcloud_amd/csrc/dev_checks.inc
+++ b/ramcloud_amd/csrc/dev_checks.inc
@@ -16,7 +16,7 @@
 
 
 __device__ __forceinline__ void obj_compare_one(const BatchDesc& d, ramcrc_seg_status* status,
-                                                uint64_t i);
+                                                uint64_t i, bool have = false, uint32_t val = 0);
 
 __global__ __launch_bounds__(256) void k_obj_compare(BatchDesc d, ramcrc_seg_status* status,
                                                      const uint32_t* nother)
@@ -30,7 +30,7 @@
 }
 
 __device__ __forceinline__ void obj_compare_one(const BatchDesc& d, ramcrc_seg_status* status,
-                                                uint64_t i)
+                                                uint64_t i, bool have, uint32_t val)
 {
     const u32x4 r = d.rec[i];
     const uint32_t type = r.w & 0x3f;
@@ -47,7 +47,7 @@
     uint32_t stored = 0, computed = 0;
     if (type == RAMCRC_LOG_ENTRY_TYPE_OBJ && readable) {
         stored = le32_g(p);
-        computed = d.out[i];
+        computed = have ? val : d.out[i];
     }
     if (!(seg_flags & RAMCRC_SEG_OK))
         return;
@@ -86,24 +86,15 @@
         atomicAdd(&status[r.x].bad_objects, 1u);
 }
 
-__global__ __launch_bounds__(256) void k_left(BatchDesc d, ramcrc_seg_status* status, const uint32_t* sum,
-                                              const uint32_t* left, const unsigned long long* nleft,
-                                              uint64_t left_cap, uint64_t nseg)
-{
-    const uint32_t sv = *sum;
-    if (!(sv & kSumFast))
-        return;
+__device__ __forceinline__ void left_records(const BatchDesc& d, ramcrc_seg_status* status,
+                                             const uint32_t* left, const unsigned long long* nleft,
+                                             uint64_t left_cap, uint32_t* tx4, uint32_t* tx1)
+{
     const uint64_t tid = uint64_t(blockIdx.x) * blockDim.x + threadIdx.x, nt = uint64_t(gridDim.x) * blockDim.x;
-    if (sv & kHardFull) {
-        for (uint64_t s = tid; s < nseg; s += nt)
-            status[s].bad_objects = 0;
-        return;
-    }
     const uint64_t nl = *nleft;
     const uint64_t n = nl < left_cap ? nl : left_cap;
     if (uint64_t(blockIdx.x) * blockDim.x >= n)
         return;
-    __shared__ uint32_t tx4[4 * 256], tx1[256];
     for (uint32_t t = threadIdx.x; t < 4 * 256; t += blockDim.x)
         tx4[t] = g_tab.comb[0].t[t >> 8][t & 0xFF];
     for (uint32_t t = threadIdx.x; t < 256; t += blockDim.x)
@@ -152,6 +143,47 @@
     }
 }
 
+__global__ __launch_bounds__(256) void k_replay_tail(BatchDesc d, Plan pl, ramcrc_seg_status* status,
+                                                     const uint32_t* sum, const uint32_t* nother,
+                                                     const uint32_t* left,
+                                                     const unsigned long long* nleft, uint64_t left_cap)
+{
+    __shared__ uint32_t tx4[4 * 256], tx1[256];
+    const uint32_t sv = *sum;
+    if ((sv & kSumFast) && !(sv & kHardFull)) {
+        left_records(d, status, left, nleft, left_cap, tx4, tx1);
+        return;
+    }
+    if (*nother == 0)
+        return;
+    const bool merge = !plan_empty(pl) && !((*pl.status) & kStatusRefused) &&
+                       pl.group_pref[pl.ngroups] != 0;
+    const int lane = threadIdx.x & (kWaveSize - 1);
+    const uint64_t wave = uint64_t(blockIdx.x) * (256 / kWaveSize) + threadIdx.x / kWaveSize;
+    const uint64_t nwave = uint64_t(gridDim.x) * (256 / kWaveSize);
+    const uint64_t n = entry_count<kRecords>(d);
+    for (uint64_t wv = wave; wv * kWaveSize < n; wv += nwave) {
+        const uint64_t i = wv * kWaveSize + lane;
+        bool big = false;
+        uint32_t crc = 0;
+        if (merge) {
+            uint64_t S = 0, E = 0;
+            big = i < n && buffer_range<kRecords>(d, i, S, E) && is_large(E - S);
+            uint64_t todo = __ballot(big);
+            while (todo) {
+                const int j = __builtin_ctzll(todo);
+                todo &= todo - 1;
+                const uint32_t v = combine_one<kRecords>(d, pl, 0, wv * kWaveSize + j, shfl64(S, j),
+                                                         shfl64(E, j), lane);
+                if (lane == j)
+                    crc = v;
+            }
+        }
+        if (i < n)
+            obj_compare_one(d, status, i, big, crc);
+    }
+}
+
 __global__ __launch_bounds__(256) void k_obj_stamp(BatchDesc d)
 {
     const uint64_t i = uint64_t(blockIdx.x) * blockDim.x + threadIdx.x;
diff --git a/ramcloud_amd/csrc/dev_chunks.inc b/ramcloud_amd/csrc/dev_chunks.inc
--- a/ramcloud_amd/csrc/dev_chunks.inc
+++ b/ramcloud_amd/csrc/dev_chunks.inc
@@ -186,7 +186,7 @@
 }
 
 template <int kMode>
-__device__ __forceinline__ void combine_one(const BatchDesc& d, const Plan& pl, uint64_t per_seg,
+__device__ __forceinline__ uint32_t combine_one(const BatchDesc& d, const Plan& pl, uint64_t per_seg,
                                             uint64_t i, uint64_t S, uint64_t E, int lane)
 {
     const uint64_t g0 = kMode == kSegAligned ? i * per_seg
@@ -207,8 +207,10 @@
     const uint32_t pad = uint32_t(pend - E);
     if (pad)
         R = mulmod_dev(R, g_tab.xinv[pad]);
+    const uint32_t v = (d.flags & RAMCRC_FINALIZE) ? ~R : R;
     if (lane == 0)
-        d.out[i] = (d.flags & RAMCRC_FINALIZE) ? ~R : R;
+        d.out[i] = v;
+    return v;
 }
 
 template <int kMode, bool kWide>
diff --git a/ramcloud_amd/csrc/dev_host.inc b/ramcloud_amd/csrc/dev_host.inc
--- a/ramcloud_amd/csrc/dev_host.inc
+++ b/ramcloud_amd/csrc/dev_host.inc
@@ -73,8 +73,6 @@
     uint64_t walk_recs_cap = 0;
     void* walk_pool = nullptr;
     uint64_t walk_pool_cap = 0;
-    uint32_t* walk_pool_owner = nullptr;
-    uint64_t walk_pool_owner_cap = 0;
     uint32_t* walk_blocks = nullptr;
     uint64_t walk_blocks_cap = 0;
     unsigned long long* walk_pool_used = nullptr;
@@ -282,11 +280,10 @@
 }
 
 template <int kMode>
-int launch_planned(ramcrc_ctx* c, const BatchDesc& d, hipStream_t s, const uint32_t** nother = nullptr,
-                   const uint32_t* sum = nullptr)
+int launch_planned(ramcrc_ctx* c, const BatchDesc& d, hipStream_t s, const uint32_t** nother = nullptr)
 {
     Sorted so;
-    int rc = bin_begin<kMode>(c, d, s, 1, &so, sum);
+    int rc = bin_begin<kMode>(c, d, s, 1, &so);
     if (rc)
         return rc;
     if (nother)
@@ -312,8 +309,8 @@
         hipLaunchKernelGGL((k_combine<kMode, false>), dim3((d.n + 3) / 4), dim3(256), 0, s, d, pl,
                            uint64_t(0));
     HIPCHK(hipGetLastError());
-    return bin_finish<kMode>(c, d, s, 1, so, sum);
-}
-
-
-}
+    return bin_finish<kMode>(c, d, s, 1, so);
+}
+
+
+}
diff --git a/ramcloud_amd/csrc/dev_plan.inc b/ramcloud_amd/csrc/dev_plan.inc
--- a/ramcloud_amd/csrc/dev_plan.inc
+++ b/ramcloud_amd/csrc/dev_plan.inc
@@ -2,11 +2,8 @@
 namespace {
 
 template <int kMode>
-__global__ __launch_bounds__(kThreads) void k_plan_count(BatchDesc d, Plan pl)
+__device__ __forceinline__ void plan_count_groups(const BatchDesc& d, const Plan& pl, uint64_t* wsum)
 {
-    __shared__ uint64_t wsum[kWavesPerGroup];
-    if (plan_empty(pl))
-        return;
     const uint64_t n = entry_count<kMode>(d);
     for (uint64_t grp = blockIdx.x; grp < pl.ngroups; grp += gridDim.x) {
         const uint64_t i = grp * kThreads + threadIdx.x;
@@ -38,24 +35,26 @@
     }
 }
 
-__global__ __launch_bounds__(kThreads) void k_plan_scan(Plan pl)
+template <int kMode>
+__global__ __launch_bounds__(kThreads) void k_plan_count(BatchDesc d, Plan pl)
 {
     __shared__ uint64_t wsum[kWavesPerGroup];
-    __shared__ uint64_t carry_s;
+    if (plan_empty(pl))
+        return;
+    plan_count_groups<kMode>(d, pl, wsum);
+}
+
+template <bool kAgent>
+__device__ __forceinline__ void plan_scan_groups(const Plan& pl, uint64_t* wsum, uint64_t* carry_s_p)
+{
+    uint64_t& carry_s = *carry_s_p;
     const int lane = threadIdx.x & 63, w = threadIdx.x >> 6;
-    if (threadIdx.x == 0) {
-        carry_s = 0;
-        atomicAnd(pl.status, ~kStatusRefused);
-    }
-    if (plan_empty(pl)) {
-        if (threadIdx.x == 0)
-            pl.group_pref[pl.ngroups] = 0;
-        return;
-    }
-    __syncthreads();
     for (uint64_t base = 0; base < pl.ngroups; base += kThreads) {
         const uint64_t i = base + threadIdx.x;
-        const uint64_t c = i < pl.ngroups ? pl.group_pref[i] : 0;
+        uint64_t c = 0;
+        if (i < pl.ngroups)
+            c = kAgent ? __hip_atomic_load(&pl.group_pref[i], __ATOMIC_RELAXED, __HIP_MEMORY_SCOPE_AGENT)
+                       : pl.group_pref[i];
         uint64_t x = c;
 #pragma unroll
         for (int s = 1; s < 64; s <<= 1) {
@@ -80,6 +79,60 @@
         pl.group_pref[pl.ngroups] = carry_s;
 }
 
+__global__ __launch_bounds__(kThreads) void k_plan_scan(Plan pl)
+{
+    __shared__ uint64_t wsum[kWavesPerGroup];
+    __shared__ uint64_t carry_s;
+    if (threadIdx.x == 0) {
+        carry_s = 0;
+        atomicAnd(pl.status, ~kStatusRefused);
+    }
+    if (plan_empty(pl)) {
+        if (threadIdx.x == 0)
+            pl.group_pref[pl.ngroups] = 0;
+        return;
+    }
+    __syncthreads();
+    plan_scan_groups<false>(pl, wsum, &carry_s);
+}
+
+template <int kMode>
+__global__ __launch_bounds__(kThreads) void k_plan_fused(BatchDesc d, Plan pl, const uint32_t* sum,
+                                                         ramcrc_seg_status* status, uint64_t nseg,
+                                                         uint32_t* ticket)
+{
+    __shared__ uint64_t wsum[kWavesPerGroup];
+    __shared__ uint64_t carry_s;
+    __shared__ uint32_t is_last;
+    const uint32_t sv = *sum;
+    if ((sv & kSumFast) && (sv & kHardFull)) {
+        for (uint64_t s = uint64_t(blockIdx.x) * blockDim.x + threadIdx.x; s < nseg;
+             s += uint64_t(gridDim.x) * blockDim.x)
+            status[s].bad_objects = 0;
+    }
+    if (blockIdx.x == 0 && threadIdx.x == 0)
+        atomicAnd(pl.status, ~kStatusRefused);
+    if (plan_empty(pl)) {
+        if (blockIdx.x == 0 && threadIdx.x == 0)
+            pl.group_pref[pl.ngroups] = 0;
+        return;
+    }
+    plan_count_groups<kMode>(d, pl, wsum);
+    __threadfence();
+    __syncthreads();
+    if (threadIdx.x == 0) {
+        carry_s = 0;
+        is_last = atomicAdd(ticket, 1u) + 1 == gridDim.x;
+    }
+    __syncthreads();
+    if (!is_last)
+        return;
+    __threadfence();
+    if (threadIdx.x == 0)
+        atomicExch(ticket, 0u);
+    plan_scan_groups<true>(pl, wsum, &carry_s);
+}
+
 __global__ void k_test_dirty_bins(BinTable* bt, uint32_t par, uint32_t bin, uint32_t add)
 {
     if (bin < kNB)
diff --git a/ramcloud_amd/csrc/dev_walk.inc b/ramcloud_amd/csrc/dev_walk.inc
--- a/ramcloud_amd/csrc/dev_walk.inc
+++ b/ramcloud_amd/csrc/dev_walk.inc
@@ -16,7 +16,6 @@
     u32x4* entries;
     uint64_t cap;
     unsigned long long* n_entries;
-    const uint32_t* only;
     uint64_t* seg_base;
     uint32_t* sum;
 };
@@ -51,6 +50,175 @@
 #pragma unroll
     for (int k = 0; k < kWalkPer; k++)
         *reinterpret_cast<u32x4*>(win + (lane + kWaveSize * k) * 16) = r[k];
+}
+
+__device__ __forceinline__ void seg_walk_one(const WalkDesc& w, uint64_t seg,
+                                             uint8_t (*win)[kWalkWin], const uint32_t* tab,
+                                             const uint32_t* xm, int lane, uint32_t& hard)
+{
+    const uint64_t sb = reinterpret_cast<uint64_t>(w.base) + seg * w.stride;
+    const ramcrc_seg_cert cert = w.certs[seg];
+    unsigned long long rbase = 0, rdone = 0, rtotal = 0;
+    for (int pass = 0; pass < 2; pass++) {
+    uint32_t pos = 0, crc = 0xFFFFFFFFu, count = 0, flags = 0;
+    uint32_t rpos = 0, rq = 0;
+    uint32_t ns = 0;
+
+    auto flush = [&](uint32_t nrec, uint32_t tail) {
+        const uint32_t pn = __shfl_down(rpos, 1, kWaveSize);
+        const uint32_t nxt = lane + 1 == int(ns) ? tail : pn;
+        const uint32_t hdr = rq & 0xFF, lb = (hdr >> 6) + 1;
+        const uint32_t rlen = nxt - rpos - 1 - lb;
+        const uint32_t rinfo = hdr | (rlen > ~(rpos + 1 + lb) ? kRecOverlong : 0u);
+        uint32_t m = 0, r = 0;
+        if (lane < int(ns)) {
+            m = 1 + lb;
+            r = crc_small(tab, 0u, hdr | (rlen << 8), m < 4 ? m : 4);
+            if (m == 5)
+                r = crc_small(tab, r, rlen >> 24, 1);
+        }
+        uint32_t incl = m;
+#pragma unroll
+        for (int s = 1; s < kWaveSize; s <<= 1) {
+            const uint32_t y = __shfl_up(incl, s, kWaveSize);
+            if (lane >= s)
+                incl += y;
+        }
+        const uint32_t total = __shfl(incl, kWaveSize - 1, kWaveSize);
+        uint32_t c = lane < int(ns) ? mulmod_horner(r, xm[total - incl]) : 0u;
+#pragma unroll
+        for (int s = 1; s < kWaveSize; s <<= 1)
+            c ^= __shfl_xor(c, s, kWaveSize);
+        crc = mulmod_horner(crc, xm[total]) ^ c;
+        if (nrec && pass == 0) {
+            rtotal += nrec;
+        } else if (nrec) {
+            const unsigned long long b = rbase + rdone;
+            if (lane < int(nrec) && b + lane < w.cap) {
+                w.entries[b + lane] = u32x4{uint32_t(seg), rpos, rlen, rinfo};
+                hard |= w.sum ? replay_hard(rpos, rlen, rinfo) | kHardFull : 0u;
+            }
+            rdone += nrec;
+        }
+        ns = 0;
+    };
+
+    int cur = 0;
+    uint32_t wb = 0;
+    u32x4 pf[kWalkPer];
+    __syncthreads();
+    walk_issue(pf, sb, 0, w.capacity, lane);
+    walk_store(win[0], pf, lane);
+    walk_issue(pf, sb, kWalkStep, w.capacity, lane);
+    __syncthreads();
+
+    const uint32_t cap32 = uint32_t(w.capacity);
+    const uint32_t limit = cert.segment_length < cap32 ? cert.segment_length : cap32;
+    uint32_t steps = 0, tail = 0;
+    bool overrun = false;
+    while (pos < limit) {
+        if (steps >= cap32) {
+            flags |= RAMCRC_SEG_CYCLE;
+            break;
+        }
+        if (pos - wb > kWalkWin - 8) {
+            const uint64_t nb = uint64_t(wb) + kWalkStep;
+            if (uint64_t(pos) >= nb && uint64_t(pos) - nb <= kWalkWin - 8) {
+                walk_store(win[cur ^ 1], pf, lane);
+                cur ^= 1;
+                wb = uint32_t(nb);
+            } else {
+                wb = pos & ~15u;
+                walk_issue(pf, sb, wb, w.capacity, lane);
+                walk_store(win[cur], pf, lane);
+            }
+            __syncthreads();
+            walk_issue(pf, sb, uint64_t(wb) + kWalkStep, w.capacity, lane);
+        }
+        if (ns == uint32_t(kWaveSize))
+            flush(ns, pos);
+        const uint32_t* w32 = reinterpret_cast<const uint32_t*>(win[cur]);
+        const uint64_t wend = uint64_t(wb) + (kWalkWin - 8);
+        const uint32_t last = limit - 1 < wend ? limit - 1 : uint32_t(wend);
+        const uint32_t span = last - wb;
+        uint32_t nsmax = uint32_t(kWaveSize);
+        if (cap32 - steps < nsmax - ns)
+            nsmax = ns + (cap32 - steps);
+        const uint32_t ns0 = ns;
+        uint32_t next;
+        for (;;) {
+            const uint32_t o = pos - wb;
+            const uint32_t d0 = __builtin_amdgcn_readfirstlane(w32[o >> 2]);
+            const uint32_t d1 = __builtin_amdgcn_readfirstlane(w32[(o >> 2) + 1]);
+            const uint64_t q = ((uint64_t(d1) << 32) | d0) >> (8 * (o & 3));
+            const uint32_t t = (uint32_t(q) >> 6) & 3;
+            uint32_t fld;
+            uint64_t len64;
+            asm("s_lshl_b32 %0, %2, 19\n\ts_add_u32 %0, %0, 0x80008\n\ts_bfe_u64 %1, %3, %0"
+                : "=&s"(fld), "=s"(len64) : "s"(t), "s"(q) : "scc");
+            next = pos + t + 2 + uint32_t(len64);
+            const bool mine = lane == int(ns);
+            rpos = mine ? pos : rpos;
+            rq = mine ? uint32_t(q) : rq;
+            ns++;
+            if (next - wb > span)
+                break;
+            if (ns == nsmax)
+                break;
+            pos = next;
+        }
+        steps += ns - ns0;
+        tail = next;
+        if (next > cap32) {
+            flags |= RAMCRC_SEG_PAST_CAPACITY;
+            overrun = true;
+            break;
+        }
+        pos = next;
+    }
+    count = steps - (overrun ? 1u : 0u);
+    if (ns)
+        flush(overrun ? ns - 1 : ns, tail);
+    if (pass == 0) {
+        unsigned long long b = 0;
+        if (lane == 0 && rtotal)
+            b = atomicAdd(w.n_entries, rtotal);
+        rbase = __shfl(b, 0, kWaveSize);
+        if (lane == 0 && w.seg_base)
+            w.seg_base[seg] = rbase;
+        if (rtotal == 0)
+            pass = 1;
+    }
+    if (rbase + rtotal > w.cap)
+        flags |= RAMCRC_SEG_TABLE_FULL;
+    if (pass == 0)
+        continue;
+    const uint32_t fin = ~crc_small(tab, crc, cert.segment_length, 4);
+    if (!(flags & (RAMCRC_SEG_PAST_CAPACITY | RAMCRC_SEG_CYCLE))) {
+        if (pos > cert.segment_length)
+            flags |= RAMCRC_SEG_PAST_LENGTH;
+        else if (fin != cert.checksum)
+            flags |= RAMCRC_SEG_BAD_CHECKSUM;
+        else if (!(flags & RAMCRC_SEG_TABLE_FULL))
+            flags |= RAMCRC_SEG_OK;
+    }
+    if (lane == 0) {
+        ramcrc_seg_status st;
+        st.flags = flags;
+        st.checksum = fin;
+        st.entries = count;
+        st.bad_objects = 0;
+        w.status[seg] = st;
+    }
+    }
+}
+
+__device__ __forceinline__ void seg_walk_sum(const WalkDesc& w, uint32_t hard, int lane)
+{
+    const uint32_t hw = (__ballot(hard & 1u) ? 1u : 0u) | (__ballot(hard & 2u) ? 2u : 0u) |
+                       (__ballot(hard & 4u) ? 4u : 0u) | (__ballot(hard & kHardFull) ? kHardFull : 0u);
+    if (w.sum && hw && lane == 0)
+        atomicOr(w.sum, hw);
 }
 
 __global__ __launch_bounds__(kWaveSize) void k_seg_walk(WalkDesc w)
@@ -65,171 +233,9 @@
     const int lane = threadIdx.x;
     uint32_t hard = 0;
 
-    for (uint64_t seg = blockIdx.x; seg < w.nseg; seg += gridDim.x) {
-        if (w.only && !w.only[seg])
-            continue;
-        const uint64_t sb = reinterpret_cast<uint64_t>(w.base) + seg * w.stride;
-        const ramcrc_seg_cert cert = w.certs[seg];
-        unsigned long long rbase = 0, rdone = 0, rtotal = 0;
-        for (int pass = 0; pass < 2; pass++) {
-        uint32_t pos = 0, crc = 0xFFFFFFFFu, count = 0, flags = 0;
-        uint32_t rpos = 0, rq = 0;
-        uint32_t ns = 0;
-
-        auto flush = [&](uint32_t nrec, uint32_t tail) {
-            const uint32_t pn = __shfl_down(rpos, 1, kWaveSize);
-            const uint32_t nxt = lane + 1 == int(ns) ? tail : pn;
-            const uint32_t hdr = rq & 0xFF, lb = (hdr >> 6) + 1;
-            const uint32_t rlen = nxt - rpos - 1 - lb;
-            const uint32_t rinfo = hdr | (rlen > ~(rpos + 1 + lb) ? kRecOverlong : 0u);
-            uint32_t m = 0, r = 0;
-            if (lane < int(ns)) {
-                m = 1 + lb;
-                r = crc_small(tab, 0u, hdr | (rlen << 8), m < 4 ? m : 4);
-                if (m == 5)
-                    r = crc_small(tab, r, rlen >> 24, 1);
-            }
-            uint32_t incl = m;
-#pragma unroll
-            for (int s = 1; s < kWaveSize; s <<= 1) {
-                const uint32_t y = __shfl_up(incl, s, kWaveSize);
-                if (lane >= s)
-                    incl += y;
-            }
-            const uint32_t total = __shfl(incl, kWaveSize - 1, kWaveSize);
-            uint32_t c = lane < int(ns) ? mulmod_horner(r, xm[total - incl]) : 0u;
-#pragma unroll
-            for (int s = 1; s < kWaveSize; s <<= 1)
-                c ^= __shfl_xor(c, s, kWaveSize);
-            crc = mulmod_horner(crc, xm[total]) ^ c;
-            if (nrec && pass == 0) {
-                rtotal += nrec;
-            } else if (nrec) {
-                const unsigned long long b = rbase + rdone;
-                if (lane < int(nrec) && b + lane < w.cap) {
-                    w.entries[b + lane] = u32x4{uint32_t(seg), rpos, rlen, rinfo};
-                    hard |= w.sum ? replay_hard(rpos, rlen, rinfo) | kHardFull : 0u;
-                }
-                rdone += nrec;
-            }
-            ns = 0;
-        };
-
-        int cur = 0;
-        uint32_t wb = 0;
-        u32x4 pf[kWalkPer];
-        __syncthreads();
-        walk_issue(pf, sb, 0, w.capacity, lane);
-        walk_store(win[0], pf, lane);
-        walk_issue(pf, sb, kWalkStep, w.capacity, lane);
-        __syncthreads();
-
-        const uint32_t cap32 = uint32_t(w.capacity);
-        const uint32_t limit = cert.segment_length < cap32 ? cert.segment_length : cap32;
-        uint32_t steps = 0, tail = 0;
-        bool overrun = false;
-        while (pos < limit) {
-            if (steps >= cap32) {
-                flags |= RAMCRC_SEG_CYCLE;
-                break;
-            }
-            if (pos - wb > kWalkWin - 8) {
-                const uint64_t nb = uint64_t(wb) + kWalkStep;
-                if (uint64_t(pos) >= nb && uint64_t(pos) - nb <= kWalkWin - 8) {
-                    walk_store(win[cur ^ 1], pf, lane);
-                    cur ^= 1;
-                    wb = uint32_t(nb);
-                } else {
-                    wb = pos & ~15u;
-                    walk_issue(pf, sb, wb, w.capacity, lane);
-                    walk_store(win[cur], pf, lane);
-                }
-                __syncthreads();
-                walk_issue(pf, sb, uint64_t(wb) + kWalkStep, w.capacity, lane);
-            }
-            if (ns == uint32_t(kWaveSize))
-                flush(ns, pos);
-            const uint32_t* w32 = reinterpret_cast<const uint32_t*>(win[cur]);
-            const uint64_t wend = uint64_t(wb) + (kWalkWin - 8);
-            const uint32_t last = limit - 1 < wend ? limit - 1 : uint32_t(wend);
-            const uint32_t span = last - wb;
-            uint32_t nsmax = uint32_t(kWaveSize);
-            if (cap32 - steps < nsmax - ns)
-                nsmax = ns + (cap32 - steps);
-            const uint32_t ns0 = ns;
-            uint32_t next;
-            for (;;) {
-                const uint32_t o = pos - wb;
-                const uint32_t d0 = __builtin_amdgcn_readfirstlane(w32[o >> 2]);
-                const uint32_t d1 = __builtin_amdgcn_readfirstlane(w32[(o >> 2) + 1]);
-                const uint64_t q = ((uint64_t(d1) << 32) | d0) >> (8 * (o & 3));
-                const uint32_t t = (uint32_t(q) >> 6) & 3;
-                uint32_t fld;
-                uint64_t len64;
-                asm("s_lshl_b32 %0, %2, 19\n\ts_add_u32 %0, %0, 0x80008\n\ts_bfe_u64 %1, %3, %0"
-                    : "=&s"(fld), "=s"(len64) : "s"(t), "s"(q) : "scc");
-                next = pos + t + 2 + uint32_t(len64);
-                const bool mine = lane == int(ns);
-                rpos = mine ? pos : rpos;
-                rq = mine ? uint32_t(q) : rq;
-                ns++;
-                if (next - wb > span)
-                    break;
-                if (ns == nsmax)
-                    break;
-                pos = next;
-            }
-            steps += ns - ns0;
-            tail = next;
-            if (next > cap32) {
-                flags |= RAMCRC_SEG_PAST_CAPACITY;
-                overrun = true;
-                break;
-            }
-            pos = next;
-        }
-        count = steps - (overrun ? 1u : 0u);
-        if (ns)
-            flush(overrun ? ns - 1 : ns, tail);
-        if (pass == 0) {
-            unsigned long long b = 0;
-            if (lane == 0 && rtotal)
-                b = atomicAdd(w.n_entries, rtotal);
-            rbase = __shfl(b, 0, kWaveSize);
-            if (lane == 0 && w.seg_base)
-                w.seg_base[seg] = rbase;
-            if (rtotal == 0)
-                pass = 1;
-        }
-        if (rbase + rtotal > w.cap)
-            flags |= RAMCRC_SEG_TABLE_FULL;
-        if (pass == 0)
-            continue;
-        const uint32_t fin = ~crc_small(tab, crc, cert.segment_length, 4);
-        if (!(flags & (RAMCRC_SEG_PAST_CAPACITY | RAMCRC_SEG_CYCLE))) {
-            if (pos > cert.segment_length)
-                flags |= RAMCRC_SEG_PAST_LENGTH;
-            else if (fin != cert.checksum)
-                flags |= RAMCRC_SEG_BAD_CHECKSUM;
-            else if (!(flags & RAMCRC_SEG_TABLE_FULL))
-                flags |= RAMCRC_SEG_OK;
-        }
-        if (lane == 0) {
-            ramcrc_seg_status st;
-            st.flags = flags;
-            st.checksum = fin;
-            st.entries = count;
-            st.bad_objects = 0;
-            w.status[seg] = st;
-        }
-        }
-    }
-    {
-        const uint32_t hw = (__ballot(hard & 1u) ? 1u : 0u) | (__ballot(hard & 2u) ? 2u : 0u) |
-                           (__ballot(hard & 4u) ? 4u : 0u) | (__ballot(hard & kHardFull) ? kHardFull : 0u);
-        if (w.sum && hw && lane == 0)
-            atomicOr(w.sum, hw);
-    }
+    for (uint64_t seg = blockIdx.x; seg < w.nseg; seg += gridDim.x)
+        seg_walk_one(w, seg, win, tab, xm, lane, hard);
+    seg_walk_sum(w, hard, lane);
 }
 
 #ifndef RAMCRC_PART_SHIFT
@@ -295,6 +301,7 @@
     uint2* pool;
     uint32_t* pool_owner;
     uint32_t* blocks;
+    uint64_t clear_words;
     unsigned long long* pool_used;
     uint64_t pool_cap;
     uint32_t* sum;
@@ -478,6 +485,16 @@
 __global__ __launch_bounds__(kSyncWaves * kWaveSize) void k_walk_sync(PWalk w0)
 {
     const PWalk w = walk_geo(w0);
+    {
+        const uint64_t tid = uint64_t(blockIdx.x) * blockDim.x + threadIdx.x;
+        const uint64_t nt = uint64_t(gridDim.x) * blockDim.x;
+        u32x4* const m4 = reinterpret_cast<u32x4*>(w.blocks);
+        const uint64_t n4 = w.clear_words / 4;
+        for (uint64_t q = tid; q < n4; q += nt)
+            m4[q] = u32x4{~0u, ~0u, ~0u, ~0u};
+        if (tid < (w.clear_words & 3))
+            w.blocks[n4 * 4 + tid] = ~0u;
+    }
     __shared__ __attribute__((aligned(16))) uint8_t wins[kSyncWaves][kSyncStage];
     __shared__ uint16_t lists[kSyncWaves][kSyncRound];
     constexpr uint32_t kSU = kSyncStage / 1024;
@@ -858,9 +875,26 @@
 {
     const PWalk w = walk_geo(w0);
     __shared__ uint32_t tab[4 * 256];
-    __shared__ __attribute__((aligned(16))) uint8_t win[kFixWin];
+    static_assert(kFixWin <= 2 * kWalkWin, "the serial walker's windows hold the fix-up's");
+    __shared__ __attribute__((aligned(16))) uint8_t swin[2][kWalkWin];
+    __shared__ uint32_t xm[kWalkMeta + 1];
+    uint8_t* const win = &swin[0][0];
+    WalkDesc sw{};
+    sw.base = w.base;
+    sw.stride = w.stride;
+    sw.capacity = w.capacity;
+    sw.nseg = w.nseg;
+    sw.certs = w.certs;
+    sw.status = w.status;
+    sw.entries = w.entries;
+    sw.cap = w.cap;
+    sw.n_entries = w.n_entries;
+    sw.seg_base = w.seg_base;
+    sw.sum = w.sum;
     walk_tab_fill(tab);
     const int lane = threadIdx.x;
+    bool xm_filled = false;
+    uint32_t hard = 0;
     for (uint64_t seg = blockIdx.x; seg < w.nseg; seg += gridDim.x) {
         const uint32_t limit = walk_limit(w, seg);
         const ramcrc_seg_cert cert = w.certs[seg];
@@ -1213,6 +1247,13 @@
         if (fallback) {
             if (lane == 0)
                 w.fallback[seg] = 1;
+            if (!xm_filled) {
+                for (uint32_t t = threadIdx.x; t <= kWalkMeta; t += blockDim.x)
+                    xm[t] = g_tab.xmeta[t];
+                xm_filled = true;
+            }
+            seg_walk_one(sw, seg, swin, tab, xm, lane, hard);
+            __syncthreads();
             continue;
         }
         uint32_t flags = 0;
@@ -1243,6 +1284,7 @@
             w.status[seg] = st;
         }
     }
+    seg_walk_sum(sw, hard, lane);
 }
 
 __global__ __launch_bounds__(256) void k_walk_emit(PWalk w0)
diff --git a/ramcloud_amd/csrc/ramcrc_device.hip b/ramcloud_amd/csrc/ramcrc_device.hip
--- a/ramcloud_amd/csrc/ramcrc_device.hip
+++ b/ramcloud_amd/csrc/ramcrc_device.hip
@@ -160,7 +160,6 @@
     if (c->walk_base) (void)hipFree(c->walk_base);
     if (c->walk_recs) (void)hipFree(c->walk_recs);
     if (c->walk_pool) (void)hipFree(c->walk_pool);
-    if (c->walk_pool_owner) (void)hipFree(c->walk_pool_owner);
     if (c->walk_blocks) (void)hipFree(c->walk_blocks);
     if (c->walk_pool_used) (void)hipFree(c->walk_pool_used);
     if (c->walk_sum) (void)hipFree(c->walk_sum);
@@ -631,9 +630,12 @@
     std::lock_guard<std::recursive_mutex> lk(c->mu);
     DeviceGuard g(c->device);
     hipStream_t s = reinterpret_cast<hipStream_t>(stream);
+    const bool fresh = !c->walk_sum;
     int rc = grow_device(reinterpret_cast<void**>(&c->walk_sum), &c->walk_sum_cap, 4, sizeof(uint32_t));
     if (rc)
         return rc;
+    if (fresh)
+        HIPCHK(hipMemset(c->walk_sum, 0, 4 * sizeof(uint32_t)));
     rc = walk_impl(c, d_base, seg_stride, seg_capacity, n_seg, d_certs, d_status, d_entries,
                    entries_cap, d_n_entries, s, c->walk_sum,
                    entries_cap && c->verify_in_walk ? d_obj_crc : nullptr);
@@ -673,7 +675,6 @@
     w.entries = reinterpret_cast<u32x4*>(d_entries);
     w.cap = entries_cap;
     w.n_entries = reinterpret_cast<unsigned long long*>(d_n_entries);
-    w.only = nullptr;
     w.sum = sum;
     {
         int rc0 = grow_device(reinterpret_cast<void**>(&c->walk_base), &c->walk_base_cap, n_seg,
@@ -701,11 +702,8 @@
         if (!rc)
             rc = grow_device(&c->walk_pool, &c->walk_pool_cap, pool_blocks * kPartRec, sizeof(uint2));
         if (!rc)
-            rc = grow_device(reinterpret_cast<void**>(&c->walk_pool_owner), &c->walk_pool_owner_cap,
-                             pool_blocks, sizeof(uint32_t));
-        if (!rc)
             rc = grow_device(reinterpret_cast<void**>(&c->walk_blocks), &c->walk_blocks_cap,
-                             total * kMaxBlocks, sizeof(uint32_t));
+                             total * kMaxBlocks + pool_blocks, sizeof(uint32_t));
         if (!rc)
             rc = grow_device(reinterpret_cast<void**>(&c->walk_pool_used), &c->walk_pool_used_cap, 3,
                              sizeof(unsigned long long));
@@ -734,8 +732,8 @@
         uint32_t* geo = reinterpret_cast<uint32_t*>(c->walk_pool_used + 1);
         pw.geo = geo;
         pw.pool = static_cast<uint2*>(c->walk_pool);
-        pw.pool_owner = c->walk_pool_owner;
         pw.blocks = c->walk_blocks;
+        pw.pool_owner = c->walk_blocks + total * kMaxBlocks;
         pw.pool_used = c->walk_pool_used;
         pw.pool_cap = pool_blocks;
         pw.sum = sum;
@@ -746,8 +744,11 @@
             pw.left_cap = left_cap;
             pw.vmode = uint32_t(c->verify_in_walk);
         }
-        HIPCHK(hipMemsetAsync(c->walk_blocks, 0xFF, total * kMaxBlocks * sizeof(uint32_t), s));
-        HIPCHK(hipMemsetAsync(c->walk_pool_owner, 0xFF, pool_blocks * sizeof(uint32_t), s));
+        const uint64_t map_words = total * kMaxBlocks + pool_blocks;
+        if (nparts > 1)
+            pw.clear_words = map_words;
+        else
+            HIPCHK(hipMemsetAsync(c->walk_blocks, 0xFF, map_words * sizeof(uint32_t), s));
         hipLaunchKernelGGL(k_walk_probe, dim3(1), dim3(kWaveSize), 0, s, pw, c->walk_pshift, geo);
         HIPCHK(hipGetLastError());
         if (nparts > 1) {
@@ -783,7 +784,7 @@
             }
             HIPCHK(hipGetLastError());
         }
-        w.only = c->walk_fallback;
+        return RAMCRC_OK;
     }
     hipLaunchKernelGGL(k_seg_walk, dim3(grid), dim3(kWaveSize), 0, s, w);
     HIPCHK(hipGetLastError());
@@ -1381,20 +1382,39 @@
     d.seg_status = reinterpret_cast<const u32x4*>(d_status);
     d.out = d_obj_crc;
     d.flags = RAMCRC_FINALIZE;
-    if (sum && c->walk_left && !c->serial_walk) {
-        uint64_t gl = uint64_t(4) * c->ncu;
-        hipLaunchKernelGGL(k_left, dim3(gl), dim3(256), 0, s, d, d_status, sum, c->walk_left,
-                           reinterpret_cast<const unsigned long long*>(c->walk_pool_used + 2),
-                           c->walk_left_cap, n_seg);
-        HIPCHK(hipGetLastError());
-    }
-    const uint32_t* nother = nullptr;
-    rc = launch_planned<kRecords>(c, d, s, &nother, sum);
-    if (rc)
-        return rc;
     uint64_t grid = (entries_cap + 255) / 256;
     grid = grid < uint64_t(16) * c->ncu ? grid : uint64_t(16) * c->ncu;
-    hipLaunchKernelGGL(k_obj_compare, dim3(grid), dim3(256), 0, s, d, d_status, nother);
+    if (!sum) {
+        const uint32_t* nother = nullptr;
+        rc = launch_planned<kRecords>(c, d, s, &nother);
+        if (rc)
+            return rc;
+        hipLaunchKernelGGL(k_obj_compare, dim3(grid), dim3(256), 0, s, d, d_status, nother);
+        HIPCHK(hipGetLastError());
+        return RAMCRC_OK;
+    }
+    Sorted so;
+    rc = bin_begin<kRecords>(c, d, s, 1, &so, sum);
+    if (rc)
+        return rc;
+    Plan pl = make_plan(c, d.n);
+    pl.nlarge = &so.bt->ctr[so.par].nlarge;
+    const uint64_t gcap = uint64_t(4) * c->ncu;
+    hipLaunchKernelGGL(k_plan_fused<kRecords>, dim3(uint32_t(pl.ngroups < gcap ? pl.ngroups : gcap)),
+                       dim3(kThreads), 0, s, d, pl, sum, d_status, n_seg,
+                       c->walk_sum + 1);
+    HIPCHK(hipGetLastError());
+    {
+        ScanTimer t(c, s);
+        t.launch(k_chunks<kRecords>, dim3(c->ncu), dim3(kThreads), d, pl, uint64_t(0));
+    }
+    HIPCHK(hipGetLastError());
+    rc = bin_finish<kRecords>(c, d, s, 1, so, sum);
+    if (rc)
+        return rc;
+    hipLaunchKernelGGL(k_replay_tail, dim3(grid), dim3(256), 0, s, d, pl, d_status, sum,
+                       &so.bt->ctr[so.par].nother, c->walk_left,
+                       c->walk_pool_used ? c->walk_pool_used + 2 : nullptr, c->walk_left_cap);
     HIPCHK(hipGetLastError());
     return RAMCRC_OK;
 }
```

Result: no change. 6889 GB/s (-0.0%).
